# aleximmer/Laplace

Hardware: AMD Instinct MI355X
Metric: KFAC-GGN fit samples/sec, ResNet-18 (higher is better)
Workload: dtype f32 (fp16x2-split products, fp32 accumulate); 1 GPU; c4: ResNet-18 (CIFAR stem, BN frozen) full-network KFAC exact GGN fit, per-GPU minibatch 128, synthetic N(0,1) 3x32x32, 10 classes, N=50000; per_gpu_batch=128, parallelism=dp1, minibatches_in_flight=2

## Files before the change

### include/laplace_hip.h

```cpp
#ifndef LAPLACE_HIP_H
#define LAPLACE_HIP_H

#include <stddef.h>
#include <stdint.h>

#ifdef __cplusplus
extern "C" {
#endif

#define LK_OK 0
#define LK_EINVAL (-1)
#define LK_EWORKSPACE (-2)
#define LK_ELAUNCH (-3)
#define LK_ENOTCONV (-4)

#define LK_GRAM_UPPER_ONLY 1u
#define LK_GRAM_SLABS_PERSIST 2u

int lk_version(void);
const char* lk_last_error(void);

size_t lk_loss_workspace_bytes(int64_t B);
int lk_softmax_hess_sqrt_f32(const float* f, const int64_t* y, int64_t B, int64_t C, float* S,
                             float* loss_accum, float* ws, void* stream);

#define LK_SOFTMAX_CHOL_MAX_C 2000
int lk_softmax_hess_chol_f32(const float* f, const int64_t* y, int64_t B, int64_t C, float* S,
                             float* loss_accum, float* ws, void* stream);

int lk_sq_err_sum_f32(const float* f, const float* y, int64_t numel, float scale, float* loss_accum,
                      float* ws, void* stream);

size_t lk_gram_workspace_bytes(int64_t n, int64_t K);
size_t lk_gram_nt_workspace_bytes(int64_t nb_total, int64_t n, int64_t L);
#define LK_GRAM_TN 0
#define LK_GRAM_NT 1
#define LK_GRAM_CONV 2
#define LK_GRAM_XCORR_FULL 3
#define LK_GRAM_XCORR_STRIPS 4
int lk_gram_launch_variant(int entry, int64_t n, int64_t K, int64_t L, int vec4_ok, unsigned flags, int* out);
int lk_gram_slabs_reduce_f32(float* slabs, size_t slabs_bytes, int64_t n, int64_t L_nt, float alpha, float* C,
                             unsigned flags, void* stream);
int lk_gram_tn_f32(const float* X, int64_t K, int64_t n, int64_t ldx, float alpha, float* C,
                   unsigned flags, void* ws, size_t ws_bytes, void* stream);
int lk_gram_nt_f32(const float* X, int64_t nb, int64_t n, int64_t L, float alpha, float* C,
                   unsigned flags, void* ws, size_t ws_bytes, void* stream);
int lk_gram_nt_seg_f32(const float* const* segs, int64_t nseg, int64_t nb, int64_t n, int64_t L, float alpha,
                       float* C, unsigned flags, void* ws, size_t ws_bytes, void* stream);
int lk_gram_conv_nhwc_f32(const float* x, int64_t B, int64_t H, int64_t W, int64_t Cin, int kh, int kw,
                          int sh, int sw, int ph, int pw, int dh, int dw, float alpha, float* C,
                          unsigned flags, void* ws, size_t ws_bytes, void* stream);

int lk_conv3x3_pixgram_assemble_f32(const float* Cp, int64_t H, int64_t W, int64_t Cin, float alpha, float* A,
                                    void* stream);

int lk_conv3x3_pixpair_plan(int64_t H, int64_t W, int64_t Cin, int64_t* tile, int64_t* n_tiles, int64_t* n_blocks);
int lk_conv3x3_pixpair_tables(int64_t H, int64_t W, int64_t Cin, int32_t* tiles, int32_t* slots);
int lk_conv3x3_pixpair_accumulate_f32(const float* x, int64_t B, int64_t H, int64_t W, int64_t Cin, float alpha,
                                      float* blocks, const int32_t* tiles_dev, int64_t n_tiles, void* stream);
int lk_conv3x3_pixpair_assemble_f32(const float* blocks, const int32_t* slots_dev, int64_t H, int64_t W, int64_t Cin,
                                    float alpha, float* A, void* stream);
int lk_conv3x3_pixpair_assemble2_f32(const float* blocks, const float* blocks2, const int32_t* slots_dev, int64_t H, int64_t W,
                                     int64_t Cin, float alpha, float* A, int upper_only, void* stream);
int lk_conv3x3_pixpair_accumulate_f16x2(const void* x_h, const void* x_l, const int* sexp, int64_t B, int64_t H, int64_t W,
                                        int64_t Cin, float alpha, float* blocks, const int32_t* tiles_dev, int64_t n_tiles,
                                        const void* zero16, void* stream);
int lk_conv3x3_pixpair_accumulate13_f16x2(const void* x_h, const void* x_l, const int* sexp, int64_t B, int64_t H, int64_t W,
                                          int64_t Cin, float alpha, float* blocks, const int32_t* slots_dev, const void* zero16,
                                          void* stream);

size_t lk_conv3x3_shiftcorr_workspace_bytes(int64_t B, int64_t H, int64_t W, int64_t Cin);
int lk_conv3x3_shiftcorr_f32(const float* x, int64_t B, int64_t H, int64_t W, int64_t Cin, float alpha, float* C,
                             void* ws, size_t ws_bytes, void* stream);

int lk_nchw_to_nhwc_f32(const float* src, int64_t B, int64_t C, int64_t HW, float* dst, void* stream);

int lk_symmetrize_f32(float* C, int64_t n, void* stream);

int lk_permute_sym_f32(const float* src, int64_t Cin, int64_t KK, float* dst, int accumulate, void* stream);

int lk_finalize_factors_f32(int64_t count, const float* const* src, float* const* dst, const float* const* scale,
                            const int64_t* n, const int64_t* cin, const int64_t* kk, void* stream);

int lk_absmax_f32(const float* x, int64_t n, const float* cscale, int64_t inner, int64_t C, unsigned* out, void* stream);
int lk_split_f16x2(const float* x, int64_t n, const float* amax, float bound_mul, void* planes_h, void* planes_l,
                   int* sexp, void* stream);
int lk_split_images_f16x2(const float* x, int64_t N, int64_t per, void* planes_h, void* planes_l, int* sexp, unsigned* amax,
                          void* stream);

int lk_im2col_split_f16x2(const float* x, int64_t B, int64_t H, int64_t W, int64_t C, int64_t KH, int64_t KW, int64_t stride,
                          int64_t pad, int64_t Ho, int64_t Wo, int64_t Kp, const float* amax, void* planes_h, void* planes_l,
                          int* sexp, void* stream);
int lk_conv_prep_weights_f16x2(const float* W, int64_t Co, int64_t Ci, int64_t taps, int transpose, const float* cscale,
                               unsigned* amax_ws, void* planes, int* sexp, void* stream);
int lk_conv_nhwc_f16x2(const void* in_h, const void* in_l, const int* in_sexp, int64_t in_nsexp, int64_t N, int64_t Hi,
                       int64_t Wi, int64_t Ci, const void* w_h, const void* w_l, const int* w_sexp, int64_t Co, int64_t Hc,
                       int64_t Wc, int64_t in_mul, int64_t Ho, int64_t Wo, int64_t out_step, int64_t oh0, int64_t ow0,
                       int64_t T, const int* taps, const void* zero16, float* out, int accumulate, unsigned* amax_out,
                       int config, void* stream);

int lk_conv_nhwc_f16x2_planes(const void* in_h, const void* in_l, const int* in_sexp, int64_t in_nsexp, const void* in_amax,
                              int64_t N, int64_t Hi, int64_t Wi, int64_t Ci, const void* w_h, const void* w_l,
                              const int* w_sexp, const float* w_l1, int64_t Co, int64_t Ho, int64_t Wo, int64_t in_mul, int64_t T,
                              const int* taps, const void* zero16, void* out_h, void* out_l, int* out_sexp, int config,
                              void* stream);

int lk_conv_bn_act_nhwc_f16x2(const void* in_h, const void* in_l, const int* in_sexp, int64_t in_nsexp, const void* in_amax,
                              int64_t in_namax, int64_t N, int64_t Hi, int64_t Wi, int64_t Ci, const void* w_h, const void* w_l,
                              const int* w_sexp, const float* w_l1, int64_t Co, int64_t Ho, int64_t Wo, int64_t in_mul,
                              int64_t T, const int* taps, const void* zero16, const float* scale, const float* shift,
                              const void* scale_amax, const void* shift_amax, const float* addend, const float* addend_bound,
                              int64_t addend_nbound, int act, float* y, void* mask, void* y_h, void* y_l, int* y_sexp,
                              float* y_bound, void* y_amax, int config, void* stream);

int lk_conv_nhwc_f16x2_vjp(const void* in_h, const void* in_l, const int* in_sexp, const void* in_amax, int64_t N, int64_t Hi,
                           int64_t Wi, int64_t Ci, const void* w_h, const void* w_l, const int* w_sexp, const float* w_l1,
                           int64_t Co, int64_t Ho, int64_t Wo, int64_t T, const int* taps, const void* zero16,
                           const void* add_h, const void* add_l, const int* add_sexp, const void* mask, int mask_is_float,
                           const void* mult_amax, int64_t mask_rows, const float* scale, const void* scale_amax, void* out_h,
                           void* out_l, int* out_sexp, void* out_amax, int config, void* stream);
int lk_conv_winp_eligible(int64_t N, int64_t Hi, int64_t Wi, int64_t Ci, int64_t Co, int64_t T, int mask_is_float);
int lk_conv_nhwc_f16x2_vjp_wc(const void* in_h, const void* in_l, const int* in_sexp, const void* in_amax, int64_t N, int64_t Hi,
                              int64_t Wi, int64_t Ci, const void* w_h, const void* w_l, const int* w_sexp, const float* w_l1,
                              const void* wc_h, const void* wc_l, int64_t Co, int64_t Ho, int64_t Wo, int64_t T, const int* taps,
                              const void* zero16, const void* add_h, const void* add_l, const int* add_sexp, const void* mask,
                              int mask_is_float, const void* mult_amax, int64_t mask_rows, const float* scale,
                              const void* scale_amax, void* out_h, void* out_l, int* out_sexp, void* out_amax, int config,
                              void* stream);

int lk_conv_nhwc_f16x2_vjp_strided(const void* in_h, const void* in_l, const int* in_sexp, const void* in_amax, const void* w_h,
                                   const void* w_l, const int* w_sexp, const float* w_l1, const void* in2_h, const void* in2_l,
                                   const int* in2_sexp, const void* in2_amax, const void* w2_h, const void* w2_l,
                                   const int* w2_sexp, const float* w2_l1, int64_t N, int64_t Hi, int64_t Wi, int64_t Ci,
                                   int64_t Co, int64_t Ho, int64_t Wo, int64_t os, int64_t T, const int* taps,
                                   const void* zero16, const void* add_h, const void* add_l, const int* add_sexp,
                                   const void* mask, int mask_is_float, const void* mult_amax, int64_t mask_rows,
                                   const float* scale, const void* scale_amax, void* out_h, void* out_l, int* out_sexp,
                                   void* out_amax, int config, void* stream);


int lk_vjp_nhwc_split_f16x2(const float* g, const unsigned* g_amax, const void* g2_h, const void* g2_l, const int* g2_sexp,
                            const void* m, int m_is_float, const unsigned* m_amax, const float* scale,
                            const unsigned* scale_amax, int64_t C, int64_t S, int64_t per, void* out_h, void* out_l,
                            int* out_sexp, void* stream);
int lk_bn_act_fwd_nhwc_f16x2(const float* x, const unsigned* x_amax, int64_t x_namax, const float* x_mul, const float* x_add,
                             const float* scale, const float* shift, const unsigned* scale_amax, const unsigned* shift_amax,
                             const float* addend, const float* addend_bound, int64_t addend_nbound, int act, int64_t C,
                             int64_t N, int64_t per, float* y, void* mask, void* y_h, void* y_l, int* y_sexp, float* y_bound,
                             unsigned* y_amax, void* stream);
int lk_copy_absmax_f32(const float* x, float* y, int64_t n, unsigned* amax, void* stream);

int lk_pack_upper_f32(const float* A, int64_t n, float* packed, void* stream);
int lk_unpack_upper_f32(const float* packed, int64_t n, float* A, void* stream);

int lk_gemm_f32(const float* A, const float* B, const float* E, float* C, int64_t batch, int64_t M, int64_t N, int64_t K,
                int64_t lda, int64_t ldb, int64_t ldc, int64_t lde, int64_t stride_a, int64_t stride_b, int64_t stride_c,
                int trans_a, int trans_b, float alpha, int accumulate, void* stream);
int lk_kron_pow_f32(const float* l1, int64_t n1, const float* l2, int64_t n2, const float* delta, float exponent,
                    int damping, float* lam, void* stream);
int lk_unsplit_transpose_f32(const void* x_h, const void* x_l, const int* sexp, int64_t S, int64_t B, int64_t L, int64_t C,
                             float* out, void* stream);
size_t lk_gram_tn_f16x2_workspace_bytes(int64_t R, int64_t C);
int lk_gram_tn_f16x2(const void* x_h, const void* x_l, const int* sexp, int64_t R, int64_t C, float alpha, float* G,
                     const void* zero16, void* ws, size_t ws_bytes, void* stream);

int lk_diag_ggn_linear_f32(const float* a, const float* g, int64_t B, int64_t Cc, int64_t Di, int64_t Do,
                           float alpha, float* h_w, float* h_b, void* stream);

int lk_jac_linear_f32(const float* a, const float* g, int64_t B, int64_t Cc, int64_t Di, int64_t Do,
                      float* Js, int64_t P, int64_t col0, int64_t bcol0, void* stream);
int lk_jac_conv_f32(const float* x_nchw, const float* g, int64_t B, int64_t Cc, int64_t Cin, int64_t H, int64_t W,
                    int64_t Do, int kh, int kw, int sh, int sw, int ph, int pw, int dh, int dw,
                    float* Js, int64_t P, int64_t col0, int64_t bcol0, void* stream);

int lk_jac_norm_affine_f32(const float* g, const float* xhat, int64_t S, int64_t B, int64_t L, int64_t Ch, int layout,
                           float* Js, int64_t P, int64_t wcol0, int64_t bcol0, void* stream);

int lk_jac_norm_affine_nhwc_f16x2(const void* g_h, const void* g_l, const int* sexp, const float* x, const float* mu,
                                  const float* rstd, int64_t S, int64_t B, int64_t L, int64_t Ch, float* Js, int64_t P,
                                  int64_t wcol0, int64_t bcol0, void* stream);
int lk_normtap_variant(int64_t S, int64_t B, int64_t L, int64_t Ch, int affine, int aligned);

#define LK_NORMVJP_ROW 0
#define LK_NORMVJP_TILE 1
int lk_norm_fwd_f32(const float* x, const float* w, const float* b, int64_t B, int64_t L, int64_t Ch, int64_t G, int layout,
                    float eps, float* y, float* xhat, float* rstd, void* stream);
int lk_norm_vjp_f32(const float* g, const float* xhat, const float* rstd, const float* w, int64_t S, int64_t B, int64_t L,
                    int64_t Ch, int64_t G, int layout, float* dx, unsigned* amax, void* stream);
int lk_norm_sweep_variant(int64_t S, int64_t B, int64_t L, int64_t Ch, int64_t G, int layout, int aligned);

int lk_rmsnorm_fwd_f32(const float* x, const float* w, int64_t rows, int64_t D, float eps, float* y, float* rstd,
                       void* stream);
int lk_rmsnorm_vjp_f32(const float* g, const float* x, const float* rstd, const float* w, int64_t S, int64_t rows, int64_t D,
                       float* dx, unsigned* amax, void* stream);
int lk_rmsnorm_variant(int64_t S, int64_t rows, int64_t D, int aligned);

#define LK_ATTN_RESIDENT_MAX_T 256
int lk_attn_fwd_f32(const float* q, const float* k, const float* v, int64_t B, int64_t H, int64_t T, int64_t D, int layout,
                    float scale, int causal, float* o, float* lse, void* stream);
size_t lk_attn_vjp_workspace_bytes(int64_t S, int64_t B, int64_t H, int64_t T, int64_t D);
int lk_attn_vjp_f32(const float* go, const float* q, const float* k, const float* v, const float* o, const float* lse, int64_t S,
                    int64_t B, int64_t H, int64_t T, int64_t D, int layout, float scale, int causal, float* dq, float* dk,
                    float* dv, void* ws, size_t ws_bytes, void* stream);
int lk_attn_variant(int64_t S, int64_t B, int64_t H, int64_t T, int64_t D, int layout, int causal);

#define LK_POOL_MAX 0
#define LK_POOL_AVG 1
int lk_pool_fwd_nhwc_f32(int kind, const float* x, int64_t B, int64_t H, int64_t W, int64_t C, int kh, int kw, int sh, int sw,
                         int ph, int pw, int count_include_pad, int divisor_override, float* y, uint8_t* arg, void* stream);
int lk_pool_vjp_nhwc_f32(int kind, const float* g, const uint8_t* arg, int64_t S, int64_t B, int64_t H, int64_t W, int64_t C,
                         int kh, int kw, int sh, int sw, int ph, int pw, int count_include_pad, int divisor_override, float* dx,
                         unsigned* amax, void* stream);
int lk_pool_variant(int kind, int64_t S, int64_t B, int64_t H, int64_t W, int64_t C, int kh, int kw, int sh, int sw, int ph,
                    int pw, int aligned);

int lk_dwconv_fwd_nhwc_f32(const float* x, const float* w_tap, const float* bias, int64_t B, int64_t H, int64_t W, int64_t C,
                           int kh, int kw, int sh, int sw, int ph, int pw, float* y, void* stream);
int lk_dwconv_bwd_nhwc_f16x2(const void* g_h, const void* g_l, const int* sexp, const float* w_tap, int64_t S, int64_t B,
                             int64_t H, int64_t W, int64_t C, int kh, int kw, int sh, int sw, int ph, int pw, float* dx,
                             unsigned* amax, void* stream);
int lk_dwconv_variant(int64_t S, int64_t B, int64_t H, int64_t W, int64_t C, int kh, int kw, int sh, int sw, int ph, int pw,
                      int aligned);
// ... 155 lines not shown
```

### laplace_amd/_lib.py

```python
from __future__ import annotations

import ctypes
import os
from typing import Optional

import torch

_HERE = os.path.dirname(os.path.abspath(__file__))
LIB_PATH = os.environ.get("LK_LIB") or os.path.join(_HERE, "csrc", "liblaplace_hip.so")

LK_GRAM_UPPER_ONLY = 1
LK_GRAM_SLABS_PERSIST = 2

_c_f32p = ctypes.c_void_p
_i64 = ctypes.c_int64
_int = ctypes.c_int
_f32 = ctypes.c_float
_sz = ctypes.c_size_t
_vp = ctypes.c_void_p
_u32 = ctypes.c_uint

SIGNATURES = {
    "lk_version": (_int, []),
    "lk_last_error": (ctypes.c_char_p, []),
    "lk_im2col_split_f16x2": (_int, [_vp, _i64, _i64, _i64, _i64, _i64, _i64, _i64, _i64, _i64, _i64, _i64, _vp, _vp, _vp, _vp, _vp]),
    "lk_comm_unique_id": (_int, [_vp]),
    "lk_comm_init_rank": (_int, [ctypes.POINTER(ctypes.c_void_p), _int, _vp, _int]),
    "lk_comm_destroy": (_int, [_vp]),
    "lk_allreduce_sum_f32": (_int, [_vp, _vp, _i64, _vp]),
    "lk_loss_workspace_bytes": (_sz, [_i64]),
    "lk_softmax_hess_sqrt_f32": (_int, [_vp, _vp, _i64, _i64, _vp, _vp, _vp, _vp]),
    "lk_softmax_hess_chol_f32": (_int, [_vp, _vp, _i64, _i64, _vp, _vp, _vp, _vp]),
    "lk_sq_err_sum_f32": (_int, [_vp, _vp, _i64, _f32, _vp, _vp, _vp]),
    "lk_gram_workspace_bytes": (_sz, [_i64, _i64]),
    "lk_gram_nt_workspace_bytes": (_sz, [_i64, _i64, _i64]),
    "lk_gram_launch_variant": (_int, [_int, _i64, _i64, _i64, _int, _u32, _vp]),
    "lk_gram_slabs_reduce_f32": (_int, [_vp, _sz, _i64, _i64, _f32, _vp, _u32, _vp]),
    "lk_gram_tn_f32": (_int, [_vp, _i64, _i64, _i64, _f32, _vp, _u32, _vp, _sz, _vp]),
    "lk_gram_nt_f32": (_int, [_vp, _i64, _i64, _i64, _f32, _vp, _u32, _vp, _sz, _vp]),
    "lk_gram_nt_seg_f32": (_int, [_vp, _i64, _i64, _i64, _i64, _f32, _vp, _u32, _vp, _sz, _vp]),
    "lk_gram_conv_nhwc_f32": (
        _int,
        [_vp, _i64, _i64, _i64, _i64, _int, _int, _int, _int, _int, _int, _int, _int, _f32, _vp, _u32, _vp, _sz, _vp],
    ),
    "lk_conv3x3_shiftcorr_workspace_bytes": (_sz, [_i64, _i64, _i64, _i64]),
    "lk_conv3x3_shiftcorr_f32": (_int, [_vp, _i64, _i64, _i64, _i64, _f32, _vp, _vp, _sz, _vp]),
    "lk_conv3x3_pixgram_assemble_f32": (_int, [_vp, _i64, _i64, _i64, _f32, _vp, _vp]),
    "lk_conv3x3_pixpair_plan": (_int, [_i64, _i64, _i64, _vp, _vp, _vp]),
    "lk_conv3x3_pixpair_tables": (_int, [_i64, _i64, _i64, _vp, _vp]),
    "lk_conv3x3_pixpair_accumulate_f32": (_int, [_vp, _i64, _i64, _i64, _i64, _f32, _vp, _vp, _i64, _vp]),
    "lk_conv3x3_pixpair_accumulate_f16x2": (_int, [_vp, _vp, _vp, _i64, _i64, _i64, _i64, _f32, _vp, _vp, _i64, _vp, _vp]),
    "lk_conv3x3_pixpair_accumulate13_f16x2": (_int, [_vp, _vp, _vp, _i64, _i64, _i64, _i64, _f32, _vp, _vp, _vp, _vp]),
    "lk_conv3x3_pixpair_assemble_f32": (_int, [_vp, _vp, _i64, _i64, _i64, _f32, _vp, _vp]),
    "lk_conv3x3_pixpair_assemble2_f32": (_int, [_vp, _vp, _vp, _i64, _i64, _i64, _f32, _vp, _int, _vp]),
    "lk_nchw_to_nhwc_f32": (_int, [_vp, _i64, _i64, _i64, _vp, _vp]),
    "lk_absmax_f32": (_int, [_vp, _i64, _vp, _i64, _i64, _vp, _vp]),
    "lk_copy_absmax_f32": (_int, [_vp, _vp, _i64, _vp, _vp]),
    "lk_split_f16x2": (_int, [_vp, _i64, _vp, _f32, _vp, _vp, _vp, _vp]),
    "lk_split_images_f16x2": (_int, [_vp, _i64, _i64, _vp, _vp, _vp, _vp, _vp]),
    "lk_conv_prep_weights_f16x2": (_int, [_vp, _i64, _i64, _i64, _int, _vp, _vp, _vp, _vp, _vp]),
    "lk_conv_nhwc_f16x2": (_int, [_vp, _vp, _vp, _i64, _i64, _i64, _i64, _i64, _vp, _vp, _vp, _i64, _i64, _i64, _i64, _i64, _i64,
                                  _i64, _i64, _i64, _i64, _vp, _vp, _vp, _int, _vp, _int, _vp]),
    "lk_conv_nhwc_f16x2_planes": (_int, [_vp, _vp, _vp, _i64, _vp, _i64, _i64, _i64, _i64, _vp, _vp, _vp, _vp, _i64, _i64, _i64, _i64,
                                         _i64, _vp, _vp, _vp, _vp, _vp, _int, _vp]),
    "lk_conv_bn_act_nhwc_f16x2": (_int, [_vp, _vp, _vp, _i64, _vp, _i64, _i64, _i64, _i64, _i64, _vp, _vp, _vp, _vp, _i64, _i64, _i64,
                                         _i64, _i64, _vp, _vp, _vp, _vp, _vp, _vp, _vp, _vp, _i64, _int, _vp, _vp, _vp, _vp, _vp,
                                         _vp, _vp, _int, _vp]),
    "lk_conv_nhwc_f16x2_vjp": (_int, [_vp, _vp, _vp, _vp, _i64, _i64, _i64, _i64, _vp, _vp, _vp, _vp, _i64, _i64, _i64, _i64,
                                      _vp, _vp, _vp, _vp, _vp, _vp, _int, _vp, _i64, _vp, _vp, _vp, _vp, _vp,
                                      _vp, _int, _vp]),
    "lk_conv_winp_eligible": (_int, [_i64, _i64, _i64, _i64, _i64, _i64, _int]),
    "lk_conv_nhwc_f16x2_vjp_wc": (_int, [_vp, _vp, _vp, _vp, _i64, _i64, _i64, _i64, _vp, _vp, _vp, _vp, _vp, _vp, _i64, _i64, _i64,
                                         _i64, _vp, _vp, _vp, _vp, _vp, _vp, _int, _vp, _i64, _vp, _vp, _vp, _vp, _vp, _vp, _int,
                                         _vp]),
    "lk_conv_nhwc_f16x2_vjp_strided": (_int, [_vp] * 16 + [_i64] * 9 + [_vp, _vp, _vp, _vp, _vp, _vp, _int, _vp, _i64, _vp, _vp, _vp,
                                               _vp, _vp, _vp, _int, _vp]),
    "lk_vjp_nhwc_split_f16x2": (_int, [_vp, _vp, _vp, _vp, _vp, _vp, _int, _vp, _vp, _vp, _i64, _i64, _i64, _vp, _vp, _vp, _vp]),
    "lk_bn_act_fwd_nhwc_f16x2": (_int, [_vp, _vp, _i64, _vp, _vp, _vp, _vp, _vp, _vp, _vp, _vp, _i64, _int, _i64, _i64, _i64, _vp, _vp,
                                        _vp, _vp, _vp, _vp, _vp, _vp]),
    "lk_unsplit_transpose_f32": (_int, [_vp, _vp, _vp, _i64, _i64, _i64, _i64, _vp, _vp]),
    "lk_gram_tn_f16x2_workspace_bytes": (_sz, [_i64, _i64]),
    "lk_gram_tn_f16x2": (_int, [_vp, _vp, _vp, _i64, _i64, _f32, _vp, _vp, _vp, _sz, _vp]),
    "lk_gemm_f32": (_int, [_vp, _vp, _vp, _vp, _i64, _i64, _i64, _i64, _i64, _i64, _i64, _i64, _i64, _i64, _i64, _int, _int, _f32,
                           _int, _vp]),
    "lk_kron_pow_f32": (_int, [_vp, _i64, _vp, _i64, _vp, _f32, _int, _vp, _vp]),
    "lk_pack_upper_f32": (_int, [_vp, _i64, _vp, _vp]),
    "lk_unpack_upper_f32": (_int, [_vp, _i64, _vp, _vp]),
    "lk_symmetrize_f32": (_int, [_vp, _i64, _vp]),
    "lk_permute_sym_f32": (_int, [_vp, _i64, _i64, _vp, _int, _vp]),
    "lk_finalize_factors_f32": (_int, [_i64, _vp, _vp, _vp, _vp, _vp, _vp, _vp]),
    "lk_diag_ggn_linear_f32": (_int, [_vp, _vp, _i64, _i64, _i64, _i64, _f32, _vp, _vp, _vp]),
    "lk_jac_linear_f32": (_int, [_vp, _vp, _i64, _i64, _i64, _i64, _vp, _i64, _i64, _i64, _vp]),
    "lk_jac_conv_f32": (
        _int,
        [_vp, _vp, _i64, _i64, _i64, _i64, _i64, _i64, _int, _int, _int, _int, _int, _int, _int, _int, _vp, _i64, _i64, _i64, _vp],
    ),
    "lk_jac_gconv_f32": (
        _int,
        [_vp, _vp, _i64, _i64, _i64, _i64, _i64, _i64, _i64, _int, _int, _int, _int, _int, _int, _int, _int, _vp, _i64, _i64, _i64,
         _vp],
    ),
    "lk_sq_colsum_f32": (_int, [_vp, _i64, _i64, _i64, _i64, _f32, _vp, _vp]),
    "lk_jac_norm_affine_f32": (_int, [_vp, _vp, _i64, _i64, _i64, _i64, _int, _vp, _i64, _i64, _i64, _vp]),
    "lk_norm_fwd_f32": (_int, [_vp, _vp, _vp, _i64, _i64, _i64, _i64, _int, _f32, _vp, _vp, _vp, _vp]),
    "lk_norm_vjp_f32": (_int, [_vp, _vp, _vp, _vp, _i64, _i64, _i64, _i64, _i64, _int, _vp, _vp, _vp]),
    "lk_norm_sweep_variant": (_int, [_i64, _i64, _i64, _i64, _i64, _int, _int]),
    "lk_rmsnorm_fwd_f32": (_int, [_vp, _vp, _i64, _i64, _f32, _vp, _vp, _vp]),
    "lk_rmsnorm_vjp_f32": (_int, [_vp, _vp, _vp, _vp, _i64, _i64, _i64, _vp, _vp, _vp]),
    "lk_rmsnorm_variant": (_int, [_i64, _i64, _i64, _int]),
    "lk_attn_fwd_f32": (_int, [_vp, _vp, _vp, _i64, _i64, _i64, _i64, _int, _f32, _int, _vp, _vp, _vp]),
    "lk_attn_vjp_workspace_bytes": (_sz, [_i64, _i64, _i64, _i64, _i64]),
    "lk_attn_vjp_f32": (_int, [_vp, _vp, _vp, _vp, _vp, _vp, _i64, _i64, _i64, _i64, _i64, _int, _f32, _int, _vp, _vp, _vp, _vp,
                               _sz, _vp]),
    "lk_attn_variant": (_int, [_i64, _i64, _i64, _i64, _i64, _int, _int]),
    "lk_pool_fwd_nhwc_f32": (_int, [_int, _vp, _i64, _i64, _i64, _i64] + [_int] * 8 + [_vp, _vp, _vp]),
    "lk_pool_vjp_nhwc_f32": (_int, [_int, _vp, _vp, _i64, _i64, _i64, _i64, _i64] + [_int] * 8 + [_vp, _vp, _vp]),
    "lk_pool_variant": (_int, [_int, _i64, _i64, _i64, _i64, _i64] + [_int] * 7),
    "lk_cat_fwd_nhwc_f32": (_int, [_vp, _i64, _i64, _vp, _i64, _i64, _vp]),
    "lk_cat_vjp_nhwc_f32": (_int, [_int, _vp, _vp, _vp, _vp, _i64, _i64, _i64, _i64, _vp, _vp, _vp]),
    "lk_cat_variant": (_int, [_int, _int, _i64, _i64, _i64, _i64, _int]),
    "lk_slice_fwd_f32": (_int, [_vp, _i64, _i64, _i64, _i64, _vp, _vp]),
    "lk_slice_vjp_f32": (_int, [_int, _vp, _vp, _vp, _vp, _vp, _vp, _i64, _i64, _vp, _vp, _vp]),
    "lk_slice_variant": (_int, [_int, _int, _vp, _vp, _i64, _i64, _int]),
    "lk_mul_vjp_f32": (_int, [_vp, _vp, _vp, _i64, _i64, _i64, _int, _vp, _vp, _vp]),
    "lk_mul_variant": (_int, [_i64, _i64, _i64, _int, _int, _int, _int]),
    "lk_gate_reduce_nhwc_f32": (_int, [_vp, _vp, _vp, _vp, _vp, _i64, _i64, _i64, _i64, _vp, _vp]),
    "lk_gate_vjp_nhwc_f32": (_int, [_vp, _vp, _vp, _vp, _vp, _vp, _i64, _i64, _i64, _i64, _vp, _vp, _vp]),
    "lk_gate_variant": (_int, [_int, _i64, _i64, _i64, _i64, _int]),
    "lk_softmax_vjp_f32": (_int, [_vp, _vp, _i64, _i64, _i64, _int, _vp, _vp]),
    "lk_softmax_vjp_variant": (_int, [_i64, _i64, _i64, _int, _int]),
    "lk_matmul_vjp_f32": (_int, [_vp, _vp, _vp, _i64, _i64, _i64, _i64, _i64, _vp, _vp, _vp]),
    "lk_matmul_vjp_variant": (_int, [_i64, _i64, _i64, _i64, _i64, _int, _int]),
    "lk_dwconv_fwd_nhwc_f32": (_int, [_vp, _vp, _vp, _i64, _i64, _i64, _i64] + [_int] * 6 + [_vp, _vp]),
    "lk_dwconv_bwd_nhwc_f16x2": (_int, [_vp, _vp, _vp, _vp, _i64, _i64, _i64, _i64, _i64] + [_int] * 6 + [_vp, _vp, _vp]),
    "lk_dwconv_variant": (_int, [_i64, _i64, _i64, _i64, _i64] + [_int] * 7),
    "lk_jac_norm_affine_nhwc_f16x2": (_int, [_vp] * 6 + [_i64] * 4 + [_vp, _i64, _i64, _i64, _vp]),
    "lk_normtap_variant": (_int, [_i64, _i64, _i64, _i64, _int, _int]),
    "lk_bn_act_fwd_f32": (_int, [_vp, _vp, _vp, _vp, _i64, _i64, _i64, _int, _vp, _vp, _vp]),
    "lk_vjp_scale_mask_f32": (_int, [_vp, _vp, _vp, _int, _vp, _i64, _i64, _i64, _i64, _vp, _vp]),
    "lk_ll_ggn_workspace_bytes": (_sz, [_i64, _i64, _i64]),
    "lk_ll_ggn_full_f32": (_int, [_vp, _vp, _i64, _i64, _i64, _int, _f32, _vp, _vp, _sz, _vp]),
    "lk_syevj_workspace_bytes": (_sz, [_i64]),
    "lk_syevj_f32": (_int, [_vp, _i64, _vp, _vp, _int, _int, _vp, _vp, _sz, _vp]),
    "lk_syevj_batched_f32": (_int, [_i64, _vp, _vp, _vp, _vp, _vp, _vp, _vp, _int, _int, _vp, _i64]),
    "lk_kron_logdet_workspace_bytes": (_sz, [_i64]),
    "lk_kron_logdet_f32": (_int, [_vp, _i64, _vp, _i64, _vp, _int, _vp, _vp, _vp, _vp, _vp, _sz, _vp]),
    "lk_kron_logdet_blocks_workspace_bytes": (_sz, [_i64, _i64]),
    "lk_kron_logdet_blocks_f32": (_int, [_i64, _vp, _vp, _vp, _vp, _vp, _vp, _vp, _vp, _vp, _vp, _sz, _vp]),
    "lk_kron_quadform_linear_f32": (_int, [_vp, _vp, _vp, _vp, _vp, _i64, _i64, _i64, _i64, _vp, _vp, _vp, _vp, _vp]),
    "lk_diag_quadform_linear_f32": (_int, [_vp, _vp, _vp, _vp, _i64, _i64, _i64, _i64, _vp, _vp]),
    "lk_quadform_shared_workspace_bytes": (_sz, [_i64, _i64, _i64, _i64]),
    "lk_kron_quadform_shared_planes_f16x2": (_int, [_vp, _vp, _vp, _vp, _vp, _vp, _i64, _vp, _vp, _vp, _i64, _i64, _i64, _i64, _i64,
                                                    _vp, _vp, _vp, _sz, _vp]),
    "lk_kron_quadform_shared_seedmajor_f32": (_int, [_vp, _vp, _vp, _vp, _vp, _i64, _i64, _i64, _i64, _i64, _vp, _vp, _sz, _vp]),
    "lk_kron_quadform_shared_f32": (_int, [_vp, _vp, _vp, _vp, _vp, _i64, _i64, _i64, _i64, _i64, _vp, _vp, _sz, _vp]),
    "lk_diag_quadform_shared_f32": (_int, [_vp, _vp, _vp, _i64, _i64, _i64, _i64, _i64, _vp, _vp, _sz, _vp]),
    "lk_diag_ggn_shared_workspace_bytes": (_sz, [_i64, _i64, _i64]),
    "lk_diag_ggn_shared_f32": (_int, [_vp, _vp, _i64, _i64, _i64, _i64, _i64, ctypes.c_float, _vp, _vp, _sz, _vp]),
    "lk_diag_quadform_js_f32": (_int, [_vp, _vp, _i64, _i64, _i64, _vp, _vp]),
    "lk_dense_quadform_ll_workspace_bytes": (_sz, [_i64, _i64, _i64]),
    "lk_jac_last_layer_f32": (_int, [_vp, _i64, _i64, _i64, _int, _vp, _vp]),
    "lk_dense_quadform_ll_f32": (_int, [_vp, _vp, _i64, _i64, _i64, _int, _vp, _vp, _sz, _vp]),
    "lk_quadform_linear_grid_f32": (_int, [_vp, _vp, _vp, _vp, _vp, _i64, _int, _i64, _i64, _i64, _i64, _vp, _vp, _vp, _vp]),
    "lk_quadform_shared_grid_workspace_bytes": (_sz, [_i64, _i64, _i64, _i64, _i64]),
    "lk_quadform_shared_grid_f32": (_int, [_vp, _vp, _vp, _vp, _vp, _i64, _int, _i64, _i64, _i64, _i64, _i64, _int, _vp, _vp, _sz,
                                           _vp]),
    "lk_quadform_shared_variant": (_int, [_int, _i64, _i64, _i64, _i64, _i64, _int]),
    "lk_conv_launch_variant": (_int, [_int] + [_i64] * 14 + [ctypes.POINTER(ctypes.c_int), _i64, _int, _int, _int,
                                      ctypes.POINTER(ctypes.c_int)]),
    "lk_conv_strided_launch_variant": (_int, [_i64] * 9 + [ctypes.POINTER(ctypes.c_int), _int, ctypes.POINTER(ctypes.c_int)]),
    "lk_probit_nll_grid_f32": (_int, [_vp, _vp, _vp, _i64, _i64, _i64, _vp, _vp]),
    "lk_spectral_workspace_bytes": (_sz, [_int, _i64, _i64, _i64, _i64]),
    "lk_spectral_quadform_ll_f32": (_int, [_vp, _vp, _vp, _f32, _vp, _i64, _i64, _i64, _int, _vp, _vp, _sz, _vp]),
    "lk_spectral_grid_ll_f32": (_int, [_vp, _vp, _vp, _f32, _vp, _i64, _i64, _i64, _i64, _int, _vp, _vp, _sz, _vp]),
    "lk_spectral_quadform_f32": (_int, [_vp, _vp, _f32, _vp, _i64, _i64, _i64, _vp, _vp, _sz, _vp]),
    "lk_spectral_grid_f32": (_int, [_vp, _vp, _f32, _vp, _i64, _i64, _i64, _i64, _vp, _vp, _sz, _vp]),
    "lk_spectral_variant": (_int, [_int, _i64, _i64, _i64, _i64, _int]),
}


class LaplaceHipError(RuntimeError):
    pass


class SplitTensor:

    __slots__ = ("planes", "sexp", "amax", "chunked")

    def __init__(self, planes: torch.Tensor, sexp: torch.Tensor, amax: torch.Tensor | None = None, chunked: bool = False):
        self.planes, self.sexp, self.amax, self.chunked = planes, sexp, amax, bool(chunked)

    @property
    def shape(self):
        if self.chunked:
            _, N, nch, D, w = self.planes.shape
            return torch.Size((N, D, nch * w))
        return self.planes.shape[1:]

    def chunk_major(self) -> "SplitTensor":
        if self.chunked:
            return self
        _, N, D, L = self.planes.shape
        pl = self.planes.view(2, N, D, L // 16, 16).permute(0, 1, 3, 2, 4).contiguous()
        return SplitTensor(pl, self.sexp, self.amax, chunked=True)

    @property
    def per_image(self) -> bool:
# ... 603 lines not shown
        out = torch.empty(B, S, C, H * W, dtype=torch.float32, device=x.planes.device)
        self._rc(self.lib.lk_unsplit_transpose_f32(_ptr(x.planes[0]), _ptr(x.planes[1]), _ptr(x.sexp), S, B, H * W, C,
                                                   _ptr(out), self._stream(out.device)), "lk_unsplit_transpose_f32")
        return out

    def gram_tn_f16x2(self, x, alpha, out):
        _check(out, "out")
        _one_scale(x, "gram_tn_f16x2")
        C = x.planes.shape[-1]
        R = x.planes[0].numel() // C
        nbytes = int(self.lib.lk_gram_tn_f16x2_workspace_bytes(R, C))
        if nbytes == 0 and R:
            raise LaplaceHipError(f"gram_tn_f16x2: C = {C} not supported (64 or a multiple of 128)")
        ws = self._workspace(nbytes, out.device)
        z = self._zero16(out.device)
        self._rc(self._timed("gram16", float(R) * C * (C + 1), out.device, lambda: self.lib.lk_gram_tn_f16x2(
            _ptr(x.planes[0]), _ptr(x.planes[1]), _ptr(x.sexp), R, C, float(alpha), _ptr(out), _ptr(z), _ptr(ws),
            ws.numel(), self._stream(out.device))), "lk_gram_tn_f16x2")
        return out

    def pack_upper(self, A, packed):
        _check(A, "A"), _check(packed, "packed")
        self._rc(self.lib.lk_pack_upper_f32(_ptr(A), A.shape[0], _ptr(packed), self._stream(A.device)), "lk_pack_upper_f32")

    def unpack_upper(self, packed, A):
        _check(A, "A"), _check(packed, "packed")
        self._rc(self.lib.lk_unpack_upper_f32(_ptr(packed), A.shape[0], _ptr(A), self._stream(A.device)), "lk_unpack_upper_f32")

    def gemm(self, A, B, C, batch, M, N, Kd, lda, ldb, ldc, sa=0, sb=0, sc=0, ta=False, tb=False, E=None, lde=0,
             alpha=1.0, accumulate=False):
        self._rc(self.lib.lk_gemm_f32(_ptr(A), _ptr(B), _ptr(E), _ptr(C), batch, M, N, Kd, lda, ldb, ldc, lde, sa, sb, sc,
                                      1 if ta else 0, 1 if tb else 0, float(alpha), 1 if accumulate else 0,
                                      self._stream(C.device)), "lk_gemm_f32")

    def kron_pow(self, l1, l2, delta, exponent, damping=False):
        _check(l1, "l1")
        n1 = l1.numel()
        n2 = 0 if l2 is None else l2.numel()
        lam = torch.empty((n1, n2) if l2 is not None else (n1,), dtype=torch.float32, device=l1.device)
        d = delta.detach().reshape(-1)[:1].to(torch.float32).contiguous()
        self._rc(self.lib.lk_kron_pow_f32(_ptr(l1), n1, _ptr(l2), n2, _ptr(d), float(exponent), 1 if damping else 0,
                                          _ptr(lam), self._stream(l1.device)), "lk_kron_pow_f32")
        return lam

    def kron_sandwich(self, W, col0, P, R, Q1, Q2, lam, out):
        _check(W, "W"), _check(out, "out"), _check(Q1, "Q1"), _check(lam, "lam")
        Wv, Ov = W.reshape(-1)[col0:], out.reshape(-1)[col0:]
        if Q2 is None:
            p = Q1.shape[0]
            T = torch.empty(R, p, dtype=torch.float32, device=W.device)
            self.gemm(Wv, Q1, T, 1, R, p, p, P, p, p, E=lam, lde=0)
            self.gemm(T, Q1, Ov, 1, R, p, p, p, p, P, tb=True)
            return out
        _check(Q2, "Q2")
        pi, po = Q1.shape[0], Q2.shape[0]
        T = torch.empty(R, pi, po, dtype=torch.float32, device=W.device)
        U = torch.empty(R, pi, po, dtype=torch.float32, device=W.device)
        self.gemm(Wv, Q2, T, R, pi, po, po, po, po, po, sa=P, sc=pi * po)
        self.gemm(Q1, T, U, R, pi, po, pi, pi, po, po, sb=pi * po, sc=pi * po, ta=True, E=lam, lde=po)
        self.gemm(Q1, U, T, R, pi, po, pi, pi, po, po, sb=pi * po, sc=pi * po)
        self.gemm(T, Q2, Ov, R, pi, po, po, po, po, po, sa=pi * po, sc=P, tb=True)
        return out

    def gram_conv(self, x, kernel_size, stride, padding, dilation, alpha, out, upper_only=False, native=False):
        _check(out, "out")
        if not self.is_channels_last(x):
            _check(x, "x")
        B, Cin, H, W = x.shape
        kh, kw = _pair(kernel_size)
        sh, sw = _pair(stride)
        ph, pw = _pair(padding)
        dh, dw = _pair(dilation)
        n = Cin * kh * kw
        assert out.shape == (n, n)
        OH = (H + 2 * ph - dh * (kh - 1) - 1) // sh + 1
        OW = (W + 2 * pw - dw * (kw - 1) - 1) // sw + 1
        xh = self.nchw_to_nhwc(x)
        direct = native or kh * kw == 1
        tgt = out if direct else torch.zeros(n, n, dtype=torch.float32, device=x.device)
        if self.use_shiftcorr and (kh, kw, sh, sw, ph, pw, dh, dw) == (3, 3, 1, 1, 1, 1, 1, 1) and H * W >= 256 and B > 0:
            nb = self.lib.lk_conv3x3_shiftcorr_workspace_bytes(B, H, W, Cin)
            ws = self._workspace(nb, x.device)
            self._rc(
                self._timed("shiftcorr", float(B * H * W) * n * (n + 1), x.device, lambda: self.lib.lk_conv3x3_shiftcorr_f32(
                    _ptr(xh), B, H, W, Cin, float(alpha), _ptr(tgt), _ptr(ws), ws.numel(), self._stream(x.device))),
                "lk_conv3x3_shiftcorr_f32",
            )
            if not direct:
                self._rc(self.lib.lk_permute_sym_f32(_ptr(tgt), Cin, kh * kw, _ptr(out), 1, self._stream(x.device)),
                         "lk_permute_sym_f32")
            return out
        nb = self.lib.lk_gram_workspace_bytes(n, max(B * OH * OW, 1))
        ws = self._workspace(nb, x.device)
        self._rc(
            self._timed("gram_conv", float(B * OH * OW) * n * (n + 1), x.device, lambda: self.lib.lk_gram_conv_nhwc_f32(
                _ptr(xh), B, H, W, Cin, kh, kw, sh, sw, ph, pw, dh, dw, float(alpha), _ptr(tgt),
                LK_GRAM_UPPER_ONLY if upper_only else 0, _ptr(ws), ws.numel(), self._stream(x.device))),
            "lk_gram_conv_nhwc_f32",
        )
        if not direct:
            self._rc(self.lib.lk_permute_sym_f32(_ptr(tgt), Cin, kh * kw, _ptr(out), 1, self._stream(x.device)),
                     "lk_permute_sym_f32")
        return out

    pixgram_max_hw = 16

    def pixgram_accumulate(self, x, alpha, Cp):
        _check(Cp, "Cp")
        B = x.shape[0]
        xh = self.nchw_to_nhwc(x)
        return self.gram_tn(xh.reshape(B, -1), alpha, Cp, upper_only=True)

    def pixgram_assemble(self, Cp, H, W, Cin, alpha, A_native):
        _check(Cp, "Cp"), _check(A_native, "A")
        self.symmetrize(Cp)
        self._rc(self.lib.lk_conv3x3_pixgram_assemble_f32(_ptr(Cp), int(H), int(W), int(Cin), float(alpha), _ptr(A_native),
                                                          self._stream(Cp.device)), "lk_conv3x3_pixgram_assemble_f32")
        return A_native

    def pixpair_plan(self, H, W, Cin, dev):
        key = (int(H), int(W), int(Cin), str(dev))
        cache = self.__dict__.setdefault("_pixpair_cache", {})
        if key not in cache:
            T, nt, nb = ctypes.c_int64(), ctypes.c_int64(), ctypes.c_int64()
            plan = None
            if Cin >= 64 and Cin % 64 == 0 and self.lib.lk_conv3x3_pixpair_plan(
                    int(H), int(W), int(Cin), ctypes.byref(T), ctypes.byref(nt), ctypes.byref(nb)) == 0:
                tiles = torch.empty(nt.value, 3, dtype=torch.int32)
                slots = torch.empty(int(H) * int(W), 13, dtype=torch.int32)
                self._rc(self.lib.lk_conv3x3_pixpair_tables(int(H), int(W), int(Cin), ctypes.c_void_p(tiles.data_ptr()),
                                                            ctypes.c_void_p(slots.data_ptr())), "lk_conv3x3_pixpair_tables")
                plan = (nb.value, tiles.to(dev), slots.to(dev))
            cache[key] = plan
        return cache[key]

    def pixpair_accumulate(self, x, alpha, blocks, plan):
        return self.pixpair_accumulate_nhwc(self.nchw_to_nhwc(x), alpha, blocks, plan)

    def pixpair_accumulate_nhwc(self, xh, alpha, blocks, plan):
        _check(xh, "xh"), _check(blocks, "blocks")
        B, H, W, Cin = xh.shape
        nb, tiles, _ = plan
        assert blocks.numel() == nb * Cin * Cin
        x = xh
        self._rc(self._timed("pixpair", 8.0 * blocks.numel() + 4.0 * x.numel(), x.device,
                             lambda: self.lib.lk_conv3x3_pixpair_accumulate_f32(
                                 _ptr(xh), B, H, W, Cin, float(alpha), _ptr(blocks), ctypes.c_void_p(tiles.data_ptr()),
                                 tiles.shape[0], self._stream(x.device))), "lk_conv3x3_pixpair_accumulate_f32")
        return blocks

    use_pixpair16 = True
    use_pixpair13 = True

    def pixpair_accumulate_split(self, xs, alpha, blocks, plan):
        _check(blocks, "blocks")
        _one_scale(xs, "pixpair_accumulate_split")
        B, H, W, Cin = xs.shape
        nb, tiles, slots = plan
        assert blocks.numel() == nb * Cin * Cin
        dev = blocks.device
        z = self._zero16(dev)
        if Cin == 64 and self.use_pixpair13:
            self._rc(self._timed("pixpair16", 8.0 * blocks.numel() + 4.0 * xs.planes[0].numel(), dev,
                                 lambda: self.lib.lk_conv3x3_pixpair_accumulate13_f16x2(
                                     _ptr(xs.planes[0]), _ptr(xs.planes[1]), _ptr(xs.sexp), B, H, W, Cin, float(alpha), _ptr(blocks),
                                     ctypes.c_void_p(slots.data_ptr()), _ptr(z), self._stream(dev))),
                     "lk_conv3x3_pixpair_accumulate13_f16x2")
            return blocks
        self._rc(self._timed("pixpair16", 8.0 * blocks.numel() + 4.0 * xs.planes[0].numel(), dev,
                             lambda: self.lib.lk_conv3x3_pixpair_accumulate_f16x2(
                                 _ptr(xs.planes[0]), _ptr(xs.planes[1]), _ptr(xs.sexp), B, H, W, Cin, float(alpha), _ptr(blocks),
                                 ctypes.c_void_p(tiles.data_ptr()), tiles.shape[0], _ptr(z), self._stream(dev))),
                 "lk_conv3x3_pixpair_accumulate_f16x2")
        return blocks

    def pixpair_assemble(self, blocks, plan, H, W, Cin, alpha, A_native, blocks2=None, upper_only=False):
        _check(blocks, "blocks"), _check(A_native, "A")
        if blocks2 is not None:
            _check(blocks2, "blocks2")
            assert blocks2.numel() == blocks.numel()
        self._rc(self.lib.lk_conv3x3_pixpair_assemble2_f32(_ptr(blocks), _ptr(blocks2), ctypes.c_void_p(plan[2].data_ptr()),
                                                           int(H), int(W), int(Cin), float(alpha), _ptr(A_native),
                                                           1 if upper_only else 0, self._stream(blocks.device)),
                 "lk_conv3x3_pixpair_assemble2_f32")
        return A_native

    def permute_native_to_unfold(self, src, Cin, KK, dst, accumulate=False):
        _check(src, "src"), _check(dst, "dst")
        self._rc(self.lib.lk_permute_sym_f32(_ptr(src), Cin, KK, _ptr(dst), 1 if accumulate else 0, self._stream(src.device)),
                 "lk_permute_sym_f32")
        return dst

    def finalize_factors(self, items):
        items = [it for it in items if it[0].numel()]
        if not items:
            return
        n = len(items)
        dev = items[0][0].device
        src = (ctypes.c_void_p * n)()
        dst = (ctypes.c_void_p * n)()
        scl = (ctypes.c_void_p * n)()
        ns = (ctypes.c_int64 * n)()
        cins = (ctypes.c_int64 * n)()
        kks = (ctypes.c_int64 * n)()
        for i, (s_, d_, sc_, cin, kk) in enumerate(items):
            _check(s_, "src")
            assert s_.dim() == 2 and s_.shape[0] == s_.shape[1] and s_.device == dev
            src[i] = s_.data_ptr()
            if d_ is not None:
                _check(d_, "dst")
                assert d_.shape == s_.shape
                dst[i] = d_.data_ptr()
            if sc_ is not None:
                _check(sc_, "scale")
                assert sc_.numel() == s_.shape[0]
                scl[i] = sc_.data_ptr()
            ns[i], cins[i], kks[i] = s_.shape[0], int(cin), int(kk)
        self._rc(self.lib.lk_finalize_factors_f32(n, src, dst, scl, ns, cins, kks, self._stream(dev)), "lk_finalize_factors_f32")

    def symmetrize(self, C):
        _check(C, "C")
        self._rc(self.lib.lk_symmetrize_f32(_ptr(C), C.shape[0], self._stream(C.device)), "lk_symmetrize_f32")
        return C

    def diag_ggn_linear(self, a, g, alpha, h_w, h_b=None):
        _check(a, "a"), _check(g, "g"), _check(h_w, "h_w")
        Cc, B, Do = g.shape
        Di = a.shape[1]
        assert a.shape[0] == B and h_w.numel() == Do * Di
        if h_b is not None:
            _check(h_b, "h_b")
        self._rc(
            self.lib.lk_diag_ggn_linear_f32(_ptr(a), _ptr(g), B, Cc, Di, Do, float(alpha), _ptr(h_w), _ptr(h_b),
                                            self._stream(a.device)),
            "lk_diag_ggn_linear_f32",
        )

    def jac_linear(self, a, g, Js, col0, bcol0=-1):
        _check(a, "a"), _check(g, "g"), _check(Js, "Js")
        Cc, B, Do = g.shape
        Di = a.shape[1]
        P = Js.shape[-1]
        self._rc(
            self.lib.lk_jac_linear_f32(_ptr(a), _ptr(g), B, Cc, Di, Do, _ptr(Js), P, int(col0), int(bcol0),
                                       self._stream(a.device)),
            "lk_jac_linear_f32",
        )

    def jac_conv(self, x, g, kernel_size, stride, padding, dilation, Js, col0, bcol0=-1):
        _check(x, "x"), _check(g, "g"), _check(Js, "Js")
        B, Cin, H, W = x.shape
        Cc, _, Do = g.shape[:3]
        kh, kw = _pair(kernel_size)
        sh, sw = _pair(stride)
        ph, pw = _pair(padding)
        dh, dw = _pair(dilation)
        P = Js.shape[-1]
        self._rc(
            self.lib.lk_jac_conv_f32(_ptr(x), _ptr(g), B, Cc, Cin, H, W, Do, kh, kw, sh, sw, ph, pw, dh, dw, _ptr(Js), P,
                                     int(col0), int(bcol0), self._stream(x.device)),
            "lk_jac_conv_f32",
        )

    def jac_gconv(self, x, g, kernel_size, stride, padding, dilation, groups, Js, col0, bcol0=-1):
        _check(x, "x"), _check(g, "g"), _check(Js, "Js")
        B, Cin, H, W = x.shape
        Cc, _, Do = g.shape[:3]
        if g.shape[1] != B or Js.shape[:2] != (B, Cc):
            raise LaplaceHipError("jac_gconv: x [B, Cin, H, W], g [S, B, Do, ...] and Js [B, S, P] do not match")
        kh, kw = _pair(kernel_size)
        sh, sw = _pair(stride)
        ph, pw = _pair(padding)
        dh, dw = _pair(dilation)
        self._rc(
            self.lib.lk_jac_gconv_f32(_ptr(x), _ptr(g), B, Cc, Cin, H, W, Do, int(groups), kh, kw, sh, sw, ph, pw, dh, dw,
                                      _ptr(Js), Js.shape[-1], int(col0), int(bcol0), self._stream(x.device)),
            "lk_jac_gconv_f32",
        )

    def jac_norm_affine(self, g, xhat, Ch, layout, Js, wcol0, bcol0=-1):
        _check(g, "g"), _check(xhat, "xhat"), _check(Js, "Js")
        S, B = g.shape[:2]
        if xhat.numel() * S != g.numel() or xhat.shape[0] != B or Js.shape[:2] != (B, S):
            raise LaplaceHipError("jac_norm_affine: g [S, B, ...], xhat [B, ...] and Js [B, S, P] do not match")
        L = xhat.numel() // max(B * int(Ch), 1)
        if B * L * int(Ch) != xhat.numel():
            raise LaplaceHipError("jac_norm_affine: xhat is not [B, Ch, L] / [B, L, Ch]")
        self._rc(
            self.lib.lk_jac_norm_affine_f32(_ptr(g), _ptr(xhat), S, B, L, int(Ch), int(layout), _ptr(Js), Js.shape[-1],
                                            int(wcol0), int(bcol0), self._stream(g.device)),
            "lk_jac_norm_affine_f32",
        )

    def jac_norm_affine_nhwc(self, g: "SplitTensor", x, mu, rstd, S, Js, wcol0, bcol0=-1):
        _one_scale(g, "jac_norm_affine_nhwc")
        if g.chunked:
            raise LaplaceHipError("jac_norm_affine_nhwc: a chunk-major split tensor is an operand of the weight-sharing "
                                  "predictive; this kernel reads position-major planes [S*B, .., Ch]")
        _check(g.planes, "g.planes", torch.float16), _check(g.sexp, "g.sexp", torch.int32), _check(x, "x"), _check(Js, "Js")
        S = int(S)
        if x.dim() < 2 or g.planes.dim() != x.dim() + 1 or S < 1 or g.planes.shape[1] != S * x.shape[0] \
                or tuple(g.planes.shape[2:]) != tuple(x.shape[1:]) or Js.dim() != 3 or tuple(Js.shape[:2]) != (x.shape[0], S):
            raise LaplaceHipError("jac_norm_affine_nhwc: g [S*B, .., Ch], x [B, .., Ch] and Js [B, S, P] do not match")
        B, Ch = x.shape[0], x.shape[-1]
        if (mu is None) != (rstd is None):
            raise LaplaceHipError("jac_norm_affine_nhwc: mu and rstd are given together or not at all")
        for name, t in (("mu", mu), ("rstd", rstd)):
            if t is not None and tuple(_check(t, name).shape) != (Ch,):
                raise LaplaceHipError(f"jac_norm_affine_nhwc: {name} must be [Ch]")
        L = x.numel() // max(B * Ch, 1)
        self._rc(
            self.lib.lk_jac_norm_affine_nhwc_f16x2(_ptr(g.planes[0]), _ptr(g.planes[1]), _ptr(g.sexp), _ptr(x), _ptr(mu), _ptr(rstd),
                                                   S, B, max(L, 1), Ch, _ptr(Js), Js.shape[-1], int(wcol0), int(bcol0),
                                                   self._stream(x.device)),
            "lk_jac_norm_affine_nhwc_f16x2",
        )

    def normtap_variant(self, S, B, L, Ch, affine=True, aligned=True):
        r = int(self.lib.lk_normtap_variant(int(S), int(B), int(L), int(Ch), int(bool(affine)), int(bool(aligned))))
        if r < 0:
            return None
        return {"vec": (1, 4, 8)[r & 3], "seed_split": bool(r & 4), "affine": bool(r & 8), "seeds_per_pass": (r >> 4) & 0xF,
                "lane_rows": 1 << ((r >> 8) & 0xF), "seeds_per_slice": (r >> 12) & 0xFF, "channel_tiles": r >> 20}

    @staticmethod
    def _norm_geometry(x, B, G, layout, what):
        if x.dim() < 2 or x.shape[0] != B:
            raise LaplaceHipError(f"{what}: expected [B, Ch, ...] / [B, ..., Ch]")
        Ch = int(x.shape[1] if layout == 0 else x.shape[-1])
        L = x.numel() // max(B * Ch, 1) if x.numel() else 1
        if G < 1 or Ch % G or layout not in (0, 1):
            raise LaplaceHipError(f"{what}: G must divide the {Ch} channels; layout is 0 or 1")
        return max(L, 1), Ch

    def norm_forward(self, x, w, b, G, layout, eps):
        _check(x, "x")
        B = x.shape[0]
        L, Ch = self._norm_geometry(x, B, int(G), int(layout), "norm_forward")
        for t, name in ((w, "w"), (b, "b")):
            if t is not None:
                _check(t, name)
                if t.numel() != Ch:
                    raise LaplaceHipError(f"norm_forward: {name} must have {Ch} elements")
        y, xhat = torch.empty_like(x), torch.empty_like(x)
        rstd = torch.empty(B, int(G), dtype=torch.float32, device=x.device)
        self._rc(self.lib.lk_norm_fwd_f32(_ptr(x), _ptr(w), _ptr(b), B, L, Ch, int(G), int(layout), float(eps), _ptr(y),
                                          _ptr(xhat), _ptr(rstd), self._stream(x.device)), "lk_norm_fwd_f32")
        return y, xhat, rstd

    def norm_vjp(self, g, xhat, rstd, w, S, G, layout, amax=None):
        _check(g, "g"), _check(xhat, "xhat"), _check(rstd, "rstd")
        B = xhat.shape[0]
        L, Ch = self._norm_geometry(xhat, B, int(G), int(layout), "norm_vjp")
        if g.numel() != int(S) * xhat.numel() or rstd.numel() != B * int(G):
            raise LaplaceHipError("norm_vjp: g [S*B, ...], xhat [B, ...] and rstd [B, G] do not match")
        if w is not None:
            _check(w, "w")
            if w.numel() != Ch:
                raise LaplaceHipError(f"norm_vjp: w must have {Ch} elements")
        if amax is not None and (amax.numel() != 1 or amax.element_size() != 4):
            raise LaplaceHipError("norm_vjp: amax is one 32-bit device word")
        dx = torch.empty_like(g)
        self._rc(self.lib.lk_norm_vjp_f32(_ptr(g), _ptr(xhat), _ptr(rstd), _ptr(w), int(S), B, L, Ch, int(G), int(layout),
                                          _ptr(dx), _ptr(amax), self._stream(g.device)), "lk_norm_vjp_f32")
        return dx

    NORMVJP_ROW, NORMVJP_TILE = 0, 1

    def norm_sweep_variant(self, S, B, L, Ch, G, layout, aligned=True):
        r = int(self.lib.lk_norm_sweep_variant(int(S), int(B), int(L), int(Ch), int(G), int(layout), int(bool(aligned))))
        if r < 0:
# ... 894 lines not shown
```

### laplace_amd/backend.py

```python
from __future__ import annotations

import collections
import math
import threading
import os
from collections.abc import MutableMapping

import torch
import torch.nn.functional as F
from torch import nn

from laplace_amd._lib import SplitTensor, get_kernels, is_channels_last, keep_layout
from laplace_amd.capture import NormTapReused, Tape, norm_servable
from laplace_amd.sweep import SeedBatchedSweep, SweepUnsupported
from laplace_amd.sweep_nhwc import NhwcNormGrad, SplitSweep
from laplace_amd.kron import HipKron
from laplace_amd.refapi import EFInterface, GGNInterface


_OWN_ROTATION = True


def shared_operands(tap, g, B, C, Q1=None, Q2=None, bounds=None, planes: bool = True):
    m = tap.module
# ... 565 lines not shown
            K.jac_norm_affine(g.g.reshape(g.g.shape[0] // B, *g.xhat.shape), g.xhat, self._norm_channels(tap.module), 1, Js,
                              wcol0, bcol0)
        else:
            xhat, Ch, layout = self._norm_xhat(tap)
            K.jac_norm_affine(g.contiguous(), xhat, Ch, layout, Js, wcol0, bcol0)

    def _norm_block(self, tap, g):
        Ch = self._norm_channels(tap.module)
        if isinstance(g, (SplitTensor, NhwcNormGrad)):
            B = tap.a.shape[0]
            S, dev = (g.shape[0] if isinstance(g, SplitTensor) else g.g.shape[0]) // B, tap.a.device
        else:
            S, B, dev = g.shape[0], g.shape[1], g.device
        n_w, n_b = (Ch if tap.w_off >= 0 else 0), (Ch if tap.b_off >= 0 else 0)
        Jl = torch.zeros(B, S, n_w + n_b, dtype=torch.float32, device=dev)
        self._norm_columns(tap, g, Jl, 0 if n_w else -1, n_w if n_b else -1)
        return Jl, n_w, n_b

    def _kron_impl(self, x, y, N, seeds_fn, hess_scale_fn, kfac_approx):
        if kfac_approx not in ("expand", "reduce"):
            raise ValueError(f"kfac_approx must be 'expand' or 'reduce', got {kfac_approx!r}")
        acc = KronAccumulator(self, N, kfac_approx, overlap=True)
        acc.defer_pix = bool(self.lazy_kron and self.lazy_pixpair and acc.use_pixgram and kfac_approx == "expand")
        if not acc.defer_pix:
            acc.use_pixgram = False
        acc._persist_slabs = False
        acc.lanes = 1
        acc.coalesce = False
        try:
            acc.add_batch(x, y)
        except NotImplementedError as e:
            if "KFAC supports" in str(e):
                raise NotImplementedError(
                    "KFAC supports nn.Linear / nn.Conv2d parameters only (as the reference, docs/index.md:364-366); "
                    "freeze the others (requires_grad=False)") from e
            raise
        if self.lazy_kron:
            return acc.loss[0].clone(), HipKron(None, pending=acc)
        return acc.finalize()

    lazy_kron = True
    lazy_pixpair = True

    def _diag_impl(self, x, y, seeds_fn, alpha):
        K = get_kernels()
        f, tape, grad_fn = self._forward(x, norm=True)
        if self._unserved(tape):
            tape.release()
            return None
        loss = torch.zeros(1, dtype=torch.float32, device=f.device)
        seeds, _ = seeds_fn(f, y, loss)
        grads = grad_fn(seeds)
        h = torch.zeros(tape.n_params, dtype=torch.float32, device=f.device)
        B, S = f.shape[0], seeds.shape[0]
        for tap, g in zip(self._served_taps(tape), grads):
            if tap.kind == "norm":
                Jl, n_w, n_b = self._norm_block(tap, g)
                if n_w:
                    K.sq_colsum(Jl, 0, n_w, alpha, h[tap.w_off:tap.w_off + n_w])
                if n_b:
                    K.sq_colsum(Jl, n_w, n_b, alpha, h[tap.b_off:tap.b_off + n_b])
                continue
            if tap.kind == "gconv":
                for _, Jl, n_w, n_b in self._gconv_blocks(tap, g):
                    K.sq_colsum(Jl, 0, n_w, alpha, h[tap.w_off:tap.w_off + n_w])
                    if n_b:
                        K.sq_colsum(Jl, n_w, n_b, alpha, h[tap.b_off:tap.b_off + n_b])
                continue
            a = tap.a.to(torch.float32)
            m = tap.module
            if tap.kind == "linear" and a.ndim == 2:
                n_w = m.out_features * m.in_features
                K.diag_ggn_linear(a.contiguous(), g.contiguous(), alpha, h[tap.w_off:tap.w_off + n_w],
                                  h[tap.b_off:tap.b_off + m.out_features] if tap.has_bias else None)
            else:
                width = m.weight.numel()
                n_out = m.weight.shape[0]
                if n_out >= 32 and width // n_out >= 64:
                    smax = K.quadform_shared_max_outputs
                    u, v, gsum = shared_operands(tap, g, B, S)
                    for s0 in range(0, S, smax):
                        us = u if S <= smax else u[:, s0:s0 + smax].contiguous()
                        K.diag_ggn_shared(us, v, alpha, h[tap.w_off:tap.w_off + width])
                    if tap.has_bias:
                        h[tap.b_off:tap.b_off + n_out] += alpha * (gsum * gsum).sum((0, 1))
                else:
                    Jl = torch.zeros(B, S, width + (n_out if tap.has_bias else 0), dtype=torch.float32, device=f.device)
                    a4, g5, ks, st, pd, dl = self._conv_view(tap, a, g)
                    K.jac_conv(a4, g5, ks, st, pd, dl, Jl, 0, width if tap.has_bias else -1)
                    K.sq_colsum(Jl, 0, width, alpha, h[tap.w_off:tap.w_off + width])
                    if tap.has_bias:
                        K.sq_colsum(Jl, width, n_out, alpha, h[tap.b_off:tap.b_off + n_out])
        tape.release()
        if self.subnetwork_indices is not None:
            h = h[self.subnetwork_indices]
        return loss[0], h

    def _full_from_rows(self, Z, alpha):
        K = get_kernels()
        Z2 = Z.reshape(-1, Z.shape[-1])
        if self.subnetwork_indices is not None:
            Z2 = Z2[:, self.subnetwork_indices]
        Z2 = Z2.contiguous()
        H = torch.zeros(Z2.shape[1], Z2.shape[1], dtype=torch.float32, device=Z.device)
        return K.gram_tn(Z2, alpha, H)


class CurvatureExchange(list):

    owner = None


_PROCESS_STREAMS: dict = {}
_PROCESS_STREAMS_LOCK = threading.Lock()


def _process_streams(key, make):
    with _PROCESS_STREAMS_LOCK:
        return _process_streams_locked(key, make)


def _process_streams_locked(key, make):
    hit = _PROCESS_STREAMS.get(key)
    if hit is None:
        hit = _PROCESS_STREAMS[key] = make()
    return hit


class KronAccumulator:

    use_pixgram = True
    _defer_bn = True
    _persist_slabs = True
    pix_group = 8
    lag_join = True

    def __init__(self, backend, N: int, kfac_approx: str = "expand", overlap: bool = True):
        twin, dt = backend._twin() if hasattr(backend, "_twin") else (None, torch.float32)
        self._caller, self._out_dtype = (backend, dt) if twin is not None else (None, torch.float32)
        if twin is not None:
            backend = twin
        self.backend, self.N, self.kfac_approx = backend, N, kfac_approx
        self.overlap = overlap
        self._side = None
        self._side_done = None
        self._side_older = []
        self.lag_depth = 1
        self.factors = None
        self.loss = None
        self._taps_meta = None
        self.defer_pix = False
        self._pix_inputs = {}
        self._pix_early = set()
        self.coalesce = bool(type(self).default_coalesce)
        self._stash, self._stash_n = [], 0
        self._dispatched = 0
        self._act_numel = 0
        self.lanes = max(1, int(type(self).default_lanes))
        self._lane_accs, self._lane_next, self._lane_id, self._lane_stream = None, 0, 0, None
        self._lane_sig = None
        self._ahead = collections.deque()
        self._a_done = None
        self._lanes_anywhere = False

    def _alloc(self, tape, dev):
        self.factors, self._taps_meta = [], []
        shapes = []
        for tap in tape.taps:
            m = tap.module
            if tap.kind == "linear":
                do, di = m.out_features, m.in_features
                native = None
            else:
                do, di = m.out_channels, m.in_channels * m.kernel_size[0] * m.kernel_size[1]
                native = (m.in_channels, m.kernel_size[0] * m.kernel_size[1])
            shapes.append((do, di, native is not None and native[1] > 1))
            self._taps_meta.append((tap.has_bias, native))
        pad = lambda n: (n + 63) // 64 * 64
        kept = sum(pad(do * do) + (0 if nat else pad(di * di)) for do, di, nat in shapes) + 64
        natv = sum(pad(di * di) for do, di, nat in shapes if nat)
        flat_k = torch.zeros(kept, dtype=torch.float32, device=dev)
        flat_n = torch.zeros(natv, dtype=torch.float32, device=dev) if natv else None
        ok, on = 0, 0
        for do, di, nat in shapes:
            G = flat_k[ok:ok + do * do].view(do, do)
            ok += pad(do * do)
            if nat:
                A = flat_n[on:on + di * di].view(di, di)
                on += pad(di * di)
            else:
                A = flat_k[ok:ok + di * di].view(di, di)
                ok += pad(di * di)
            self.factors.append([G, A])
        self.loss = flat_k[ok:ok + 1]
        self._pix = {}
        self._pix_pending = {}
        self._gscale = {}
        self._gslabs = {}
        self._tap_index = {tap.name: i for i, tap in enumerate(tape.taps)}

    def ensure_allocated(self, device):
        self._fold_lanes()
        if self.factors is None:
            self._alloc(self.backend._tape(), device)

    def _pix_geometry(self, tap):
        m = tap.module
        if tap.kind != "conv2d" or self.kfac_approx != "expand" or not self.use_pixgram:
            return None
        if (tuple(m.kernel_size), tuple(m.stride), tuple(m.padding), tuple(m.dilation)) != ((3, 3), (1, 1), (1, 1), (1, 1)):
            return None
        K = get_kernels()
        H, W = (int(v) for v in tap.a.shape[-2:])
        Cin = int(m.in_channels)
        if H * W > K.pixgram_max_hw or Cin % 64 == 0:
            plan = K.pixpair_plan(H, W, Cin, tap.a.device)
            if plan is not None and plan[0] * Cin * Cin * 4 <= (1 << 30):
                return ("pair", H, W, Cin, plan)
        if H * W <= K.pixgram_max_hw and H * W * Cin <= 16384:
            return ("dense", H, W, Cin)
        return None

    def _accumulate_A(self, idx, tap, F, rt):
        K = get_kernels()
        if self.defer_pix:
            geo = self._pix_geometry(tap)
            if geo is not None and geo[0] == "pair" and tap.a.dtype == torch.float32:
                t = K.nchw_to_nhwc(keep_layout(tap.a))
                self._pix_inputs.setdefault(idx, []).append((geo, rt / (self.N * geo[1] * geo[2]), t, tap.module))
                return
            self.backend._factor_A(tap, self.N, rt, self.kfac_approx, F[1], fused=True)
            return
        acc = self._pix.get(idx)
        if acc is None:
            self.backend._factor_A(tap, self.N, rt, self.kfac_approx, F[1], fused=True)
            return
        geo, buf = acc
        alpha = rt / (self.N * geo[1] * geo[2])
        a = keep_layout(tap.a.to(torch.float32))
        if geo[0] != "pair":
            K.pixgram_accumulate(a, alpha, buf)
        elif self.pix_group <= 1:
            K.pixpair_accumulate(a, alpha, buf, geo[4])
        else:
            self._push_pix_input(idx, geo, alpha, a, nhwc=False)

    direct_stack = True

    def _pix_sink(self, name, shape, device):
        idx = self._tap_index.get(name)
        pend = self._pix_pending.get(idx) if idx is not None else None
        if pend is None or pend["n"] >= self.pix_group:
            return None
        B = pend["B"]
        stack = pend["stack"]
        if tuple(shape) != (B,) + tuple(stack.shape[1:]) or stack.device != device:
            return None
        cur = torch.cuda.current_stream(device)
        free = pend.pop("free", None)
        if free is not None:
            cur.wait_event(free)
        stack.record_stream(cur)
        return stack[pend["n"] * B:(pend["n"] + 1) * B]

    def _push_pix_input(self, idx, geo, alpha, a, nhwc: bool):
        K = get_kernels()
        B = a.shape[0]
        pend = self._pix_pending.get(idx)
        if pend is not None and (pend["B"] != B or pend["alpha"] != alpha):
            self._drain_pixpair(idx)
            pend = None
        if pend is None:
            stack = torch.empty(self.pix_group * B, geo[1], geo[2], geo[3], dtype=torch.float32, device=a.device)
            planes = (torch.empty((2,) + tuple(stack.shape), dtype=torch.float16, device=a.device)
                      if getattr(K, "use_pixpair16", False) and stack.numel() % 8 == 0 else None)
            word = torch.zeros(1, dtype=torch.float32, device=a.device) if planes is not None and getattr(K, "use_copy_absmax", False) else None
            pend = self._pix_pending[idx] = {"B": B, "alpha": alpha, "stack": stack, "n": 0, "planes": planes, "amax": word}
        slot = pend["stack"][pend["n"] * B:(pend["n"] + 1) * B]
        src = a if nhwc else (a.permute(0, 2, 3, 1) if K.is_channels_last(a) else None)
        if src is not None and src.data_ptr() == slot.data_ptr() and tuple(src.shape) == tuple(slot.shape) and src.is_contiguous():
            pend["amax"] = None
        elif (pend["amax"] is not None and src is not None and src.is_contiguous() and src.dtype == torch.float32
                and src.numel() % 4 == 0 and src.data_ptr() % 16 == 0 and slot.data_ptr() % 16 == 0):
            K.copy_absmax(src, slot, pend["amax"])
        else:
            pend["amax"] = None
            if nhwc:
                slot.copy_(a)
            else:
                K.nchw_to_nhwc(a, out=slot)
        pend["n"] += 1
        if pend["n"] == self.pix_group:
            self._drain_pixpair(idx, keep=True)

    def _adopt_pix_inputs(self, other):
        todo = []
        for idx, items in other._pix_inputs.items():
            if idx not in self._pix:
                mine = self._pix_inputs.setdefault(idx, [])
                mine.extend(items)
                if len(mine) < max(self.pix_group, 2):
                    continue
                geo = mine[0][0]
                self._pix[idx] = (geo, torch.zeros(geo[4][0] * geo[3] * geo[3], dtype=torch.float32, device=mine[0][2].device))
                items = self._pix_inputs.pop(idx)
            todo.append((idx, items))
        return todo

    def _push_adopted(self, todo):
        for idx, items in todo:
            for geo, alpha, t, _ in items:
                self._push_pix_input(idx, geo, alpha, t, nhwc=True)

    def _resolve_pix_inputs(self):
        if not self._pix_inputs:
            return
        K = get_kernels()
        self._join_side()
        for idx, items in self._pix_inputs.items():
            for _, alpha, t, m in items:
                K.gram_conv(t.permute(0, 3, 1, 2), m.kernel_size, m.stride, m.padding, m.dilation, alpha, self.factors[idx][1],
                            upper_only=True, native=True)
        self._pix_inputs = {}

    def _drain_pixpair(self, idx, keep=False):
        pend = self._pix_pending.get(idx)
        if pend is None:
            return
        if pend["n"]:
            geo, buf = self._pix[idx]
            xh = pend["stack"][:pend["n"] * pend["B"]]
            cur = torch.cuda.current_stream(xh.device) if xh.is_cuda else None
            K = get_kernels()
            if getattr(K, "use_pixpair16", False) and xh.numel() % 8 == 0:
                ws = pend.get("planes")
                xs = K.split_f16x2(xh, amax=pend.get("amax"), out=None if ws is None else ws[:, :xh.shape[0]])
                if cur is not None and keep:
                    pend["free"] = torch.cuda.Event()
                    pend["free"].record(cur)
                K.pixpair_accumulate_split(xs, pend["alpha"], buf, geo[4])
            else:
                K.pixpair_accumulate_nhwc(xh, pend["alpha"], buf, geo[4])
                if cur is not None and keep:
                    pend["free"] = torch.cuda.Event()
                    pend["free"].record(cur)
            if cur is not None:
                pend["stack"].record_stream(cur)
                if pend.get("planes") is not None:
                    pend["planes"].record_stream(cur)
                if pend.get("amax") is not None:
                    pend["amax"].record_stream(cur)
        if keep:
            pend["n"] = 0
            if pend.get("planes") is not None and getattr(get_kernels(), "use_copy_absmax", False):
                pend["amax"] = torch.zeros(1, dtype=torch.float32, device=pend["stack"].device)
        else:
            del self._pix_pending[idx]

    def _ensure_pixgrams(self, tape):
        todo = []
        for idx, tap in enumerate(tape.taps):
            if idx in self._pix:
                old = self._pix[idx][0]
                if (old[1], old[2]) == tuple(int(v) for v in tap.a.shape[-2:]):
                    continue
                self._flush_pixgrams(only=idx)
                self._pix_early.add(idx)
            geo = self._pix_geometry(tap)
            if geo is None:
                continue
            if geo[0] == "pair":
                todo.append((idx, geo, (geo[4][0] * geo[3] * geo[3],), tap.a.device))
            else:
                npix = geo[1] * geo[2] * geo[3]
                todo.append((idx, geo, (npix, npix), tap.a.device))
        if not todo:
            return
        pad = lambda n: (n + 63) // 64 * 64
        numel = [math.prod(shape) for _, _, shape, _ in todo]
        flat = torch.zeros(sum(pad(n) for n in numel), dtype=torch.float32, device=todo[0][3])
        off = 0
        for (idx, geo, shape, _), n in zip(todo, numel):
            self._pix[idx] = (geo, flat[off:off + n].view(shape))
            off += pad(n)

    flush_streams = 3
    lane_priority = -1

    def _flush_pixgrams(self, only=None):
        K = get_kernels()
        self._join_side()
        todo = [only] if only is not None else sorted(self._pix, key=lambda i: -self._pix[i][1].numel())

        def one(idx):
            self._drain_pixpair(idx)
            geo, buf = self._pix.pop(idx)
            if geo[0] == "pair":
                K.pixpair_assemble(buf, geo[4], geo[1], geo[2], geo[3], 1.0, self.factors[idx][1], upper_only=True)
            else:
                K.pixgram_assemble(buf, geo[1], geo[2], geo[3], 1.0, self.factors[idx][1])
            return buf

        dev = self.loss.device if self.loss is not None else None
        if len(todo) < 3 or self.flush_streams < 2 or dev is None or dev.type != "cuda" or not self.overlap:
            for idx in todo:
                one(idx)
            return
        streams = _process_streams(("flush", dev, self.flush_streams), lambda: [torch.cuda.Stream(dev) for _ in range(self.flush_streams)])
        cur = torch.cuda.current_stream(dev)
        for st in streams:
            st.wait_stream(cur)
        for j, idx in enumerate(todo):
            st = streams[j % len(streams)]
            with torch.cuda.stream(st):
                buf = one(idx)
            buf.record_stream(st)
            self.factors[idx][1].record_stream(st)
        for st in streams:
            cur.wait_stream(st)

    def _lane_add_batch(self, x, y):
        dev = x.device
        on_device = x.is_cuda
        cur = torch.cuda.current_stream(dev) if on_device else None
        if self._lane_accs is None:
            streams = [None] * self.lanes
            if on_device:
                prio = int(self.lane_priority)
                streams = _process_streams(("lanes", dev, self.lanes, prio),
                                           lambda: [torch.cuda.Stream(dev, priority=prio) for _ in range(self.lanes)])
            self._lane_accs = []
            for k in range(self.lanes):
                sub = KronAccumulator(self.backend, self.N, self.kfac_approx, self.overlap)
                sub.lanes, sub._lane_id, sub._lane_stream = 1, k, streams[k]
                sub.coalesce = False
                sub.use_pixgram, sub.pix_group, sub.lag_join = self.use_pixgram, self.pix_group, self.lag_join
                sub.lag_depth, sub.direct_stack = self.lag_depth, self.direct_stack
                sub._defer_bn, sub._persist_slabs = self._defer_bn, self._persist_slabs
                self._lane_accs.append(sub)
        k = self._lane_next
        self._lane_next = (k + 1) % self.lanes
        sub = self._lane_accs[k]
        if not on_device:
            sub.add_batch(x, y)
            return
        st = sub._lane_stream
        x = x.clone()
        y = y.clone() if torch.is_tensor(y) and y.is_cuda else y
        st.wait_stream(cur)
        if sub.factors is None and k > 0 and self.backend.__dict__.get("_lanes_warm") != self._shared_signature(x):
            first = self._lane_accs[0]
            st.wait_stream(first._lane_stream)
            if first._side is not None:
                st.wait_stream(first._side)
        if self._lane_sig is None:
            self._lane_sig = self._shared_signature(x)
        with torch.cuda.stream(st):
            sub.add_batch(x, y)
        for t in (x, y):
            if torch.is_tensor(t) and t.is_cuda:
                t.record_stream(st)
        self._act_numel = max(self._act_numel, sub._act_numel)
        sub.max_ahead = self.max_ahead
        sub._throttle(st)

    def _shared_signature(self, x):
        m = self.backend.model
        ts = list(m.parameters()) + list(m.buffers())
        return (tuple((t.data_ptr(), t._version) for t in ts), tuple(x.shape[1:]), x.dtype, x.device)

    early_flush = True
    drain_before_fold = True

    def _fold_lanes(self):
        self._flush_stash()
        subs, self._lane_accs = self._lane_accs, None
        if not subs:
            return
        if self._lane_sig is not None and any(sub.factors is not None for sub in subs):
            self.backend.__dict__["_lanes_warm"] = self._lane_sig
        K = get_kernels()
        on_device = subs[0]._lane_stream is not None
        dev = subs[0]._lane_stream.device if on_device else None
        cur = torch.cuda.current_stream(dev) if on_device else None
        live = [sub for sub in subs if sub.factors is not None]
        if on_device and self.drain_before_fold:
            for sub in subs:
                sub._lane_stream.synchronize()
                if sub._side is not None:
                    sub._side.synchronize()
        early = (on_device and self.overlap and self.early_flush and bool(live) and all(sub._a_done is not None for sub in live)
                 and any(sub._pix for sub in live))
        fstreams = None
        if early:
            nfs = max(self.flush_streams, 1)
            fstreams = _process_streams(("flush", dev, nfs), lambda: [torch.cuda.Stream(dev) for _ in range(nfs)])
            for st in fstreams:
                st.wait_stream(cur)
                for sub in live:
                    st.wait_event(sub._a_done)
        else:
            for sub in subs:
                if on_device:
                    cur.wait_stream(sub._lane_stream)
            for sub in live:
                sub._join_side()
        merged = set()
        if live:
            base = live[0]

            def one(idx, st):
                geo, buf = base._pix[idx]
                others = []
                for sub in live[1:]:
                    o = sub._pix.get(idx)
                    if o is None or o[0][:4] != geo[:4] or (geo[0] == "pair" and o[0][4] is not geo[4]):
                        continue
                    pend = sub._pix_pending.pop(idx, None)
                    if pend is not None and pend["n"]:
                        bp = base._pix_pending.get(idx)
                        B = pend["B"]
                        if (bp is not None and bp["B"] == B and bp["alpha"] == pend["alpha"]
                                and bp["n"] + pend["n"] <= bp["stack"].shape[0] // B):
                            bp["stack"][bp["n"] * B:(bp["n"] + pend["n"]) * B].copy_(pend["stack"][:pend["n"] * B])
                            bp["n"] += pend["n"]
                            if bp.get("amax") is not None:
                                if pend.get("amax") is not None:
                                    torch.maximum(bp["amax"], pend["amax"], out=bp["amax"])
                                else:
                                    bp["amax"] = None
                            if st is not None:
                                pend["stack"].record_stream(st)
                        else:
                            sub._pix_pending[idx] = pend
                            sub._drain_pixpair(idx)
                    others.append(o[1])
                    del sub._pix[idx]
                if not others:
                    return False
                base._drain_pixpair(idx)
                del base._pix[idx]
                A = base.factors[idx][1]
                for o in others[1:]:
                    buf.add_(o)
                if geo[0] == "pair":
                    K.pixpair_assemble(buf, geo[4], geo[1], geo[2], geo[3], 1.0, A, blocks2=others[0], upper_only=True)
                else:
                    buf.add_(others[0])
                    K.pixgram_assemble(buf, geo[1], geo[2], geo[3], 1.0, A)
                if st is not None:
                    for t in [buf, A] + others:
                        t.record_stream(st)
                return True

            todo = sorted(base._pix, key=lambda i: -base._pix[i][1].numel())
            for j, idx in enumerate(todo):
                if fstreams is not None:
                    st = fstreams[j % len(fstreams)]
                    with torch.cuda.stream(st):
                        if one(idx, st):
                            merged.add(idx)
                elif one(idx, None):
                    merged.add(idx)
        if early:
            for sub in subs:
                cur.wait_stream(sub._lane_stream)
            for sub in live:
                sub._join_side()
            for st in fstreams:
                cur.wait_stream(st)
        first = True
        for sub in subs:
            if sub.factors is None:
                continue
            sub._flush_pixgrams()
            sub._flush_g_slabs()
            if self.factors is None:
                self.factors, self.loss, self._taps_meta = sub.factors, sub.loss, sub._taps_meta
                self._pix, self._pix_pending, self._gslabs = {}, {}, {}
                self._gscale, self._tap_index = dict(sub._gscale), dict(sub._tap_index)
            else:
                if set(self._gscale) != set(sub._gscale):
                    raise RuntimeError("the lanes of a fit disagree about the deferred BatchNorm scales")
                skip = (merged - sub._pix_early) if not first else set()
                mine = [t for i, F in enumerate(self.factors) for j, t in enumerate(F) if not (j == 1 and i in skip)] + [self.loss]
                theirs = [t for i, F in enumerate(sub.factors) for j, t in enumerate(F) if not (j == 1 and i in skip)] + [sub.loss]
                torch._foreach_add_(mine, theirs)
            first = False
            if on_device:
                for t in sub._raw_tensors():
                    t.record_stream(cur)

    default_coalesce = True
    default_lanes = 2
    coalesce_act_floats = 1 << 28
    coalesce_max_batches = 32

    def coalesce_target(self, x) -> int:
        b = self.backend
        if (not self.coalesce or not torch.is_tensor(x) or not x.is_floating_point() or x.dim() < 2
                or getattr(b, "stochastic", False) or b.last_layer or not self._dispatched):
            return 0
        n_params = sum(p.numel() for p in b.params)
        act = max(int(self._act_numel), x[0].numel(), 1)
        target = min(8192, (1 << 27) // max(n_params, 1), (1 << 24) // max(x[0].numel(), 1),
                     int(self.coalesce_act_floats) // act, int(self.coalesce_max_batches) * x.shape[0])
        return target if target >= 2 * x.shape[0] else 0

    def _flush_stash(self):
        if not self._stash:
            return
        stash, self._stash, self._stash_n = self._stash, [], 0
        if len(stash) == 1:
            self._dispatch(*stash[0])
        else:
            self._dispatch(torch.cat([x for x, _ in stash]), torch.cat([y for _, y in stash]))

    def add_batch(self, x, y):
        if self._caller is not None:
            twin, _ = self._caller._twin()
            x, y = twin._to32(x), twin._to32(y)
        target = self.coalesce_target(x) if torch.is_tensor(x) and torch.is_tensor(y) and y.shape[:1] == x.shape[:1] else 0
        if target:
            if self._stash and (self._stash[0][0].shape[1:] != x.shape[1:] or self._stash[0][0].dtype != x.dtype
                                or self._stash[0][1].shape[1:] != y.shape[1:] or self._stash[0][1].dtype != y.dtype
                                or self._stash[0][0].device != x.device or self._stash_n + x.shape[0] > target):
                self._flush_stash()
            self._stash.append((x.clone(), y.clone()))
            self._stash_n += x.shape[0]
            if self._stash_n >= target:
                self._flush_stash()
            return
        self._flush_stash()
        self._dispatch(x, y)

    max_ahead = 2

    def _throttle(self, stream):
        if not self.max_ahead or stream is None:
            return
        ev = torch.cuda.Event()
        ev.record(stream)
        self._ahead.append(ev)
        if len(self._ahead) > self.max_ahead:
            self._ahead.popleft().synchronize()

    def _dispatch(self, x, y):
        b = self.backend
        self._dispatched += 1
        if self.lanes > 1 and self.overlap and not self.defer_pix and torch.is_tensor(x) and (x.is_cuda or self._lanes_anywhere):
            return self._lane_add_batch(x, y)
        self._add_batch(x, y)
        if torch.is_tensor(x) and x.is_cuda and self._lane_stream is None:
            self._throttle(torch.cuda.current_stream(x.device))

    def _add_batch(self, x, y):
        b = self.backend
        b._tape().refuse_kfac()
        b._act_sink = self._pix_sink if (self.direct_stack and self.overlap and not self.defer_pix and getattr(self, "_pix_pending", None)
                                         and torch.is_tensor(x) and x.is_cuda) else None
        try:
            f, tape, grad_fn = b._forward(x)
        finally:
            b._act_sink = None
        if tape.uncovered:
            raise NotImplementedError("KFAC supports nn.Linear / nn.Conv2d parameters only")
        if self.factors is None:
            self._alloc(tape, f.device)
        if not self._act_numel:
            nb = max(int(f.shape[0]), 1)
            acts = [int(t.a.numel()) // nb for t in tape.taps if torch.is_tensor(getattr(t, "a", None))]
            self._act_numel = max(acts + [1]) * max(int(f.shape[-1]) - 1, 1)
        rt = math.sqrt(float(b.factor))
        if not self.defer_pix:
            self._ensure_pixgrams(tape)
        side = None
        if self.overlap and f.is_cuda:
            if self._side is None:
                self._side = _process_streams(("side", f.device, self._lane_id), lambda: torch.cuda.Stream(f.device))
            side = self._side
            main = torch.cuda.current_stream(f.device)
            side.wait_stream(main)
            with torch.cuda.stream(side):
                for i, (tap, F) in enumerate(zip(tape.taps, self.factors)):
                    self._accumulate_A(i, tap, F, rt)
            self._a_done = torch.cuda.Event()
            self._a_done.record(side)
        else:
            for i, (tap, F) in enumerate(zip(tape.taps, self.factors)):
                self._accumulate_A(i, tap, F, rt)
        seeds, hs = b._kron_seeds(f, y, self.loss)
        defer = getattr(grad_fn, "streams_taps", False) and self._defer_bn
        if getattr(grad_fn, "streams_taps", False):
            by_name = {tap.name: (tap, F) for tap, F in zip(tape.taps, self.factors)}

            def on_tap(name, g):
                tap, F = by_name[name]
                persist = None if isinstance(g, SplitTensor) else self._g_slabs(tap, g, rt * hs)
                if side is None:
                    b._factor_G(tap, g, rt * hs, self.kfac_approx, F[0], fused=True, persist=persist)
                    return
                ev = torch.cuda.Event()
                ev.record(main)
                side.wait_event(ev)
                with torch.cuda.stream(side):
                    b._factor_G(tap, g, rt * hs, self.kfac_approx, F[0], fused=True, persist=persist)
                (g.planes if isinstance(g, SplitTensor) else g).record_stream(side)
                if isinstance(g, SplitTensor) and torch.is_tensor(g.sexp):
                    g.sexp.record_stream(side)

            grad_fn(seeds, stack=False, on_tap=on_tap, defer_bn_scale=defer)
        else:
            grads = grad_fn(seeds, stack=False)
            for tap, g, F in zip(tape.taps, grads, self.factors):
                b._factor_G(tap, g, rt * hs, self.kfac_approx, F[0], fused=True)
        if defer:
            self._note_grad_scales(tape, grad_fn.grad_scale())
        if side is not None:
            if self.lag_join:
                for tap in tape.taps:
                    if torch.is_tensor(tap.a) and tap.a.is_cuda:
                        tap.a.record_stream(side)
                if self._side_done is not None:
                    self._side_older.append(self._side_done)
                while len(self._side_older) >= self.lag_depth and self._side_older:
                    main.wait_event(self._side_older.pop(0))
                self._side_done = torch.cuda.Event()
                self._side_done.record(side)
            else:
                main.wait_stream(side)
        tape.release()

    def _g_slabs(self, tap, g, alpha):
        if not self._persist_slabs or tap.kind != "conv2d" or self.kfac_approx != "expand" or g.dim() != 5:
            return None
        K = get_kernels()
        S, B, Do = g.shape[0], g.shape[1], g.shape[2]
        L = g.shape[3] * g.shape[4]
        need = K.gram_nt_slab_bytes(S * B, Do, L)
        idx = self._tap_index[tap.name]
        cur = self._gslabs.get(idx)
        if cur is not None and (cur[0].numel() < need or cur[2] != L or cur[3] != alpha):
            self._flush_g_slabs(only=idx)
            cur = None
        if cur is None:
            cur = (torch.zeros(need, dtype=torch.uint8, device=g.device), Do, L, alpha)
            self._gslabs[idx] = cur
        return cur[0]

    def _raw_tensors(self):
        return [t for F in self.factors for t in F] + [self.loss]

    def _raw_compatible(self, other) -> bool:
        return (self.factors is not None and other.factors is not None and not other._pix
                and not other._pix_pending and not self._gslabs and not other._gslabs
                and (not (self._pix or self._pix_pending) or all(g[0] == "pair" for g, _ in self._pix.values()))
                and self.N == other.N and self.kfac_approx == other.kfac_approx and self.backend is other.backend
                and self._taps_meta == other._taps_meta and len(self.factors) == len(other.factors)
                and all(a.shape == b.shape for a, b in zip(self._raw_tensors(), other._raw_tensors()))
                and set(self._gscale) == set(other._gscale)
                and all(self._gscale[k] is other._gscale[k] or torch.equal(self._gscale[k], other._gscale[k])
                        for k in self._gscale))

    def clone(self) -> "KronAccumulator":
        self._fold_lanes()
        self._join_side()
        new = KronAccumulator(self.backend, self.N, self.kfac_approx, self.overlap)
        new._caller, new._out_dtype, new.coalesce = self._caller, self._out_dtype, self.coalesce
        new.use_pixgram, new._persist_slabs = self.use_pixgram, self._persist_slabs
        new.defer_pix, new.pix_group = self.defer_pix, self.pix_group
        new._pix_inputs = {k: list(v) for k, v in self._pix_inputs.items()}
        if self.factors is not None:
            if self._gslabs or any(g[0] != "pair" for g, _ in self._pix.values()):
                raise RuntimeError("clone() of an accumulator with dense pixel-pair / slab state is not supported")
            for idx in list(self._pix_pending):
                self._drain_pixpair(idx)
            new.factors = [[t.clone() for t in F] for F in self.factors]
            new.loss = self.loss.clone()
            new._taps_meta = list(self._taps_meta)
            new._gscale = dict(self._gscale)
            new._tap_index = dict(self._tap_index)
            new._pix = {idx: (geo, buf.clone()) for idx, (geo, buf) in self._pix.items()}
            new._pix_pending, new._gslabs = {}, {}
            new._side = self._side
        return new

    def merge_(self, other: "KronAccumulator") -> bool:
        self._fold_lanes()
        other._fold_lanes()
        if not self._raw_compatible(other):
            return False
        skip = set(other._pix_inputs)
        mine = [t for i, F in enumerate(self.factors) for j, t in enumerate(F) if not (j == 1 and i in skip)] + [self.loss]
        theirs = [t for i, F in enumerate(other.factors) for j, t in enumerate(F) if not (j == 1 and i in skip)] + [other.loss]
        side = self._side or other._side
        if side is None or not self.lag_join or not self.loss.is_cuda:
            self._join_side()
            other._join_side()
            torch._foreach_add_(mine, theirs)
            self._push_adopted(self._adopt_pix_inputs(other))
        else:
            self._side = side
            main = torch.cuda.current_stream(self.loss.device)
            if self._side_done is not None:
                main.wait_event(self._side_done)
            todo = self._adopt_pix_inputs(other)
            side.wait_stream(main)
            with torch.cuda.stream(side):
                torch._foreach_add_(mine, theirs)
                self._push_adopted(todo)
            for t in theirs:
                t.record_stream(side)
            for items in other._pix_inputs.values():
                for _, _, t, _ in items:
                    t.record_stream(side)
            self._side_done = torch.cuda.Event()
            self._side_done.record(side)
        return True

    def _join_side(self):
        if self._side is not None:
            torch.cuda.current_stream(self._side.device).wait_stream(self._side)
            self._side_done = None
            self._side_older = []

    def _flush_g_slabs(self, only=None):
        K = get_kernels()
        if self._gslabs:
            self._join_side()
        for idx in ([only] if only is not None else list(self._gslabs)):
            buf, n, L, alpha = self._gslabs.pop(idx)
            K.gram_slabs_reduce(buf, n, L, alpha, self.factors[idx][0], upper_only=True)

    def _note_grad_scales(self, tape, scales):
        for idx, tap in enumerate(tape.taps):
            s_new = scales.get(tap.name)
            s_old = self._gscale.get(idx)
            if s_old is None:
                if s_new is not None:
                    self._gscale[idx] = s_new
            elif s_new is None or (s_new is not s_old and not torch.equal(s_new, s_old)):
                raise RuntimeError(f"{tap.name}: the BatchNorm scale changed during the fit (model not in eval mode?)")

    def _apply_grad_scales(self):
        self._join_side()
        for idx, s_ in self._gscale.items():
            G = self.factors[idx][0]
            G.mul_(s_.reshape(-1, 1) * s_.reshape(1, -1))
        self._gscale = {}

    def tensors(self) -> list[torch.Tensor]:
        self._fold_lanes()
        self._resolve_pix_inputs()
        self._flush_pixgrams()
        self._flush_g_slabs()
        self._apply_grad_scales()
        out = CurvatureExchange([t for F in self.factors for t in F] + [self.loss])
        out.owner = self
        return out

    def finalize(self):
        K = get_kernels()
        rt = math.sqrt(float(self.backend.factor))
        self._fold_lanes()
        self._resolve_pix_inputs()
        self._flush_pixgrams()
        self._flush_g_slabs()
        self._join_side()
        items, done = [], []
        for idx, ((G, A), (has_bias, native)) in enumerate(zip(self.factors, self._taps_meta)):
            s_ = self._gscale.get(idx)
            if s_ is not None:
                s_ = s_.detach().to(torch.float32).reshape(-1).contiguous()
            items.append((G, None, s_, 0, 1))
            if native is not None and native[1] > 1:
                A_out = torch.empty_like(A)
                items.append((A, A_out, None, native[0], native[1]))
                A = A_out
            else:
                items.append((A, None, None, 0, 1))
            done.append((G, A, has_bias))
        K.finalize_factors(items)
        self._gscale = {}
        kfacs = []
        for G, A, has_bias in done:
            if G.numel() == 1 and A.numel() == 1 and not has_bias:
                kfacs.append([G * A])
            else:
                kfacs.append([G, A])
            if has_bias:
                kfacs.append([G * rt])
        self.factors = None
        if self._out_dtype != torch.float32:
            return _HipCurvatureMixin._cast((self.loss[0], HipKron(kfacs)), self._out_dtype)
        return self.loss[0], HipKron(kfacs)


class HipGGN(_HipCurvatureMixin, GGNInterface):

    def __init__(self, model, likelihood, last_layer=False, subnetwork_indices=None,
                 dict_key_x="input_ids", dict_key_y="labels", stochastic=False, num_samples=1):
        if stochastic and int(num_samples) < 1:
            raise ValueError("num_samples must be >= 1")
        super().__init__(model, likelihood, last_layer, subnetwork_indices, dict_key_x, dict_key_y,
                         stochastic=stochastic, num_samples=num_samples)
        self.generator = None

    _kron_seeds = _HipCurvatureMixin._ggn_seeds

    def kron_accumulator(self, N: int, **kwargs) -> KronAccumulator:
        acc = KronAccumulator(self, N, kwargs.get("kfac_approx", "expand"), kwargs.get("overlap", True))
        if kwargs.get("coalesce") is not None:
            acc.coalesce = bool(kwargs["coalesce"])
        return acc

    def kron(self, x, y, N, **kwargs):
        twin, dt = self._twin()
        if twin is not None:
            return self._cast(twin.kron(self._to32(x), self._to32(y), N, **kwargs), dt)
        kfac_approx = kwargs.get("kfac_approx", "expand")
        return self._kron_impl(x, y, N, self._ggn_seeds, None, kfac_approx)

    def diag(self, x, y, **kwargs):
        twin, dt = self._twin()
        if twin is not None:
            return self._cast(twin.diag(self._to32(x), self._to32(y), **kwargs), dt)
        out = self._diag_impl(x, y, self._ggn_seeds, 1.0)
        if out is None:
            return super().diag(x, y, **kwargs)
        return out

    def full(self, x, y, **kwargs):
        twin, dt = self._twin()
        if twin is not None:
            return self._cast(twin.full(self._to32(x), self._to32(y), **kwargs), dt)
        K = get_kernels()
        if self.last_layer and self.subnetwork_indices is None and not self.stochastic:
            f, tape, _ = self._forward(x)
            phi = tape.taps[0].a.to(torch.float32).contiguous()
            B, C = f.shape
            has_bias = tape.taps[0].has_bias
            loss = torch.zeros(1, dtype=torch.float32, device=f.device)
            if self.likelihood == "regression":
                K.sq_err_sum(f, y.reshape(B, C).to(torch.float32).contiguous(), self.factor, loss)
                probs = None
            else:
                K.softmax_hess_sqrt(f, y.reshape(B).to(torch.int64).contiguous(), loss)
                probs = torch.softmax(f, dim=-1).contiguous()
            P = tape.n_params
            H = torch.zeros(P, P, dtype=torch.float32, device=f.device)
            K.ll_ggn_full(phi, probs, has_bias, 1.0, H)
            tape.release()
            return loss[0], H
        if not self._supported():
            return super().full(x, y, **kwargs)
        loss = None

        def seeds_fn(f):
            nonlocal loss
            loss = torch.zeros(1, dtype=torch.float32, device=f.device)
            return self._ggn_seeds(f, y, loss)[0]

        try:
            Z, _ = self._rows(x, seeds_fn)
        except Unserved:
            return super().full(x, y, **kwargs)
        return loss[0], self._full_from_rows(Z, 1.0)

    def last_layer_jacobians(self, x, enable_backprop: bool = False):
        twin, dt = self._twin()
        if twin is not None and not enable_backprop:
            return self._cast(twin.last_layer_jacobians(self._to32(x), False), dt)
        if enable_backprop or not self._supported() or not self.last_layer:
            return super().last_layer_jacobians(x, enable_backprop)
        try:
            f, tape, _ = self._forward(x)
        except NotImplementedError:
            return super().last_layer_jacobians(x, enable_backprop)
        tap = tape.taps[0]
        phi = tap.a.reshape(tap.a.shape[0], -1).contiguous()
        tap.a = None
        C = f.shape[1]
        Js = get_kernels().jac_last_layer(phi, C, tap.module.bias is not None)
        return Js, f

    def jacobians(self, x, enable_backprop: bool = False):
        twin, dt = self._twin()
        if twin is not None and not enable_backprop:
            return self._cast(twin.jacobians(self._to32(x), False), dt)
        if enable_backprop or self.last_layer or not self._supported():
            return super().jacobians(x, enable_backprop)

        def seeds_fn(f):
            B, C = f.shape
            eye = torch.eye(C, dtype=f.dtype, device=f.device)
            return eye[:, None, :].expand(C, B, C).contiguous()

        try:
            Js, f = self._rows(x, seeds_fn)
        except Unserved:
            return super().jacobians(x, enable_backprop)
        if self.subnetwork_indices is not None:
            Js = Js[:, :, self.subnetwork_indices]
        return Js, f


class HipEF(_HipCurvatureMixin, EFInterface):

    def _ef_seeds(self, f, y, loss):
        return self._ef_seed(f, y, loss), 1.0

    _kron_seeds = _ef_seeds

    def kron_accumulator(self, N: int, **kwargs) -> KronAccumulator:
        acc = KronAccumulator(self, N, kwargs.get("kfac_approx", "expand"))
        if kwargs.get("coalesce") is not None:
            acc.coalesce = bool(kwargs["coalesce"])
        return acc

    def kron(self, x, y, N, **kwargs):
        twin, dt = self._twin()
        if twin is not None:
            return self._cast(twin.kron(self._to32(x), self._to32(y), N, **kwargs), dt)
        return self._kron_impl(x, y, N, self._ef_seeds, None, kwargs.get("kfac_approx", "expand"))

    def diag(self, x, y, **kwargs):
        twin, dt = self._twin()
        if twin is not None:
            return self._cast(twin.diag(self._to32(x), self._to32(y), **kwargs), dt)
        out = self._diag_impl(x, y, self._ef_seeds, float(self.factor))
        if out is None:
            return super().diag(x, y, **kwargs)
        return out

# ... 41 lines not shown
```

### laplace_amd/csrc/lk_gram.hip

```cpp
#include <cstdlib>

#include "lk_common.h"
#include "lk_split16.h"

namespace lk {

enum { MODE_TN = 0, MODE_NT = 1, MODE_CONV = 2, MODE_XCORR = 3, MODE_TNP = 4, MODE_NTB = 5 };
__host__ __device__ constexpr bool is_nt(int mode) { return mode == MODE_NT || mode == MODE_NTB; }
#ifdef LK_GRAM_TRACE
__device__ long long g_gram_trace[5];
#endif
constexpr int MAX_SEG = 16;

struct GramGeom {
  const float* x;
  int64_t K;
  int n;
  int64_t ldx;
  const int* tiles;
  int ldc;
  int slab_accumulate;
  int L, Lp;
  int seg_nb;
  int nseg;
// ... 891 lines not shown
#pragma unroll
    for (int a = 0; a < 3; ++a)
#pragma unroll
      for (int b = 0; b < 3; ++b) {
        const int dy = a - 1, dx = b - 1;
        if (!(dy >= dy_lo && dy <= dy_hi && dx >= dx_lo && dx <= dx_hi)) continue;
        const int d = a * 3 + b, e = (dy + Dy + 1) * 3 + (dx + Dx + 1);
        const float4 t = acc[a][b];
        const float v4[4] = {alpha * t.x, alpha * t.y, alpha * t.z, alpha * t.w};
        float4* dst = reinterpret_cast<float4*>(A + (int64_t)(d * Cin + ci) * n + e * Cin + cj);
        float4 o = *dst;
        o.x += v4[0], o.y += v4[1], o.z += v4[2], o.w += v4[3];
        *dst = o;
        if (MIRROR && h != 0) {
#pragma unroll
          for (int j = 0; j < 4; ++j) A[(int64_t)(e * Cin + cj + j) * n + d * Cin + ci] += v4[j];
        }
      }
  }
}

struct ShiftCorrPlan {
  size_t off_Rf, off_strips, off_pix, off_ws, ws_each, total;
};
static ShiftCorrPlan shiftcorr_plan(int64_t B, int64_t H, int64_t W, int64_t Cin) {
  ShiftCorrPlan p;
  size_t off = 0;
  p.off_Rf = off; off += align_up((size_t)Cin * 13 * Cin * 4, 256);
  p.off_strips = off;
  p.off_pix = off + (size_t)4 * Cin * 25 * Cin * 4;
  off += align_up((size_t)8 * Cin * 25 * Cin * 4, 256);
  size_t w = make_plan_rect(Cin, 13 * Cin, B * H * W).ws_bytes;
  const int64_t strip_len = H > W ? H : W;
  size_t w2 = make_plan_rect(Cin, 25 * Cin, B * strip_len).ws_bytes * 8;
  p.ws_each = w > w2 ? w : w2;
  p.off_ws = off; off += align_up(p.ws_each, 256);
  p.total = off;
  return p;
}

__global__ __launch_bounds__(256) void nchw_to_nhwc_kernel(const float* __restrict__ src, int C, int HW,
                                                           float* __restrict__ dst) {
  __shared__ float tile[64][65];
  const int b = blockIdx.z;
  const int c0 = blockIdx.y * 64, p0 = blockIdx.x * 64;
  const int tx = threadIdx.x & 63, ty = threadIdx.x >> 6;
  const float* s = src + (int64_t)b * C * HW;
  float* d = dst + (int64_t)b * C * HW;
  for (int i = ty; i < 64; i += 4) {
    const int c = c0 + i, p = p0 + tx;
    tile[i][tx] = (c < C && p < HW) ? s[(int64_t)c * HW + p] : 0.f;
  }
  __syncthreads();
  for (int i = ty; i < 64; i += 4) {
    const int p = p0 + i, c = c0 + tx;
    if (c < C && p < HW) d[(int64_t)p * C + c] = tile[tx][i];
  }
}

__global__ __launch_bounds__(256) void symmetrize_kernel(float* __restrict__ Cm, int n) {
  __shared__ float tile[64][65];
  const int bi = blockIdx.y, bj = blockIdx.x;
  if (bi > bj) return;
  const int tx = threadIdx.x & 63, ty = threadIdx.x >> 6;
  for (int i = ty; i < 64; i += 4) {
    const int r = bi * 64 + i, c = bj * 64 + tx;
    tile[i][tx] = (r < n && c < n) ? Cm[(int64_t)r * n + c] : 0.f;
  }
  __syncthreads();
  for (int i = ty; i < 64; i += 4) {
    const int r = bj * 64 + i, c = bi * 64 + tx;
    if (r < n && c < n && r > c) Cm[(int64_t)r * n + c] = tile[tx][i];
  }
}

__global__ __launch_bounds__(256) void permute_sym_kernel(const float* __restrict__ src, int Cin, int KK,
                                                          float* __restrict__ dst, int accumulate) {
  const int n = Cin * KK;
  const int64_t total = (int64_t)n * n;
  for (int64_t idx = (int64_t)blockIdx.x * 256 + threadIdx.x; idx < total; idx += (int64_t)gridDim.x * 256) {
    const int r = (int)(idx / n), c = (int)(idx - (int64_t)r * n);
    const int ci = r / KK, d = r - ci * KK;
    const int cj = c / KK, e = c - cj * KK;
    const float v = src[(int64_t)(d * Cin + ci) * n + (e * Cin + cj)];
    dst[idx] = accumulate ? dst[idx] + v : v;
  }
}

struct FinDesc {
  const float* src;
  float* dst;
  const float* scale;
  int n, cin, kk, blk0;
};
constexpr int FIN_MAX = 48;
struct FinBatch {
  int count, nblk;
  FinDesc d[FIN_MAX];
};
constexpr int FIN_PERM_ELEMS = 4096;

__global__ __launch_bounds__(256) void finalize_factors_kernel(const FinBatch fb) {
  __shared__ float tile[64][65];
  int k = 0;
  for (int i = 1; i < fb.count; ++i)
    if ((int)blockIdx.x >= fb.d[i].blk0) k = i;
  const FinDesc& D = fb.d[k];
  const int local = (int)blockIdx.x - D.blk0;
  const int n = D.n;
  if (D.kk <= 1) {
    int bj = (int)((sqrtf(8.f * (float)local + 1.f) - 1.f) * 0.5f);
    while ((bj + 1) * (bj + 2) / 2 <= local) ++bj;
    while (bj * (bj + 1) / 2 > local) --bj;
    const int bi = local - bj * (bj + 1) / 2;
    float* Cm = D.dst ? D.dst : const_cast<float*>(D.src);
    const int tx = threadIdx.x & 63, ty = threadIdx.x >> 6;
    for (int i = ty; i < 64; i += 4) {
      const int r = bi * 64 + i, c = bj * 64 + tx;
      float v = (r < n && c < n) ? D.src[(int64_t)r * n + c] : 0.f;
      if (D.scale && r < n && c < n) v *= D.scale[r] * D.scale[c];
      tile[i][tx] = v;
    }
    __syncthreads();
    if (D.scale || D.dst) {
      for (int i = ty; i < 64; i += 4) {
        const int r = bi * 64 + i, c = bj * 64 + tx;
        if (r < n && c < n && r <= c) Cm[(int64_t)r * n + c] = tile[i][tx];
      }
    }
    for (int i = ty; i < 64; i += 4) {
      const int r = bj * 64 + i, c = bi * 64 + tx;
      if (r < n && c < n && r > c) Cm[(int64_t)r * n + c] = tile[tx][i];
    }
    return;
  }
  const int Cin = D.cin, KK = D.kk;
  const int64_t total = (int64_t)n * n;
  const int64_t e0 = (int64_t)local * FIN_PERM_ELEMS;
  for (int j = threadIdx.x; j < FIN_PERM_ELEMS; j += 256) {
    const int64_t idx = e0 + j;
    if (idx >= total) break;
    const int r = (int)(idx / n), c = (int)(idx - (int64_t)r * n);
    const int ci = r / KK, d = r - ci * KK;
    const int cj = c / KK, e = c - cj * KK;
    int rs = d * Cin + ci, cs = e * Cin + cj;
    if (rs > cs) {
      const int t = rs;
      rs = cs, cs = t;
    }
    D.dst[idx] = D.src[(int64_t)rs * n + cs];
  }
}

}

using namespace lk;

#ifdef LK_GRAM_TRACE
extern "C" int lk_gram_trace_read(long long* out) {
  return hipMemcpyFromSymbol(out, HIP_SYMBOL(g_gram_trace), 5 * sizeof(long long)) == hipSuccess ? 0 : -1;
}
#endif

extern "C" size_t lk_gram_workspace_bytes(int64_t n, int64_t K) {
  if (n <= 0) return 0;
  return make_plan(n, K < 1 ? 1 : K).ws_bytes;
}

extern "C" size_t lk_gram_nt_workspace_bytes(int64_t nb_total, int64_t n, int64_t L) {
  if (n <= 0 || L <= 0) return 0;
  const int BK = nt_chunk_rows(n, L);
  const int64_t Lp = (L + BK - 1) / BK * BK;
  return make_plan(n, nb_total < 1 ? Lp : nb_total * Lp, L).ws_bytes;
}

extern "C" int lk_gram_launch_variant(int entry, int64_t n, int64_t K, int64_t L, int vec4_ok, unsigned flags, int* out) {
  if (!out || entry < LK_GRAM_TN || entry > LK_GRAM_XCORR_STRIPS) return -1;
  if (n < 1 || K < 0 || n >= (1 << 30)) return -1;
  GramPlan p;
  int mode;
  bool vec4;
  unsigned fl = flags;
  if (entry == LK_GRAM_TN) {
    p = make_plan(n, K);
    mode = MODE_TN;
    vec4 = vec4_rule(n, vec4_ok != 0);
  } else if (entry == LK_GRAM_NT) {
    if (L < 1 || L >= (1 << 30)) return -1;
    const int BK = nt_chunk_rows(n, L);
    const int64_t Lp = (L + BK - 1) / BK * BK;
    p = make_plan(n, K * Lp, L);
    vec4 = vec4_rule(L, vec4_ok != 0);
    mode = nt_mode_rule(vec4, BK);
  } else if (entry == LK_GRAM_CONV) {
    if (K >= (1ll << 31) - 64) return -1;
    p = make_plan(n, K);
    mode = MODE_CONV;
    vec4 = vec4_ok != 0;
  } else {
    if (K < 1 || K >= (1ll << 31) - 64 || 25 * n >= (1 << 24)) return -1;
    p = make_plan_rect(n, (entry == LK_GRAM_XCORR_FULL ? 13 : 25) * n, K);
    mode = MODE_XCORR;
    vec4 = vec4_rule(n, vec4_ok != 0);
    fl = 0;
  }
  const bool persist = (fl & LK_GRAM_SLABS_PERSIST) != 0;
  const bool direct = direct_rule(p, fl);
  out[0] = mode, out[1] = vec4 ? 4 : 1, out[2] = p.cfg, out[3] = p.T, out[4] = p.BK, out[5] = p.npairs;
  out[6] = p.nchunks, out[7] = p.nsplit, out[8] = p.chunks_per_split;
  out[9] = persist ? 2 : (direct ? 1 : 0);
  out[10] = (!direct && two_level_rule(p.nslabs)) ? 1 : 0;
  out[11] = p.rpw;
  return 0;
}

extern "C" int lk_gram_slabs_reduce_f32(float* slabs, size_t slabs_bytes, int64_t n, int64_t L_nt, float alpha, float* C,
                                        unsigned flags, void* stream) {
  LK_REQUIRE(slabs && C && n > 0 && n < (1 << 30), "lk_gram_slabs_reduce_f32: bad arguments");
  const GramPlan p = make_plan(n, 1, L_nt);
  const size_t slab_bytes = (size_t)p.npairs * p.T * p.T * sizeof(float);
  const int nslabs = (int)(slabs_bytes / slab_bytes);
  LK_REQUIRE(nslabs >= 1, "lk_gram_slabs_reduce_f32: buffer smaller than one slab");
  return reduce_slabs(p, slabs, nslabs, alpha, C, (int)n, flags, (hipStream_t)stream);
}

extern "C" int lk_gram_tn_f32(const float* X, int64_t K, int64_t n, int64_t ldx, float alpha, float* C,
                              unsigned flags, void* ws, size_t ws_bytes, void* stream) {
  LK_REQUIRE(X && C && K >= 0 && n >= 0 && ldx >= n, "lk_gram_tn_f32: bad arguments");
  LK_REQUIRE(n < (1 << 30), "lk_gram_tn_f32: n too large");
  GramGeom g{};
  g.x = X; g.K = K; g.n = (int)n; g.ldx = ldx;
  const bool vec4 = vec4_rule(n, ldx % 4 == 0 && aligned16(X));
  return launch_gram<MODE_TN>(g, vec4, alpha, C, flags, ws, ws_bytes, (hipStream_t)stream);
}

extern "C" int lk_gram_nt_seg_f32(const float* const* segs, int64_t nseg, int64_t nb, int64_t n, int64_t L,
                                  float alpha, float* C, unsigned flags, void* ws, size_t ws_bytes, void* stream) {
  LK_REQUIRE(segs && C && nseg >= 1 && nseg <= MAX_SEG && nb >= 0 && n >= 0 && L >= 1,
             "lk_gram_nt_seg_f32: bad arguments (at most 16 segments)");
  LK_REQUIRE(n < (1 << 30) && L < (1 << 30), "lk_gram_nt_seg_f32: dims too large");
  const int BK = nt_chunk_rows(n, L);
  GramGeom g{};
  g.n = (int)n; g.L = (int)L;
  g.Lp = (int)((L + BK - 1) / BK * BK);
  g.seg_nb = (int)(nb > 0 ? nb : 1);
  g.nseg = (int)nseg;
  g.K = nseg * nb * g.Lp;
  bool all_aligned = true;
  for (int i = 0; i < nseg; ++i) {
    LK_REQUIRE(segs[i] != nullptr, "lk_gram_nt_seg_f32: null segment");
    g.seg[i] = segs[i];
    all_aligned = all_aligned && aligned16(segs[i]);
  }
  const bool vec4 = vec4_rule(L, all_aligned);
  g.x = segs[0];
  if (nt_mode_rule(vec4, BK) == MODE_NTB) return launch_gram<MODE_NTB>(g, vec4, alpha, C, flags, ws, ws_bytes, (hipStream_t)stream);
  return launch_gram<MODE_NT>(g, vec4, alpha, C, flags, ws, ws_bytes, (hipStream_t)stream);
}

extern "C" int lk_gram_nt_f32(const float* X, int64_t nb, int64_t n, int64_t L, float alpha, float* C,
                              unsigned flags, void* ws, size_t ws_bytes, void* stream) {
  LK_REQUIRE(X != nullptr, "lk_gram_nt_f32: bad arguments");
  const float* segs[1] = {X};
  return lk_gram_nt_seg_f32(segs, 1, nb, n, L, alpha, C, flags, ws, ws_bytes, stream);
}

extern "C" int lk_gram_conv_nhwc_f32(const float* x, int64_t B, int64_t H, int64_t W, int64_t Cin, int kh, int kw,
                                     int sh, int sw, int ph, int pw, int dh, int dw, float alpha, float* C,
                                     unsigned flags, void* ws, size_t ws_bytes, void* stream) {
  LK_REQUIRE(x && C && B >= 0 && H > 0 && W > 0 && Cin > 0 && kh > 0 && kw > 0 && sh > 0 && sw > 0 && dh > 0 && dw > 0,
             "lk_gram_conv_nhwc_f32: bad arguments");
  const int64_t OH = (H + 2 * ph - dh * (kh - 1) - 1) / sh + 1;
  const int64_t OW = (W + 2 * pw - dw * (kw - 1) - 1) / sw + 1;
  LK_REQUIRE(OH > 0 && OW > 0, "lk_gram_conv_nhwc_f32: empty output");
  GramGeom g{};
  g.x = x; g.n = (int)(Cin * kh * kw); g.K = B * OH * OW;
  g.H = (int)H; g.W = (int)W; g.Cin = (int)Cin; g.OH = (int)OH; g.OW = (int)OW; g.kw = kw;
  g.sh = sh; g.sw = sw; g.ph = ph; g.pw = pw; g.dh = dh; g.dw = dw;
  LK_REQUIRE(g.K < (1ll << 31) - 64, "lk_gram_conv_nhwc_f32: B*OH*OW must be < 2^31");
  g.div_ohw = make_fastdiv((int)(OH * OW));
  g.div_ow = make_fastdiv((int)OW);
  const bool vec4 = vec4_rule(Cin, aligned16(x));
  return launch_gram<MODE_CONV>(g, vec4, alpha, C, flags, ws, ws_bytes, (hipStream_t)stream);
}

extern "C" int lk_nchw_to_nhwc_f32(const float* src, int64_t B, int64_t C, int64_t HW, float* dst, void* stream) {
  LK_REQUIRE(src && dst && B >= 0 && C > 0 && HW > 0, "lk_nchw_to_nhwc_f32: bad arguments");
  if (B == 0) return LK_OK;
  LK_REQUIRE(B < 65536, "lk_nchw_to_nhwc_f32: batch too large for grid.z");
  LK_REQUIRE(C <= 65535 * 64 && HW < (1ll << 31) - 64, "lk_nchw_to_nhwc_f32: C too large for grid.y (C <= %d) or HW >= 2^31 - 64", 65535 * 64);
  dim3 grid((unsigned)((HW + 63) / 64), (unsigned)((C + 63) / 64), (unsigned)B);
  hipLaunchKernelGGL(nchw_to_nhwc_kernel, grid, dim3(256), 0, (hipStream_t)stream, src, (int)C, (int)HW, dst);
  return check_launch("nchw_to_nhwc_kernel");
}

extern "C" int lk_symmetrize_f32(float* C, int64_t n, void* stream) {
  LK_REQUIRE(C && n >= 0, "lk_symmetrize_f32: bad arguments");
  LK_REQUIRE(n <= 65535 * 64, "lk_symmetrize_f32: n too large for grid.y (n <= %d)", 65535 * 64);
  if (n == 0) return LK_OK;
  const unsigned nb = (unsigned)((n + 63) / 64);
  hipLaunchKernelGGL(symmetrize_kernel, dim3(nb, nb), dim3(256), 0, (hipStream_t)stream, C, (int)n);
  return check_launch("symmetrize_kernel");
}

extern "C" int lk_permute_sym_f32(const float* src, int64_t Cin, int64_t KK, float* dst, int accumulate,
                                  void* stream) {
  LK_REQUIRE(src && dst && Cin > 0 && KK > 0 && src != dst, "lk_permute_sym_f32: bad arguments");
  LK_REQUIRE(Cin < (1ll << 24) && KK < (1ll << 24) && Cin * KK < (1ll << 24), "lk_permute_sym_f32: Cin * KK must be < 2^24");
  const int64_t n = Cin * KK;
  const int64_t total = n * n;
  int64_t blocks = (total + 255) / 256;
  if (blocks > 8192) blocks = 8192;
  hipLaunchKernelGGL(permute_sym_kernel, dim3((unsigned)blocks), dim3(256), 0, (hipStream_t)stream, src, (int)Cin,
                     (int)KK, dst, accumulate);
  return check_launch("permute_sym_kernel");
}

extern "C" int lk_finalize_factors_f32(int64_t count, const float* const* src, float* const* dst, const float* const* scale,
                                       const int64_t* n, const int64_t* cin, const int64_t* kk, void* stream) {
  LK_REQUIRE(count >= 0 && (count == 0 || (src && dst && scale && n && cin && kk)), "lk_finalize_factors_f32: bad arguments");
  int64_t i = 0;
  while (i < count) {
    FinBatch fb;
    fb.count = 0, fb.nblk = 0;
    for (; i < count && fb.count < FIN_MAX; ++i) {
      LK_REQUIRE(src[i] && n[i] >= 0 && n[i] < (1ll << 24), "lk_finalize_factors_f32: bad factor");
      if (n[i] == 0) continue;
      FinDesc& D = fb.d[fb.count];
      D.src = src[i], D.dst = dst[i], D.scale = scale[i];
      D.n = (int)n[i], D.cin = (int)cin[i], D.kk = (int)kk[i], D.blk0 = fb.nblk;
      int64_t blocks;
      if (kk[i] > 1) {
        LK_REQUIRE(dst[i] && dst[i] != src[i] && cin[i] * kk[i] == n[i] && !scale[i],
                   "lk_finalize_factors_f32: a permuted factor needs dst != src, n = cin * kk and no scale");
        blocks = (n[i] * n[i] + FIN_PERM_ELEMS - 1) / FIN_PERM_ELEMS;
      } else {
        const int64_t nb = (n[i] + 63) / 64;
        blocks = nb * (nb + 1) / 2;
      }
      if ((int64_t)fb.nblk + blocks >= (1ll << 30)) break;
      fb.nblk += (int)blocks;
      ++fb.count;
    }
    if (fb.count == 0) continue;
    hipLaunchKernelGGL(finalize_factors_kernel, dim3((unsigned)fb.nblk), dim3(256), 0, (hipStream_t)stream, fb);
    if (int rc = check_launch("finalize_factors_kernel")) return rc;
  }
  return LK_OK;
}

extern "C" int lk_conv3x3_pixpair_plan(int64_t H, int64_t W, int64_t Cin, int64_t* tile, int64_t* n_tiles,
                                       int64_t* n_blocks) {
  LK_REQUIRE(H >= 1 && W >= 1 && Cin >= 64 && Cin % 64 == 0 && tile && n_tiles && n_blocks,
             "lk_conv3x3_pixpair_plan: needs Cin % 64 == 0");
  LK_REQUIRE(H < (1ll << 31) && W < (1ll << 31) && Cin < (1ll << 31) && H * W < (1ll << 31) && H * W * Cin < (1ll << 31),
             "lk_conv3x3_pixpair_plan: problem too large");
  int64_t nb = 0;
  for (int64_t y = 0; y < H; ++y)
    for (int64_t x = 0; x < W; ++x)
      for (int h = 0; h < 13; ++h) {
        const int64_t y2 = y + kHalfDy[h], x2 = x + kHalfDx[h];
        nb += (y2 >= 0 && y2 < H && x2 >= 0 && x2 < W);
      }
  const int64_t T = Cin % 128 == 0 ? 128 : 64, tpp = Cin / T;
  LK_REQUIRE(nb * Cin * Cin < (1ll << 31) && H * W * Cin < (1ll << 31), "lk_conv3x3_pixpair_plan: problem too large");
  *tile = T;
  *n_blocks = nb;
  *n_tiles = nb * tpp * tpp;
  return LK_OK;
}

extern "C" int lk_conv3x3_pixpair_tables(int64_t H, int64_t W, int64_t Cin, int32_t* tiles, int32_t* slots) {
  int64_t T, nt, nb;
  if (int rc = lk_conv3x3_pixpair_plan(H, W, Cin, &T, &nt, &nb)) return rc;
  LK_REQUIRE(tiles && slots, "lk_conv3x3_pixpair_tables: null table");
  const int64_t tpp = Cin / T;
  int64_t slot = 0, k = 0;
  for (int64_t y = 0; y < H; ++y)
    for (int64_t x = 0; x < W; ++x)
      for (int h = 0; h < 13; ++h) {
        const int64_t q = y * W + x, y2 = y + kHalfDy[h], x2 = x + kHalfDx[h];
        if (!(y2 >= 0 && y2 < H && x2 >= 0 && x2 < W)) {
          slots[q * 13 + h] = -1;
          continue;
        }
        const int64_t q2 = y2 * W + x2;
        slots[q * 13 + h] = (int32_t)slot;
        for (int64_t ta = 0; ta < tpp; ++ta)
          for (int64_t tb = 0; tb < tpp; ++tb) {
            tiles[3 * k] = (int32_t)(q * Cin + ta * T);
            tiles[3 * k + 1] = (int32_t)(q2 * Cin + tb * T);
            tiles[3 * k + 2] = (int32_t)(slot * Cin * Cin + ta * T * Cin + tb * T);
            ++k;
          }
        ++slot;
      }
  return LK_OK;
}

extern "C" int lk_conv3x3_pixpair_accumulate_f32(const float* x, int64_t B, int64_t H, int64_t W, int64_t Cin, float alpha,
                                                 float* blocks, const int32_t* tiles_dev, int64_t n_tiles, void* stream) {
  LK_REQUIRE(x && blocks && tiles_dev && B >= 0 && n_tiles >= 0, "lk_conv3x3_pixpair_accumulate_f32: bad arguments");
  int64_t T, nt, nb;
  if (int rc = lk_conv3x3_pixpair_plan(H, W, Cin, &T, &nt, &nb)) return rc;
  LK_REQUIRE(nt == n_tiles, "lk_conv3x3_pixpair_accumulate_f32: table does not match the geometry");
  LK_REQUIRE(aligned16(x) && n_tiles < (1ll << 31), "lk_conv3x3_pixpair_accumulate_f32: unaligned input / too many tiles");
  if (B == 0 || n_tiles == 0) return LK_OK;
  GramGeom g{};
  g.x = x; g.K = B; g.n = (int)(H * W * Cin); g.ldx = H * W * Cin;
  g.tiles = tiles_dev; g.ldc = (int)Cin;
  const int cfg = T == 64 ? CFG_SMALL16 : CFG_BIG;
  const int nchunks = (int)((B + cfg_bk(cfg) - 1) / cfg_bk(cfg));
  const size_t lds = cfg_lds_bytes(cfg, true);
  dim3 grid((unsigned)n_tiles, 1), block(256);
  hipStream_t st = (hipStream_t)stream;
  if (cfg == CFG_SMALL16) {
    hipLaunchKernelGGL((gram_kernel<MODE_TNP, 4, CFG_SMALL16>), grid, block, lds, st, g, (float*)nullptr, 1, (int)n_tiles,
                       nchunks, nchunks, blocks, alpha);
  } else {
    if (!allow_big_lds((const void*)gram_kernel<MODE_TNP, 4, CFG_BIG>, lds)) return LK_ELAUNCH;
    hipLaunchKernelGGL((gram_kernel<MODE_TNP, 4, CFG_BIG>), grid, block, lds, st, g, (float*)nullptr, 1, (int)n_tiles, nchunks,
                       nchunks, blocks, alpha);
  }
  return check_launch("gram_kernel<TNP>");
}

extern "C" int lk_conv3x3_pixpair_assemble2_f32(const float* blocks, const float* blocks2, const int32_t* slots_dev, int64_t H,
                                                int64_t W, int64_t Cin, float alpha, float* A, int upper_only, void* stream) {
  LK_REQUIRE(blocks && slots_dev && A && H >= 1 && W >= 1 && Cin >= 1 && 9 * Cin < (1ll << 24) && H * W < (1ll << 24),
             "lk_conv3x3_pixpair_assemble_f32: bad arguments");
  LK_REQUIRE(Cin % 4 == 0 && ((reinterpret_cast<uintptr_t>(blocks) | reinterpret_cast<uintptr_t>(blocks2) | reinterpret_cast<uintptr_t>(A)) & 15) == 0,
             "lk_conv3x3_pixpair_assemble_f32: Cin % 4 == 0 and 16-byte aligned buffers");
  const int64_t total4 = 13 * Cin * Cin / 4;
  int64_t nblk = (total4 + 63) / 64;
  if (nblk > 65536) nblk = 65536;
  int P = 1;
  while (P < 4 && nblk * 64 * P < (1 << 18) && H * W >= 64 * P) P *= 2;
  if (upper_only)
    hipLaunchKernelGGL(pixpair_assemble_kernel<false>, dim3((unsigned)nblk), dim3(64 * P), 0, (hipStream_t)stream, blocks, blocks2,
                       slots_dev, (int)H, (int)W, (int)Cin, alpha, A);
  else
    hipLaunchKernelGGL(pixpair_assemble_kernel<true>, dim3((unsigned)nblk), dim3(64 * P), 0, (hipStream_t)stream, blocks, blocks2,
                       slots_dev, (int)H, (int)W, (int)Cin, alpha, A);
  return check_launch("pixpair_assemble_kernel");
}

extern "C" int lk_conv3x3_pixpair_assemble_f32(const float* blocks, const int32_t* slots_dev, int64_t H, int64_t W,
                                               int64_t Cin, float alpha, float* A, void* stream) {
  return lk_conv3x3_pixpair_assemble2_f32(blocks, nullptr, slots_dev, H, W, Cin, alpha, A, 0, stream);
}

extern "C" int lk_conv3x3_pixgram_assemble_f32(const float* Cp, int64_t H, int64_t W, int64_t Cin, float alpha, float* A,
                                               void* stream) {
  LK_REQUIRE(Cp && A && H >= 1 && W >= 1 && Cin >= 1 && H * W * Cin < (1ll << 31) && 9 * Cin < (1ll << 24),
             "lk_conv3x3_pixgram_assemble_f32: bad arguments");
  const int64_t total = 81 * Cin * Cin;
  int64_t blocks = (total + 255) / 256;
  if (blocks > 16384) blocks = 16384;
  hipLaunchKernelGGL(pixgram_assemble_kernel, dim3((unsigned)blocks), dim3(256), 0, (hipStream_t)stream, Cp, (int)H, (int)W,
                     (int)Cin, alpha, A);
  return check_launch("pixgram_assemble_kernel");
}

extern "C" size_t lk_conv3x3_shiftcorr_workspace_bytes(int64_t B, int64_t H, int64_t W, int64_t Cin) {
  if (B < 0 || H < 1 || W < 1 || Cin < 1) return 0;
  return shiftcorr_plan(B < 1 ? 1 : B, H, W, Cin).total;
}

extern "C" int lk_conv3x3_shiftcorr_f32(const float* x, int64_t B, int64_t H, int64_t W, int64_t Cin, float alpha,
                                        float* C, void* ws, size_t ws_bytes, void* stream_) {
  LK_REQUIRE(x && C && B >= 0 && H >= 2 && W >= 2 && Cin >= 1, "lk_conv3x3_shiftcorr_f32: bad arguments");
  LK_REQUIRE(B * H * W < (1ll << 31) - 64 && 25 * Cin < (1 << 24), "lk_conv3x3_shiftcorr_f32: problem too large");
  if (B == 0) return LK_OK;
  hipStream_t stream = (hipStream_t)stream_;
  const ShiftCorrPlan p = shiftcorr_plan(B, H, W, Cin);
  if (ws == nullptr || ws_bytes < p.total) {
    set_error("lk_conv3x3_shiftcorr_f32: workspace too small (%zu < %zu bytes)", ws_bytes, p.total);
    return LK_EWORKSPACE;
  }
  char* base = static_cast<char*>(ws);
  float* Rf = reinterpret_cast<float*>(base + p.off_Rf);
  float* strips = reinterpret_cast<float*>(base + p.off_strips);
  float* pix = reinterpret_cast<float*>(base + p.off_pix);
  void* gws = base + p.off_ws;
  if (hipMemsetAsync(base, 0, p.off_ws, stream) != hipSuccess) {
    set_error("lk_conv3x3_shiftcorr_f32: hipMemsetAsync failed");
    return LK_ELAUNCH;
  }
  signed char hy[13], hx[13], ay[25], ax[25];
  int k = 0;
  for (int dx = 0; dx <= 2; ++dx) { hy[k] = 0; hx[k] = (signed char)dx; ++k; }
  for (int dy = 1; dy <= 2; ++dy)
    for (int dx = -2; dx <= 2; ++dx) { hy[k] = (signed char)dy; hx[k] = (signed char)dx; ++k; }
  for (int t = 0; t < 25; ++t) { ay[t] = (signed char)(t / 5 - 2); ax[t] = (signed char)(t % 5 - 2); }
  const int h = (int)H, w = (int)W, c = (int)Cin;
  const int64_t blk = Cin * 25 * Cin;
  const Region full = {0, 0, h, w};
  int rc = launch_xcorr(x, B, h, w, c, &full, 1, hy, hx, 13, Rf, gws, p.ws_each, stream);
  if (rc) return rc;
  const Region regs[8] = {{0, 0, 1, w},     {h - 1, 0, 1, w},     {0, 0, h, 1},     {0, w - 1, h, 1},
                          {0, 0, 1, 1},     {0, w - 1, 1, 1},     {h - 1, 0, 1, 1}, {h - 1, w - 1, 1, 1}};
  if (pix != strips + 4 * blk) {
    set_error("lk_conv3x3_shiftcorr_f32: internal layout error");
    return LK_EINVAL;
  }
  rc = launch_xcorr(x, B, h, w, c, regs, 8, ay, ax, 25, strips, gws, p.ws_each, stream);
  if (rc) return rc;
  const int64_t total = 81 * Cin * Cin;
  int64_t blocks = (total + 255) / 256;
  if (blocks > 8192) blocks = 8192;
  hipLaunchKernelGGL(shiftcorr_assemble_kernel, dim3((unsigned)blocks), dim3(256), 0, stream, Rf, strips, pix, c, alpha,
                     C);
  return check_launch("shiftcorr_assemble_kernel");
}
```

### laplace_amd/csrc/lk_sweep16.hip

```cpp
#include "lk_common.h"
#include "lk_split16.h"

namespace lk {

typedef short s16x4 __attribute__((ext_vector_type(4)));

template <bool MFLOAT>
__global__ __launch_bounds__(256) void vjp_nhwc_split_kernel(
    const float* __restrict__ g, const unsigned* __restrict__ g_amax, const _Float16* __restrict__ g2h,
    const _Float16* __restrict__ g2l, const int* __restrict__ g2_sexp, const void* __restrict__ m,
    const unsigned* __restrict__ m_amax, const float* __restrict__ scale, const unsigned* __restrict__ scale_amax, int C,
    int S, int64_t per8, _Float16* __restrict__ oh, _Float16* __restrict__ ol, int* __restrict__ out_sexp) {
  float bound = 0.f;
  if (g) bound += __uint_as_float(g_amax[0]);
  const VjpScale vs = vjp_bound_scale<true>(bound, g2h != nullptr, g2_sexp, m != nullptr, MFLOAT, m_amax, scale != nullptr, scale_amax);
  const float sc_out = exp2i_sat(vs.so);
  if (blockIdx.x == 0 && threadIdx.x == 0) out_sexp[0] = vs.so;
  const int64_t e8 = (int64_t)blockIdx.x * 256 + threadIdx.x;
  if (e8 >= per8) return;
  float mult[8];
#pragma unroll
  for (int j = 0; j < 8; ++j) mult[j] = sc_out;
  if (m) {
    if (MFLOAT) vjp_mult8_times(mult, reinterpret_cast<const float*>(m) + 8 * e8);
    else vjp_mult8_mask(mult, reinterpret_cast<const uint2*>(m)[e8]);
  }
  if (scale) vjp_mult8_times(mult, scale + (int)((e8 * 8) % C));
#pragma unroll 2
  for (int s = 0; s < S; ++s) {
    const int64_t i8 = (int64_t)s * per8 + e8;
    float v[8];
    if (g) {
      const float4 a = reinterpret_cast<const float4*>(g)[2 * i8], b = reinterpret_cast<const float4*>(g)[2 * i8 + 1];
      v[0] = a.x, v[1] = a.y, v[2] = a.z, v[3] = a.w, v[4] = b.x, v[5] = b.y, v[6] = b.z, v[7] = b.w;
    } else {
#pragma unroll
      for (int j = 0; j < 8; ++j) v[j] = 0.f;
    }
    if (g2h) vjp_add8(v, reinterpret_cast<const f16x8*>(g2h)[i8], reinterpret_cast<const f16x8*>(g2l)[i8], vs.inv2);
    f16x8 h, l;
    unsigned vmax = 0;
    vjp_chunk8(v, mult, vmax, h, l);
    reinterpret_cast<f16x8*>(oh)[i8] = h;
    reinterpret_cast<f16x8*>(ol)[i8] = l;
  }
}

constexpr int BN_ACT_IT = 4;
__global__ __launch_bounds__(256) void bn_act_fwd_nhwc_kernel(
    const float* __restrict__ x, const unsigned* __restrict__ x_amax, int x_namax, const float* __restrict__ x_mul,
    const float* __restrict__ x_add, const float* __restrict__ scale, const float* __restrict__ shift,
    const unsigned* __restrict__ scale_amax, const unsigned* __restrict__ shift_amax, const float* __restrict__ addend,
    const float* __restrict__ addend_bound, int addend_nbound, int act, int C, int64_t per8, float* __restrict__ y,
    unsigned char* __restrict__ mask, _Float16* __restrict__ yh, _Float16* __restrict__ yl, int* __restrict__ y_sexp,
    float* __restrict__ y_bound, unsigned* __restrict__ y_amax) {
  const int n = blockIdx.y;
  float bx = __uint_as_float(x_amax[n < x_namax ? n : x_namax - 1]);
  if (x_mul) bx *= x_mul[0];
  if (x_add) bx += x_add[0];
  float bound = bx * __uint_as_float(scale_amax[0]) + __uint_as_float(shift_amax[0]);
  if (addend) bound += addend_bound[n < addend_nbound ? n : addend_nbound - 1];
  if (act == 2) bound = 1.f;
  const int so = scale_exp_for(bound);
  if (blockIdx.x == 0 && threadIdx.x == 0) {
    y_sexp[n] = so;
    y_bound[n] = bound;
  }
  const float sc_out = exp2i_sat(so);
  unsigned vmax = 0;
  for (int64_t i8 = (int64_t)blockIdx.x * (256 * BN_ACT_IT) + threadIdx.x, it = 0; it < BN_ACT_IT && i8 < per8; ++it, i8 += 256) {
    const int64_t e8 = (int64_t)n * per8 + i8;
    const int c0 = (int)((i8 * 8) % C);
    const float4 s0 = *reinterpret_cast<const float4*>(scale + c0), s1 = *reinterpret_cast<const float4*>(scale + c0 + 4);
    const float4 t0 = *reinterpret_cast<const float4*>(shift + c0), t1 = *reinterpret_cast<const float4*>(shift + c0 + 4);
    const float4 a = reinterpret_cast<const float4*>(x)[2 * e8], b = reinterpret_cast<const float4*>(x)[2 * e8 + 1];
    float v[8] = {a.x * s0.x + t0.x, a.y * s0.y + t0.y, a.z * s0.z + t0.z, a.w * s0.w + t0.w,
                  b.x * s1.x + t1.x, b.y * s1.y + t1.y, b.z * s1.z + t1.z, b.w * s1.w + t1.w};
    if (addend) {
      const float4 p = reinterpret_cast<const float4*>(addend)[2 * e8], q = reinterpret_cast<const float4*>(addend)[2 * e8 + 1];
      v[0] += p.x, v[1] += p.y, v[2] += p.z, v[3] += p.w, v[4] += q.x, v[5] += q.y, v[6] += q.z, v[7] += q.w;
    }
    if (act == 1) {
      unsigned m0 = 0, m1 = 0;
#pragma unroll
      for (int j = 0; j < 8; ++j) {
        v[j] = fmaxf(v[j], 0.f);
        if (v[j] > 0.f) (j < 4 ? m0 : m1) |= 1u << (8 * (j & 3));
      }
      if (mask) reinterpret_cast<uint2*>(mask)[e8] = make_uint2(m0, m1);
    } else if (act == 2) {
#pragma unroll
      for (int j = 0; j < 8; ++j) v[j] = tanhf(v[j]);
    }
    reinterpret_cast<float4*>(y)[2 * e8] = make_float4(v[0], v[1], v[2], v[3]);
    reinterpret_cast<float4*>(y)[2 * e8 + 1] = make_float4(v[4], v[5], v[6], v[7]);
#pragma unroll
    for (int j = 0; j < 8; ++j) vmax = max(vmax, __float_as_uint(v[j]) & 0x7fffffffu);
    if (yh) {
      f16x8 h, l;
#pragma unroll
      for (int j = 0; j < 8; ++j) split2_at(v[j] * sc_out, h, l, j);
      reinterpret_cast<f16x8*>(yh)[e8] = h;
      reinterpret_cast<f16x8*>(yl)[e8] = l;
    }
  }
  if (y_amax) {
    __shared__ unsigned wave_max[4];
#pragma unroll
    for (int off = 32; off > 0; off >>= 1) vmax = max(vmax, (unsigned)__shfl_xor((int)vmax, off, 64));
    if ((threadIdx.x & 63) == 0) wave_max[threadIdx.x >> 6] = vmax;
    __syncthreads();
    if (threadIdx.x == 0) {
      vmax = max(max(wave_max[0], wave_max[1]), max(wave_max[2], wave_max[3]));
      if (vmax) atomicMax(y_amax + n, vmax);
    }
  }
}

__global__ __launch_bounds__(256) void unsplit_transpose_kernel(const _Float16* __restrict__ xh,
                                                                const _Float16* __restrict__ xl,
                                                                const int* __restrict__ sexp, int S, int B, int L, int C,
                                                                float* __restrict__ out) {
  __shared__ float tile[32][33];
  const int n = blockIdx.z, s = n / B, b = n - s * B;
  const int c0 = blockIdx.x * 32, l0 = blockIdx.y * 32;
  const float inv = exp2i_sat(-sexp[0]);
  const int tx = threadIdx.x & 31, ty = threadIdx.x >> 5;
  for (int i = ty; i < 32; i += 8) {
    const int l = l0 + i, c = c0 + tx;
    float v = 0.f;
    if (l < L && c < C) {
      const int64_t e = ((int64_t)n * L + l) * C + c;
      v = ((float)xh[e] + (float)xl[e]) * inv;
    }
    tile[i][tx] = v;
  }
  __syncthreads();
  for (int i = ty; i < 32; i += 8) {
    const int c = c0 + i, l = l0 + tx;
    if (l < L && c < C) out[(((int64_t)b * S + s) * C + c) * L + l] = tile[tx][i];
  }
}

template <int NB, int BKR, int KW>
struct Gram16Cfg {
  static constexpr int PITCH = NB * 2;
  static constexpr int PLANE = BKR * PITCH;
  static constexpr int PANEL = 2 * PLANE;
  static constexpr int STAGE = 2 * PANEL;
  static constexpr int SLOTS = BKR * NB / 8;
  static constexpr int LD = SLOTS / 256;
  static constexpr int TW = KW == 4 ? NB / 32 : NB / 64;
  static_assert(SLOTS % 256 == 0, "whole instructions");
};

template <int NB>
__device__ __forceinline__ int gram16_swz(int row) {
  return NB == 64 ? ((row >> 1) & 1) : (row & 3);
}

__device__ __forceinline__ float gram16_unscale_add(float old, float v, float alpha, float inv) {
  return __builtin_fmaf(alpha, (v * inv) * inv, old);
}

typedef __attribute__((address_space(3))) void lds_void16;
typedef __attribute__((address_space(1))) const void gbl_void16;

struct Gram16Tnp {
  const int* tiles;
  int ldc;
  const int* sexp;
  float alpha;
  float* blocks;
};

template <int NB, int BKR, int KW, bool TNP>
__global__ __launch_bounds__(256) void gram16_kernel(const _Float16* __restrict__ Xh, const _Float16* __restrict__ Xl,
                                                     int64_t R, int64_t C, int64_t rows_per_split,
                                                     const _Float16* __restrict__ zero16, float* __restrict__ ws,
                                                     int nbc, const Gram16Tnp tp) {
  using G = Gram16Cfg<NB, BKR, KW>;
  constexpr int TW = G::TW;
  extern __shared__ __attribute__((aligned(16))) char smem[];
  const int tid = threadIdx.x, lane = tid & 63, wave = tid >> 6;
  int bi = 0, bj = 0;
  int64_t colA = 0, colB = 0, out_off = 0;
  if constexpr (TNP) {
    const int nblk = gridDim.x;
    int bid = blockIdx.x;
    bid = xcd_tile_order(bid, nblk);
    colA = tp.tiles[3 * bid], colB = tp.tiles[3 * bid + 1], out_off = tp.tiles[3 * bid + 2];
  } else {
    int p = blockIdx.x;
    while (p >= nbc - bi) p -= nbc - bi, ++bi;
    bj = bi + p;
    colA = (int64_t)bi * NB, colB = (int64_t)bj * NB;
  }
  const bool diag = !TNP && bi == bj;
  const int64_t r0 = TNP ? 0 : (int64_t)blockIdx.y * rows_per_split;
  const int64_t r1 = TNP ? R : (r0 + rows_per_split < R ? r0 + rows_per_split : R);
  const int nstage = r1 > r0 ? (int)((r1 - r0 + BKR - 1) / BKR) : 0;

  int st_row[G::LD], st_col[G::LD];
#pragma unroll
  for (int i = 0; i < G::LD; ++i) {
    const int slot = i * 256 + tid;
    const int row = slot / (NB / 8), pq = slot % (NB / 8);
    st_row[i] = row;
    st_col[i] = (pq ^ (gram16_swz<NB>(row) << 2)) * 8;
  }
  auto stage = [&](int s, int buf) {
    char* base = smem + buf * G::STAGE;
    const int64_t rb = r0 + (int64_t)s * BKR;
#pragma unroll
    for (int pnl = 0; pnl < 2; ++pnl) {
      if (pnl == 1 && diag) break;
      const int64_t cb = pnl ? colB : colA;
#pragma unroll
      for (int i = 0; i < G::LD; ++i) {
        const int64_t r = rb + st_row[i];
        const bool ok = r < r1;
        const int64_t e = r * C + cb + st_col[i];
        char* d = base + pnl * G::PANEL + (i * 256 + wave * 64) * 16;
        __builtin_amdgcn_global_load_lds((gbl_void16*)(ok ? Xh + e : zero16), (lds_void16*)d, 16, 0, 0);
        __builtin_amdgcn_global_load_lds((gbl_void16*)(ok ? Xl + e : zero16), (lds_void16*)(d + G::PLANE), 16, 0, 0);
      }
    }
  };

  const int wr = KW == 4 ? 0 : (wave >> 1), wc = KW == 4 ? 0 : (wave & 1);
  const bool wave_active = !(KW == 1 && diag && wr > wc);
  f32x16 acc[TW][TW];
#pragma unroll
  for (int a = 0; a < TW; ++a)
#pragma unroll
    for (int b = 0; b < TW; ++b)
#pragma unroll
      for (int r = 0; r < 16; ++r) acc[a][b][r] = 0.f;

  const int grp = lane >> 4, r16 = lane & 15;
  const int f_row = (grp >> 1) * 8 + (r16 >> 2);
  const int f_col = (grp & 1) * 16 + (r16 & 3) * 4;

  auto load_frag = [&](const char* plane, int k16, int col0) -> f16x8 {
    s16x4 v[2];
#pragma unroll
    for (int j = 0; j < 2; ++j) {
      const int row = k16 * 16 + f_row + j * 4;
      const int col = col0 + f_col;
      const int off = row * G::PITCH + (((col >> 5) ^ gram16_swz<NB>(row)) << 6) + (col & 31) * 2;
      const unsigned addr = (unsigned)(uintptr_t)(__attribute__((address_space(3))) const char*)(plane + off);
      asm volatile("ds_read_b64_tr_b16 %0, %1" : "=v"(v[j]) : "v"(addr));
    }
    const f16x4 f0 = __builtin_bit_cast(f16x4, v[0]), f1 = __builtin_bit_cast(f16x4, v[1]);
    return f16x8{f0[0], f0[1], f0[2], f0[3], f1[0], f1[1], f1[2], f1[3]};
  };

  constexpr int NOLD = TNP ? (KW == 4 ? TW * TW * 4 : TW * TW * 16) : 1;
  float old[NOLD];
  if constexpr (TNP) {
    const int lr_ = lane & 31, lh_ = lane >> 5;
    if (KW == 4) {
#pragma unroll
      for (int i = 0; i < NOLD; ++i) {
        const int e = tid + 256 * i, t = e >> 10, a = t / TW, b = t % TW, row = (e >> 5) & 31, col = e & 31;
        old[i] = tp.blocks[out_off + (int64_t)(a * 32 + row) * tp.ldc + b * 32 + col];
      }
    } else {
#pragma unroll
      for (int a = 0; a < TW; ++a)
#pragma unroll
        for (int b = 0; b < TW; ++b)
#pragma unroll
          for (int r = 0; r < 16; ++r) {
            const int row = wr * 64 + a * 32 + (r & 3) + 8 * (r >> 2) + 4 * lh_;
            const int col = wc * 64 + b * 32 + lr_;
            old[(a * TW + b) * 16 + r] = tp.blocks[out_off + (int64_t)row * tp.ldc + col];
          }
    }
  }
  if (nstage > 0) stage(0, 0);
  for (int s = 0; s < nstage; ++s) {
    const int buf = s & 1;
    __builtin_amdgcn_s_waitcnt(0x0f70);
    __syncthreads();
    if (s + 1 < nstage) stage(s + 1, buf ^ 1);
    if (!wave_active) continue;
    const char* pa = smem + buf * G::STAGE;
    const char* pb = diag ? pa : pa + G::PANEL;
#pragma unroll
    for (int kk = 0; kk < (KW == 4 ? 1 : BKR / 16); ++kk) {
      const int k16 = KW == 4 ? wave : kk;
      f16x8 ah[TW], al[TW], bh[TW], bl[TW];
#pragma unroll
      for (int a = 0; a < TW; ++a) {
        ah[a] = load_frag(pa, k16, wr * 64 + a * 32);
        al[a] = load_frag(pa + G::PLANE, k16, wr * 64 + a * 32);
      }
#pragma unroll
      for (int b = 0; b < TW; ++b) {
        bh[b] = load_frag(pb, k16, wc * 64 + b * 32);
        bl[b] = load_frag(pb + G::PLANE, k16, wc * 64 + b * 32);
      }
      if constexpr (TW == 2)
        asm volatile("s_waitcnt lgkmcnt(0)" : "+v"(ah[0]), "+v"(al[0]), "+v"(bh[0]), "+v"(bl[0]), "+v"(ah[1]), "+v"(al[1]), "+v"(bh[1]), "+v"(bl[1]));
      else
        asm volatile("s_waitcnt lgkmcnt(0)" : "+v"(ah[0]), "+v"(al[0]), "+v"(bh[0]), "+v"(bl[0]));
#pragma unroll
      for (int a = 0; a < TW; ++a)
#pragma unroll
        for (int b = 0; b < TW; ++b) {
          if (diag && wr == wc && a > b) continue;
          f32x16 c = acc[a][b];
          c = __builtin_amdgcn_mfma_f32_32x32x16_f16(al[a], bh[b], c, 0, 0, 0);
          c = __builtin_amdgcn_mfma_f32_32x32x16_f16(ah[a], bl[b], c, 0, 0, 0);
          c = __builtin_amdgcn_mfma_f32_32x32x16_f16(ah[a], bh[b], c, 0, 0, 0);
          acc[a][b] = c;
        }
    }
  }

  const int lr = lane & 31, lh = lane >> 5;
  float* blk = TNP ? nullptr : ws + ((int64_t)blockIdx.y * gridDim.x + blockIdx.x) * (NB * NB);
  if (KW == 4) {
    __syncthreads();
    float* red = reinterpret_cast<float*>(smem);
#pragma unroll
    for (int a = 0; a < TW; ++a)
#pragma unroll
      for (int b = 0; b < TW; ++b) {
        if (!TNP && a > b) continue;
#pragma unroll
        for (int r = 0; r < 16; ++r) {
          const int row = (r & 3) + 8 * (r >> 2) + 4 * lh;
          red[((wave * TW + a) * TW + b) * 1024 + row * 32 + lr] = acc[a][b][r];
        }
      }
    __syncthreads();
    float inv = 0.f;
    if constexpr (TNP) inv = exp2i_sat(-tp.sexp[0]);
#pragma unroll
    for (int i = 0; i < TW * TW * 4; ++i) {
      const int e = tid + 256 * i;
      const int t = e >> 10, a = t / TW, b = t % TW;
      if (!TNP && a > b) continue;
      const float v = ((red[e] + red[TW * TW * 1024 + e]) + red[2 * TW * TW * 1024 + e]) + red[3 * TW * TW * 1024 + e];
      const int row = (e >> 5) & 31, col = e & 31;
      if constexpr (TNP) tp.blocks[out_off + (int64_t)(a * 32 + row) * tp.ldc + b * 32 + col] = gram16_unscale_add(old[i], v, tp.alpha, inv);
      else blk[(a * 32 + row) * NB + b * 32 + col] = v;
    }
    return;
  }
  if (!wave_active) return;
  float inv = 0.f;
  if constexpr (TNP) inv = exp2i_sat(-tp.sexp[0]);
#pragma unroll
  for (int a = 0; a < TW; ++a)
#pragma unroll
    for (int b = 0; b < TW; ++b) {
      if (diag && wr == wc && a > b) continue;
#pragma unroll
      for (int r = 0; r < 16; ++r) {
        const int row = wr * 64 + a * 32 + (r & 3) + 8 * (r >> 2) + 4 * lh;
        const int col = wc * 64 + b * 32 + lr;
        if constexpr (TNP)
          tp.blocks[out_off + (int64_t)row * tp.ldc + col] = gram16_unscale_add(old[(a * TW + b) * 16 + r], acc[a][b][r], tp.alpha, inv);
        else blk[row * NB + col] = acc[a][b][r];
      }
    }
}

template <int NB>
__global__ __launch_bounds__(256) void gram16_reduce4_kernel(const float* __restrict__ ws, int nparts, int npairs, int nbc,
                                                             int C, const int* __restrict__ sexp, float alpha,
                                                             float* __restrict__ Gm) {
  __shared__ float4 red[4][64];
  const int pair = blockIdx.y;
  int bi = 0, bj = 0;
  {
    int p = pair;
    while (p >= nbc - bi) p -= nbc - bi, ++bi;
    bj = bi + p;
  }
  const int q = threadIdx.x & 63, g = threadIdx.x >> 6;
  const int e = blockIdx.x * 256 + 4 * q;
  const int row = e / NB, col = e % NB;
  const bool live = !(bi == bj && (row >> 5) > (col >> 5));
  float4 s = make_float4(0.f, 0.f, 0.f, 0.f);
  const float* src = ws + (int64_t)pair * (NB * NB) + e;
  const int64_t pstride = (int64_t)npairs * (NB * NB);
  int p = g;
  for (; live && p + 28 < nparts; p += 32) {
    float4 v[8];
#pragma unroll
    for (int u = 0; u < 8; ++u) v[u] = *reinterpret_cast<const float4*>(src + (int64_t)(p + 4 * u) * pstride);
#pragma unroll
    for (int u = 0; u < 8; ++u) s.x += v[u].x, s.y += v[u].y, s.z += v[u].z, s.w += v[u].w;
  }
  for (; live && p < nparts; p += 4) {
    const float4 v = *reinterpret_cast<const float4*>(src + (int64_t)p * pstride);
    s.x += v.x, s.y += v.y, s.z += v.z, s.w += v.w;
  }
  red[g][q] = s;
  __syncthreads();
  if (g == 0 && live) {
    float4 t = red[0][q];
#pragma unroll
    for (int k = 1; k < 4; ++k) t.x += red[k][q].x, t.y += red[k][q].y, t.z += red[k][q].z, t.w += red[k][q].w;
    const float inv = exp2i_sat(-sexp[0]);
    float4* dst = reinterpret_cast<float4*>(Gm + (int64_t)(bi * NB + row) * C + bj * NB + col);
    float4 o = *dst;
    o.x = gram16_unscale_add(o.x, t.x, alpha, inv), o.y = gram16_unscale_add(o.y, t.y, alpha, inv);
    o.z = gram16_unscale_add(o.z, t.z, alpha, inv), o.w = gram16_unscale_add(o.w, t.w, alpha, inv);
// ... 4 lines not shown
}

using namespace lk;

extern "C" int lk_vjp_nhwc_split_f16x2(const float* g, const unsigned* g_amax, const void* g2_h, const void* g2_l,
                                       const int* g2_sexp, const void* m, int m_is_float, const unsigned* m_amax,
                                       const float* scale, const unsigned* scale_amax, int64_t C, int64_t S, int64_t per,
                                       void* out_h, void* out_l, int* out_sexp, void* stream) {
  LK_REQUIRE((g || g2_h) && out_h && out_l && out_sexp && S >= 0 && per >= 0, "lk_vjp_nhwc_split_f16x2: bad arguments");
  LK_REQUIRE(!g || g_amax, "lk_vjp_nhwc_split_f16x2: the fp32 addend needs its max|.| word");
  LK_REQUIRE(!g2_h || (g2_l && g2_sexp), "lk_vjp_nhwc_split_f16x2: incomplete split addend");
  LK_REQUIRE(!scale || (scale_amax && C >= 8 && C % 8 == 0 && per % C == 0), "lk_vjp_nhwc_split_f16x2: scale needs C % 8 == 0");
  LK_REQUIRE(per % 8 == 0 && S < (1 << 30), "lk_vjp_nhwc_split_f16x2: per % 8 == 0");
  if (S == 0 || per == 0) return LK_OK;
  const int64_t per8 = per / 8, nb = (per8 + 255) / 256;
  LK_REQUIRE(nb < (1ll << 31), "lk_vjp_nhwc_split_f16x2: grid too large");
  hipStream_t st = (hipStream_t)stream;
  if (m && m_is_float)
    hipLaunchKernelGGL(vjp_nhwc_split_kernel<true>, dim3((unsigned)nb), dim3(256), 0, st, g, g_amax, (const _Float16*)g2_h,
                       (const _Float16*)g2_l, g2_sexp, m, m_amax, scale, scale_amax, (int)(scale ? C : 8), (int)S, per8,
                       (_Float16*)out_h, (_Float16*)out_l, out_sexp);
  else
    hipLaunchKernelGGL(vjp_nhwc_split_kernel<false>, dim3((unsigned)nb), dim3(256), 0, st, g, g_amax, (const _Float16*)g2_h,
                       (const _Float16*)g2_l, g2_sexp, m, m_amax, scale, scale_amax, (int)(scale ? C : 8), (int)S, per8,
                       (_Float16*)out_h, (_Float16*)out_l, out_sexp);
  return check_launch("vjp_nhwc_split_kernel");
}

extern "C" int lk_bn_act_fwd_nhwc_f16x2(const float* x, const unsigned* x_amax, int64_t x_namax, const float* x_mul,
                                       const float* x_add, const float* scale, const float* shift,
                                       const unsigned* scale_amax, const unsigned* shift_amax, const float* addend,
                                       const float* addend_bound, int64_t addend_nbound, int act, int64_t C, int64_t N,
                                       int64_t per, float* y, void* mask, void* y_h, void* y_l, int* y_sexp, float* y_bound,
                                       unsigned* y_amax, void* stream) {
  LK_REQUIRE(x && x_amax && scale && shift && scale_amax && shift_amax && y && y_sexp && y_bound && per >= 0 && N >= 0,
             "lk_bn_act_fwd_nhwc_f16x2: null pointer");
  LK_REQUIRE(C >= 8 && C % 8 == 0 && per % C == 0 && act >= 0 && act <= 2, "lk_bn_act_fwd_nhwc_f16x2: C % 8 == 0, act in 0..2");
  LK_REQUIRE(x_namax == 1 || x_namax == N, "lk_bn_act_fwd_nhwc_f16x2: x_amax has 1 or N words");
  LK_REQUIRE(!addend || (addend_bound && (addend_nbound == 1 || addend_nbound == N)),
             "lk_bn_act_fwd_nhwc_f16x2: the addend needs its bound (1 or N words)");
  LK_REQUIRE((y_h == nullptr) == (y_l == nullptr), "lk_bn_act_fwd_nhwc_f16x2: both planes or none");
  LK_REQUIRE(N <= 65535, "lk_bn_act_fwd_nhwc_f16x2: at most 65535 images");
  if (per == 0 || N == 0) return LK_OK;
  const int64_t per8 = per / 8, nb = (per8 + 256 * BN_ACT_IT - 1) / (256 * BN_ACT_IT);
  LK_REQUIRE(nb < (1ll << 31), "lk_bn_act_fwd_nhwc_f16x2: grid too large");
  hipLaunchKernelGGL(bn_act_fwd_nhwc_kernel, dim3((unsigned)nb, (unsigned)N), dim3(256), 0, (hipStream_t)stream, x, x_amax,
                     (int)x_namax, x_mul, x_add, scale, shift, scale_amax, shift_amax, addend, addend_bound,
                     (int)(addend ? addend_nbound : 1), act, (int)C, per8, y, (unsigned char*)mask, (_Float16*)y_h,
                     (_Float16*)y_l, y_sexp, y_bound, y_amax);
  return check_launch("bn_act_fwd_nhwc_kernel");
}

extern "C" int lk_unsplit_transpose_f32(const void* x_h, const void* x_l, const int* sexp, int64_t S, int64_t B, int64_t L,
                                       int64_t C, float* out, void* stream) {
  LK_REQUIRE(x_h && x_l && sexp && out && S >= 0 && B >= 0 && L >= 0 && C >= 0 && S * B <= 65535,
             "lk_unsplit_transpose_f32: bad arguments (S * B <= 65535)");
  LK_REQUIRE(L <= 65535 * 32ll, "lk_unsplit_transpose_f32: L too large for grid.y (L <= %lld positions)", 65535 * 32ll);
  LK_REQUIRE(C < (1ll << 31) - 32, "lk_unsplit_transpose_f32: C too large (C < 2^31 - 32 channels)");
  if (S * B == 0 || L == 0 || C == 0) return LK_OK;
  hipLaunchKernelGGL(unsplit_transpose_kernel, dim3((unsigned)((C + 31) / 32), (unsigned)((L + 31) / 32), (unsigned)(S * B)),
                     dim3(256), 0, (hipStream_t)stream, (const _Float16*)x_h, (const _Float16*)x_l, sexp, (int)S, (int)B,
                     (int)L, (int)C, out);
  return check_launch("unsplit_transpose_kernel");
}

namespace {
struct Gram16Plan {
  int nb, nbc, npairs, kw, bkr;
  int64_t nsplit, rows_per_split, nparts;
};
Gram16Plan gram16_plan(int64_t R, int64_t C) {
  Gram16Plan p;
  p.nb = C == 64 ? 64 : 128;
  p.kw = C == 64 ? 4 : 1;
  p.bkr = C == 64 ? 64 : 32;
  p.nbc = (int)(C / p.nb);
  p.npairs = p.nbc * (p.nbc + 1) / 2;
  int64_t want = (512 + p.npairs - 1) / p.npairs;
  int64_t stages = (R + p.bkr - 1) / p.bkr;
  int64_t per = (stages + want - 1) / want;
  if (per < 8) per = 8;
  p.rows_per_split = per * p.bkr;
  p.nsplit = (R + p.rows_per_split - 1) / p.rows_per_split;
  if (p.nsplit < 1) p.nsplit = 1;
  p.nparts = p.nsplit;
  return p;
}
}

extern "C" size_t lk_gram_tn_f16x2_workspace_bytes(int64_t R, int64_t C) {
  if (C < 64 || (C != 64 && C % 128)) return 0;
  const Gram16Plan p = gram16_plan(R, C);
  return (size_t)p.nparts * p.npairs * p.nb * p.nb * sizeof(float);
}

extern "C" int lk_gram_tn_f16x2(const void* x_h, const void* x_l, const int* sexp, int64_t R, int64_t C, float alpha,
                                float* Gm, const void* zero16, void* ws, size_t ws_bytes, void* stream) {
  LK_REQUIRE(x_h && x_l && sexp && Gm && zero16 && ws && R >= 0, "lk_gram_tn_f16x2: null pointer");
  LK_REQUIRE(C == 64 || (C >= 128 && C % 128 == 0 && C <= 4096), "lk_gram_tn_f16x2: C must be 64 or a multiple of 128");
  if (R == 0) return LK_OK;
  const Gram16Plan p = gram16_plan(R, C);
  LK_REQUIRE(ws_bytes >= lk_gram_tn_f16x2_workspace_bytes(R, C), "lk_gram_tn_f16x2: workspace too small");
  hipStream_t st = (hipStream_t)stream;
  dim3 grid((unsigned)p.npairs, (unsigned)p.nsplit);
  if (C == 64) {
    using Gc = Gram16Cfg<64, 64, 4>;
    hipLaunchKernelGGL((gram16_kernel<64, 64, 4, false>), grid, dim3(256), 2 * Gc::STAGE, st, (const _Float16*)x_h,
                       (const _Float16*)x_l, R, C, p.rows_per_split, (const _Float16*)zero16, (float*)ws, p.nbc, Gram16Tnp{});
  } else {
    using Gc = Gram16Cfg<128, 32, 1>;
    hipLaunchKernelGGL((gram16_kernel<128, 32, 1, false>), grid, dim3(256), 2 * Gc::STAGE, st, (const _Float16*)x_h,
                       (const _Float16*)x_l, R, C, p.rows_per_split, (const _Float16*)zero16, (float*)ws, p.nbc, Gram16Tnp{});
  }
  int rc = check_launch("gram16_kernel");
  if (rc != LK_OK) return rc;
  dim3 rgrid((unsigned)(p.nb * p.nb / 256), (unsigned)p.npairs);
  if (C == 64)
    hipLaunchKernelGGL(gram16_reduce4_kernel<64>, rgrid, dim3(256), 0, st, (const float*)ws, (int)p.nparts, p.npairs, p.nbc,
                       (int)C, sexp, alpha, Gm);
  else
    hipLaunchKernelGGL(gram16_reduce4_kernel<128>, rgrid, dim3(256), 0, st, (const float*)ws, (int)p.nparts, p.npairs, p.nbc,
                       (int)C, sexp, alpha, Gm);
  return check_launch("gram16_reduce4_kernel");
}

namespace lk {
struct Pix13Args {
  const _Float16 *xh, *xl;
  const _Float16* zero16;
  const int* slots;
  const int* sexp;
  float* blocks;
  float alpha;
  int R, H, W;
};

__device__ __forceinline__ f16x8 pix13_frag(unsigned plane, int lane, int col0) {
  const int grp = lane >> 4, r16 = lane & 15;
  const int f_row = (grp >> 1) * 8 + (r16 >> 2), col = col0 + (grp & 1) * 16 + (r16 & 3) * 4;
  s16x4 v[2];
#pragma unroll
  for (int j = 0; j < 2; ++j) {
    const int row = f_row + j * 4;
    const unsigned off = plane + row * 128 + (((col >> 5) ^ gram16_swz<64>(row)) << 6) + (col & 31) * 2;
    asm volatile("ds_read_b64_tr_b16 %0, %1" : "=v"(v[j]) : "v"(off));
  }
  const f16x4 f0 = __builtin_bit_cast(f16x4, v[0]), f1 = __builtin_bit_cast(f16x4, v[1]);
  return f16x8{f0[0], f0[1], f0[2], f0[3], f1[0], f1[1], f1[2], f1[3]};
}

#ifndef LK_PIX13_ABLATE
#define LK_PIX13_ABLATE 0
#endif
__global__ __launch_bounds__(512) void pixpair13_kernel(const Pix13Args p) {
  constexpr int C = 64, BKR = 16, PLANE = BKR * C * 2, PANEL = 2 * PLANE, STAGE = 13 * PANEL;
  extern __shared__ __attribute__((aligned(16))) char smem[];
  const int tid = threadIdx.x, lane = tid & 63;
  const int wave = __builtin_amdgcn_readfirstlane(tid >> 6);
  int q;
  {
    const int nblk = gridDim.x, bid = blockIdx.x;
    q = xcd_tile_order(bid, nblk);
  }
  auto panel_col = [&](int h) {
    const int dy = h < 3 ? 0 : (h < 8 ? 1 : 2), dx = h < 3 ? h : (h < 8 ? h - 5 : h - 10);
    return (q + dy * p.W + dx) * C;
  };
  unsigned valid = 0;
#pragma unroll
  for (int h = 0; h < 13; ++h)
    if (p.slots[q * 13 + h] >= 0) valid |= 1u << h;
  valid = (unsigned)__builtin_amdgcn_readfirstlane((int)valid);
  const int g = wave >> 2;
  int myslot[7];
#pragma unroll
  for (int i = 0; i < 7; ++i) myslot[i] = g * 7 + i < 13 ? __builtin_amdgcn_readfirstlane(p.slots[q * 13 + (g * 7 + i < 13 ? g * 7 + i : 0)]) : -1;
  const int64_t ld = (int64_t)p.H * p.W * C;
  const int nstage = (p.R + BKR - 1) / BKR;
  const unsigned lds0 = (unsigned)(uintptr_t)(__attribute__((address_space(3))) char*)smem;

  const int s_half = wave & 1, s_pl = wave >> 1;
  const int s_row = s_half * 8 + (lane >> 3);
  const int s_col = ((lane & 7) ^ (gram16_swz<64>(s_row) << 2)) * 8;
  auto stage_one = [&](int s, int buf, int i) {
    const int64_t r = (int64_t)s * BKR + s_row;
    const bool ok = r < p.R;
    const int64_t e0 = r * ld + s_col;
    int pnl = 2 * i + (s_pl >> 1), hl = s_pl & 1;
    if (pnl > 12) pnl = 12;
    const bool live = ok && ((valid >> pnl) & 1u);
    const _Float16* src = live ? (hl ? p.xl : p.xh) + e0 + panel_col(pnl) : p.zero16;
    const unsigned dst = lds0 + buf * STAGE + pnl * PANEL + hl * PLANE + s_half * 1024;
    __builtin_amdgcn_global_load_lds((gbl_void16*)src, (lds_void16*)(uintptr_t)dst, 16, 0, 0);
  };
  auto stage = [&](int s, int buf) {
#pragma unroll
    for (int i = 0; i < 7; ++i) stage_one(s, buf, i);
  };

  const int t_a = (wave >> 1) & 1, t_b = wave & 1;
  f32x16 acc[7];
#pragma unroll
  for (int i = 0; i < 7; ++i)
#pragma unroll
    for (int r = 0; r < 16; ++r) acc[i][r] = 0.f;

  if (nstage > 0) stage(0, 0);
  if (nstage > 1) stage(1, 1);
  int buf = 0;
  for (int s = 0; s < nstage; ++s) {
    if (s + 1 < nstage) asm volatile("s_waitcnt vmcnt(7)\n\ts_barrier" ::: "memory");
    else asm volatile("s_waitcnt vmcnt(0)\n\ts_barrier" ::: "memory");
    const bool more = !(LK_PIX13_ABLATE & 2) && s + 2 < nstage;
    const int nbuf = buf == 0 ? 2 : buf - 1;
    const unsigned base = lds0 + buf * STAGE;
    buf = buf == 2 ? 0 : buf + 1;
    if (LK_PIX13_ABLATE & 4) {
      if (more) stage(s + 2, nbuf);
      continue;
    }
    f16x8 ah = pix13_frag(base, lane, t_a * 32), al = pix13_frag(base + PLANE, lane, t_a * 32);
#pragma unroll
    for (int i = 0; i < 7; ++i) {
      const int h = g * 7 + i;
      if (more) stage_one(s + 2, nbuf, i);
      if (myslot[i] >= 0) {
        f16x8 bh = pix13_frag(base + h * PANEL, lane, t_b * 32), bl = pix13_frag(base + h * PANEL + PLANE, lane, t_b * 32);
        asm volatile("s_waitcnt lgkmcnt(0)" : "+v"(ah), "+v"(al), "+v"(bh), "+v"(bl));
        f32x16 c = acc[i];
        c = __builtin_amdgcn_mfma_f32_32x32x16_f16(al, bh, c, 0, 0, 0);
        c = __builtin_amdgcn_mfma_f32_32x32x16_f16(ah, bl, c, 0, 0, 0);
        c = __builtin_amdgcn_mfma_f32_32x32x16_f16(ah, bh, c, 0, 0, 0);
        acc[i] = c;
      }
      __builtin_amdgcn_sched_barrier(0);
    }
  }

  const float inv = exp2i_sat(-p.sexp[0]);
  const int lr = lane & 31, lh = lane >> 5;
#pragma unroll
  for (int i0 = 0; i0 < 7; i0 += 4) {
    float old[4][16];
#pragma unroll
    for (int i = i0; i < (i0 + 4 < 7 ? i0 + 4 : 7); ++i) {
      if (myslot[i] < 0 || ((LK_PIX13_ABLATE & 1) && p.alpha != 12345.f)) continue;
      const float* blk = p.blocks + (int64_t)myslot[i] * (C * C);
#pragma unroll
      for (int r = 0; r < 16; ++r) old[i - i0][r] = blk[(t_a * 32 + (r & 3) + 8 * (r >> 2) + 4 * lh) * C + t_b * 32 + lr];
    }
#pragma unroll
    for (int i = i0; i < (i0 + 4 < 7 ? i0 + 4 : 7); ++i) {
      if (myslot[i] < 0 || ((LK_PIX13_ABLATE & 1) && p.alpha != 12345.f)) continue;
      float* blk = p.blocks + (int64_t)myslot[i] * (C * C);
#pragma unroll
      for (int r = 0; r < 16; ++r) blk[(t_a * 32 + (r & 3) + 8 * (r >> 2) + 4 * lh) * C + t_b * 32 + lr] =
            gram16_unscale_add(old[i - i0][r], acc[i][r], p.alpha, inv);
    }
  }
}
}

extern "C" int lk_conv3x3_pixpair_accumulate13_f16x2(const void* x_h, const void* x_l, const int* sexp, int64_t B, int64_t H,
                                                     int64_t W, int64_t Cin, float alpha, float* blocks,
                                                     const int32_t* slots_dev, const void* zero16, void* stream) {
  LK_REQUIRE(x_h && x_l && sexp && blocks && slots_dev && zero16 && B >= 0 && H >= 1 && W >= 1,
             "lk_conv3x3_pixpair_accumulate13_f16x2: bad arguments");
  LK_REQUIRE(Cin == 64 && H * W * Cin < (1ll << 31) && B < (1ll << 31) && H * W * 13 * Cin * Cin < (1ll << 31),
             "lk_conv3x3_pixpair_accumulate13_f16x2: needs Cin == 64 (and a map within 2^31 elements)");
  if (B == 0) return LK_OK;
  Pix13Args a;
  a.xh = (const _Float16*)x_h, a.xl = (const _Float16*)x_l, a.zero16 = (const _Float16*)zero16, a.slots = slots_dev, a.sexp = sexp;
  a.blocks = blocks, a.alpha = alpha, a.R = (int)B, a.H = (int)H, a.W = (int)W;
  constexpr int LDS = 3 * 13 * 4096;
  static bool attr_set = false;
  if (!attr_set) {
    (void)hipFuncSetAttribute((const void*)pixpair13_kernel, hipFuncAttributeMaxDynamicSharedMemorySize, LDS);
    attr_set = true;
  }
  hipLaunchKernelGGL(pixpair13_kernel, dim3((unsigned)(H * W)), dim3(512), LDS, (hipStream_t)stream, a);
  return check_launch("pixpair13_kernel");
}

extern "C" int lk_conv3x3_pixpair_accumulate_f16x2(const void* x_h, const void* x_l, const int* sexp, int64_t B, int64_t H,
                                                   int64_t W, int64_t Cin, float alpha, float* blocks,
                                                   const int32_t* tiles_dev, int64_t n_tiles, const void* zero16,
                                                   void* stream) {
  LK_REQUIRE(x_h && x_l && sexp && blocks && tiles_dev && zero16 && B >= 0 && n_tiles >= 0,
             "lk_conv3x3_pixpair_accumulate_f16x2: bad arguments");
  LK_REQUIRE(Cin >= 64 && Cin % 64 == 0 && n_tiles < (1ll << 31) && H * W * Cin < (1ll << 31),
             "lk_conv3x3_pixpair_accumulate_f16x2: needs Cin % 64 == 0");
  if (B == 0 || n_tiles == 0) return LK_OK;
  Gram16Tnp tp;
  tp.tiles = tiles_dev, tp.ldc = (int)Cin, tp.sexp = sexp, tp.alpha = alpha, tp.blocks = blocks;
  hipStream_t st = (hipStream_t)stream;
  const int64_t ld = H * W * Cin;
  if (Cin % 128) {
    using Gc = Gram16Cfg<64, 64, 4>;
    hipLaunchKernelGGL((gram16_kernel<64, 64, 4, true>), dim3((unsigned)n_tiles), dim3(256), 2 * Gc::STAGE, st,
                       (const _Float16*)x_h, (const _Float16*)x_l, B, ld, B, (const _Float16*)zero16, (float*)nullptr, 0, tp);
  } else {
    using Gc = Gram16Cfg<128, 32, 1>;
    hipLaunchKernelGGL((gram16_kernel<128, 32, 1, true>), dim3((unsigned)n_tiles), dim3(256), 2 * Gc::STAGE, st,
                       (const _Float16*)x_h, (const _Float16*)x_l, B, ld, B, (const _Float16*)zero16, (float*)nullptr, 0, tp);
  }
  return check_launch("gram16_kernel<pixel pairs>");
}
```

Baseline: 20990 samples/s.

## Overwrite fresh pixel-pair blocks and batch the finalize assembly into one kernel

Pixel-pair block buffers are now allocated uninitialised. The first accumulate into each buffer uses new overwrite kernel variants that skip reading the old values, which removes both the zero-fill and one read of the buffer. At finalize time, the lane-fold assembly and the factor finalize for conv3x3 pair layers are deferred and run as one batched finish kernel, which also adds a dirty addend where needed. Every path that reads the buffer first has to go through a settle step, otherwise it would see uninitialised memory, so the bookkeeping gets more complex.

```diff
diff --git a/include/laplace_hip.h b/include/laplace_hip.h
--- a/include/laplace_hip.h
+++ b/include/laplace_hip.h
@@ -62,12 +62,21 @@
                                     float alpha, float* A, void* stream);
 int lk_conv3x3_pixpair_assemble2_f32(const float* blocks, const float* blocks2, const int32_t* slots_dev, int64_t H, int64_t W,
                                      int64_t Cin, float alpha, float* A, int upper_only, void* stream);
+int lk_conv3x3_pixpair_finish_f32(int64_t count, const float* const* blocks, const float* const* blocks2,
+                                  const int32_t* const* slots_dev, const int64_t* H, const int64_t* W, const int64_t* Cin,
+                                  const float* alpha, const float* const* addend, float* const* dst, void* stream);
 int lk_conv3x3_pixpair_accumulate_f16x2(const void* x_h, const void* x_l, const int* sexp, int64_t B, int64_t H, int64_t W,
                                         int64_t Cin, float alpha, float* blocks, const int32_t* tiles_dev, int64_t n_tiles,
                                         const void* zero16, void* stream);
 int lk_conv3x3_pixpair_accumulate13_f16x2(const void* x_h, const void* x_l, const int* sexp, int64_t B, int64_t H, int64_t W,
                                           int64_t Cin, float alpha, float* blocks, const int32_t* slots_dev, const void* zero16,
                                           void* stream);
+int lk_conv3x3_pixpair_accumulate_ow_f16x2(const void* x_h, const void* x_l, const int* sexp, int64_t B, int64_t H, int64_t W,
+                                           int64_t Cin, float alpha, float* blocks, const int32_t* tiles_dev, int64_t n_tiles,
+                                           const void* zero16, void* stream);
+int lk_conv3x3_pixpair_accumulate13_ow_f16x2(const void* x_h, const void* x_l, const int* sexp, int64_t B, int64_t H, int64_t W,
+                                             int64_t Cin, float alpha, float* blocks, const int32_t* slots_dev, const void* zero16,
+                                             void* stream);
 
 size_t lk_conv3x3_shiftcorr_workspace_bytes(int64_t B, int64_t H, int64_t W, int64_t Cin);
 int lk_conv3x3_shiftcorr_f32(const float* x, int64_t B, int64_t H, int64_t W, int64_t Cin, float alpha, float* C,
diff --git a/laplace_amd/_lib.py b/laplace_amd/_lib.py
--- a/laplace_amd/_lib.py
+++ b/laplace_amd/_lib.py
@@ -51,8 +51,11 @@
     "lk_conv3x3_pixpair_accumulate_f32": (_int, [_vp, _i64, _i64, _i64, _i64, _f32, _vp, _vp, _i64, _vp]),
     "lk_conv3x3_pixpair_accumulate_f16x2": (_int, [_vp, _vp, _vp, _i64, _i64, _i64, _i64, _f32, _vp, _vp, _i64, _vp, _vp]),
     "lk_conv3x3_pixpair_accumulate13_f16x2": (_int, [_vp, _vp, _vp, _i64, _i64, _i64, _i64, _f32, _vp, _vp, _vp, _vp]),
+    "lk_conv3x3_pixpair_accumulate_ow_f16x2": (_int, [_vp, _vp, _vp, _i64, _i64, _i64, _i64, _f32, _vp, _vp, _i64, _vp, _vp]),
+    "lk_conv3x3_pixpair_accumulate13_ow_f16x2": (_int, [_vp, _vp, _vp, _i64, _i64, _i64, _i64, _f32, _vp, _vp, _vp, _vp]),
     "lk_conv3x3_pixpair_assemble_f32": (_int, [_vp, _vp, _i64, _i64, _i64, _f32, _vp, _vp]),
     "lk_conv3x3_pixpair_assemble2_f32": (_int, [_vp, _vp, _vp, _i64, _i64, _i64, _f32, _vp, _int, _vp]),
+    "lk_conv3x3_pixpair_finish_f32": (_int, [_i64, _vp, _vp, _vp, _vp, _vp, _vp, _vp, _vp, _vp, _vp]),
     "lk_nchw_to_nhwc_f32": (_int, [_vp, _i64, _i64, _i64, _vp, _vp]),
     "lk_absmax_f32": (_int, [_vp, _i64, _vp, _i64, _i64, _vp, _vp]),
     "lk_copy_absmax_f32": (_int, [_vp, _vp, _i64, _vp, _vp]),
@@ -962,7 +965,9 @@
     use_pixpair16 = True
     use_pixpair13 = True
 
-    def pixpair_accumulate_split(self, xs, alpha, blocks, plan):
+    pixpair_overwrite = True
+
+    def pixpair_accumulate_split(self, xs, alpha, blocks, plan, overwrite=False):
         _check(blocks, "blocks")
         _one_scale(xs, "pixpair_accumulate_split")
         B, H, W, Cin = xs.shape
@@ -970,18 +975,19 @@
         assert blocks.numel() == nb * Cin * Cin
         dev = blocks.device
         z = self._zero16(dev)
+        work = (4.0 if overwrite else 8.0) * blocks.numel() + 4.0 * xs.planes[0].numel()
         if Cin == 64 and self.use_pixpair13:
-            self._rc(self._timed("pixpair16", 8.0 * blocks.numel() + 4.0 * xs.planes[0].numel(), dev,
-                                 lambda: self.lib.lk_conv3x3_pixpair_accumulate13_f16x2(
-                                     _ptr(xs.planes[0]), _ptr(xs.planes[1]), _ptr(xs.sexp), B, H, W, Cin, float(alpha), _ptr(blocks),
-                                     ctypes.c_void_p(slots.data_ptr()), _ptr(z), self._stream(dev))),
-                     "lk_conv3x3_pixpair_accumulate13_f16x2")
+            name = "lk_conv3x3_pixpair_accumulate13_ow_f16x2" if overwrite else "lk_conv3x3_pixpair_accumulate13_f16x2"
+            fn = getattr(self.lib, name)
+            self._rc(self._timed("pixpair16", work, dev,
+                                 lambda: fn(_ptr(xs.planes[0]), _ptr(xs.planes[1]), _ptr(xs.sexp), B, H, W, Cin, float(alpha), _ptr(blocks),
+                                            ctypes.c_void_p(slots.data_ptr()), _ptr(z), self._stream(dev))), name)
             return blocks
-        self._rc(self._timed("pixpair16", 8.0 * blocks.numel() + 4.0 * xs.planes[0].numel(), dev,
-                             lambda: self.lib.lk_conv3x3_pixpair_accumulate_f16x2(
-                                 _ptr(xs.planes[0]), _ptr(xs.planes[1]), _ptr(xs.sexp), B, H, W, Cin, float(alpha), _ptr(blocks),
-                                 ctypes.c_void_p(tiles.data_ptr()), tiles.shape[0], _ptr(z), self._stream(dev))),
-                 "lk_conv3x3_pixpair_accumulate_f16x2")
+        name = "lk_conv3x3_pixpair_accumulate_ow_f16x2" if overwrite else "lk_conv3x3_pixpair_accumulate_f16x2"
+        fn = getattr(self.lib, name)
+        self._rc(self._timed("pixpair16", work, dev,
+                             lambda: fn(_ptr(xs.planes[0]), _ptr(xs.planes[1]), _ptr(xs.sexp), B, H, W, Cin, float(alpha), _ptr(blocks),
+                                        ctypes.c_void_p(tiles.data_ptr()), tiles.shape[0], _ptr(z), self._stream(dev))), name)
         return blocks
 
     def pixpair_assemble(self, blocks, plan, H, W, Cin, alpha, A_native, blocks2=None, upper_only=False):
@@ -1027,6 +1033,33 @@
                 scl[i] = sc_.data_ptr()
             ns[i], cins[i], kks[i] = s_.shape[0], int(cin), int(kk)
         self._rc(self.lib.lk_finalize_factors_f32(n, src, dst, scl, ns, cins, kks, self._stream(dev)), "lk_finalize_factors_f32")
+
+    pixpair_finish_max = 48
+
+    def pixpair_finish(self, items):
+        if not items:
+            return
+        n = len(items)
+        assert n <= self.pixpair_finish_max
+        dev = items[0][0].device
+        b1, b2, sl, ad, ds = ((ctypes.c_void_p * n)() for _ in range(5))
+        Hs, Ws, Cs = ((ctypes.c_int64 * n)() for _ in range(3))
+        al = (ctypes.c_float * n)()
+        for i, (blocks, blocks2, plan, H, W, Cin, alpha, addend, dst) in enumerate(items):
+            _check(blocks, "blocks"), _check(dst, "dst")
+            assert blocks.numel() == plan[0] * Cin * Cin and tuple(dst.shape) == (9 * Cin, 9 * Cin) and blocks.device == dev
+            b1[i], sl[i], ds[i] = blocks.data_ptr(), plan[2].data_ptr(), dst.data_ptr()
+            if blocks2 is not None:
+                _check(blocks2, "blocks2")
+                assert blocks2.numel() == blocks.numel()
+                b2[i] = blocks2.data_ptr()
+            if addend is not None:
+                _check(addend, "addend")
+                assert addend.shape == dst.shape
+                ad[i] = addend.data_ptr()
+            Hs[i], Ws[i], Cs[i], al[i] = int(H), int(W), int(Cin), float(alpha)
+        self._rc(self.lib.lk_conv3x3_pixpair_finish_f32(n, b1, b2, sl, Hs, Ws, Cs, al, ad, ds, self._stream(dev)),
+                 "lk_conv3x3_pixpair_finish_f32")
 
     def symmetrize(self, C):
         _check(C, "C")
diff --git a/laplace_amd/backend.py b/laplace_amd/backend.py
--- a/laplace_amd/backend.py
+++ b/laplace_amd/backend.py
@@ -741,6 +741,7 @@
         self.defer_pix = False
         self._pix_inputs = {}
         self._pix_early = set()
+        self._pix_fresh = set()
         self.coalesce = bool(type(self).default_coalesce)
         self._stash, self._stash_n = [], 0
         self._dispatched = 0
@@ -783,6 +784,7 @@
             self.factors.append([G, A])
         self.loss = flat_k[ok:ok + 1]
         self._pix = {}
+        self._pix_fresh = set()
         self._pix_pending = {}
         self._gscale = {}
         self._gslabs = {}
@@ -830,6 +832,7 @@
         if geo[0] != "pair":
             K.pixgram_accumulate(a, alpha, buf)
         elif self.pix_group <= 1:
+            self._pix_settle(idx)
             K.pixpair_accumulate(a, alpha, buf, geo[4])
         else:
             self._push_pix_input(idx, geo, alpha, a, nhwc=False)
@@ -927,8 +930,13 @@
                 if cur is not None and keep:
                     pend["free"] = torch.cuda.Event()
                     pend["free"].record(cur)
-                K.pixpair_accumulate_split(xs, pend["alpha"], buf, geo[4])
+                if idx in self._pix_fresh:
+                    K.pixpair_accumulate_split(xs, pend["alpha"], buf, geo[4], overwrite=True)
+                    self._pix_fresh.discard(idx)
+                else:
+                    K.pixpair_accumulate_split(xs, pend["alpha"], buf, geo[4])
             else:
+                self._pix_settle(idx)
                 K.pixpair_accumulate_nhwc(xh, pend["alpha"], buf, geo[4])
                 if cur is not None and keep:
                     pend["free"] = torch.cuda.Event()
@@ -967,11 +975,27 @@
             return
         pad = lambda n: (n + 63) // 64 * 64
         numel = [math.prod(shape) for _, _, shape, _ in todo]
-        flat = torch.zeros(sum(pad(n) for n in numel), dtype=torch.float32, device=todo[0][3])
+        K = get_kernels()
+        lazy = (bool(getattr(K, "pixpair_overwrite", False)) and bool(getattr(K, "use_pixpair16", False)) and self.pix_group > 1
+                and todo[0][3].type == "cuda")
+        if lazy and any(geo[0] == "pair" for _, geo, _, _ in todo):
+            flat = torch.empty(sum(pad(n) for n in numel), dtype=torch.float32, device=todo[0][3])
+        else:
+            lazy = False
+            flat = torch.zeros(sum(pad(n) for n in numel), dtype=torch.float32, device=todo[0][3])
         off = 0
         for (idx, geo, shape, _), n in zip(todo, numel):
             self._pix[idx] = (geo, flat[off:off + n].view(shape))
+            if lazy and geo[0] == "pair":
+                self._pix_fresh.add(idx)
+            elif lazy:
+                self._pix[idx][1].zero_()
             off += pad(n)
+
+    def _pix_settle(self, idx):
+        if idx in self._pix_fresh:
+            self._pix_fresh.discard(idx)
+            self._pix[idx][1].zero_()
 
     flush_streams = 3
     lane_priority = -1
@@ -983,6 +1007,7 @@
 
         def one(idx):
             self._drain_pixpair(idx)
+            self._pix_settle(idx)
             geo, buf = self._pix.pop(idx)
             if geo[0] == "pair":
                 K.pixpair_assemble(buf, geo[4], geo[1], geo[2], geo[3], 1.0, self.factors[idx][1], upper_only=True)
@@ -1061,7 +1086,7 @@
     early_flush = True
     drain_before_fold = True
 
-    def _fold_lanes(self):
+    def _fold_lanes(self, defer_finish=False):
         self._flush_stash()
         subs, self._lane_accs = self._lane_accs, None
         if not subs:
@@ -1095,6 +1120,8 @@
             for sub in live:
                 sub._join_side()
         merged = set()
+        finish = {} if (defer_finish and on_device and getattr(K, "pixpair_finish", None) is not None) else None
+        self._pix_finish = finish
         if live:
             base = live[0]
 
@@ -1123,16 +1150,20 @@
                         else:
                             sub._pix_pending[idx] = pend
                             sub._drain_pixpair(idx)
+                    sub._pix_settle(idx)
                     others.append(o[1])
                     del sub._pix[idx]
                 if not others:
                     return False
                 base._drain_pixpair(idx)
+                base._pix_settle(idx)
                 del base._pix[idx]
                 A = base.factors[idx][1]
                 for o in others[1:]:
                     buf.add_(o)
-                if geo[0] == "pair":
+                if geo[0] == "pair" and finish is not None:
+                    finish[idx] = (geo, buf, others[0], self.factors is not None or any(idx in sub._pix_early for sub in live))
+                elif geo[0] == "pair":
                     K.pixpair_assemble(buf, geo[4], geo[1], geo[2], geo[3], 1.0, A, blocks2=others[0], upper_only=True)
                 else:
                     buf.add_(others[0])
@@ -1167,6 +1198,7 @@
             if self.factors is None:
                 self.factors, self.loss, self._taps_meta = sub.factors, sub.loss, sub._taps_meta
                 self._pix, self._pix_pending, self._gslabs = {}, {}, {}
+                self._pix_fresh = set()
                 self._gscale, self._tap_index = dict(sub._gscale), dict(sub._tap_index)
             else:
                 if set(self._gscale) != set(sub._gscale):
@@ -1364,6 +1396,8 @@
                 raise RuntimeError("clone() of an accumulator with dense pixel-pair / slab state is not supported")
             for idx in list(self._pix_pending):
                 self._drain_pixpair(idx)
+            for idx in list(self._pix_fresh):
+                self._pix_settle(idx)
             new.factors = [[t.clone() for t in F] for F in self.factors]
             new.loss = self.loss.clone()
             new._taps_meta = list(self._taps_meta)
@@ -1451,24 +1485,41 @@
     def finalize(self):
         K = get_kernels()
         rt = math.sqrt(float(self.backend.factor))
-        self._fold_lanes()
+        late = set(self._pix_inputs)
+        self._fold_lanes(defer_finish=True)
+        finish = self.__dict__.pop("_pix_finish", None) or {}
         self._resolve_pix_inputs()
         self._flush_pixgrams()
         self._flush_g_slabs()
         self._join_side()
+        fin_items = []
         items, done = [], []
         for idx, ((G, A), (has_bias, native)) in enumerate(zip(self.factors, self._taps_meta)):
             s_ = self._gscale.get(idx)
             if s_ is not None:
                 s_ = s_.detach().to(torch.float32).reshape(-1).contiguous()
             items.append((G, None, s_, 0, 1))
-            if native is not None and native[1] > 1:
+            if idx in finish:
+                geo, buf, other, dirty = finish[idx]
+                assert native is not None and native[1] == 9 and native[0] == geo[3]
+                A_out = torch.empty_like(A)
+                fin_items.append((buf, other, geo[4], geo[1], geo[2], geo[3], 1.0, A if (dirty or idx in late) else None, A_out))
+                A = A_out
+            elif native is not None and native[1] > 1:
                 A_out = torch.empty_like(A)
                 items.append((A, A_out, None, native[0], native[1]))
                 A = A_out
             else:
                 items.append((A, None, None, 0, 1))
             done.append((G, A, has_bias))
+        if fin_items:
+            cur = torch.cuda.current_stream(fin_items[0][0].device)
+            fin_items.sort(key=lambda it: -it[3] * it[4])
+            for k in range(0, len(fin_items), K.pixpair_finish_max):
+                K.pixpair_finish(fin_items[k:k + K.pixpair_finish_max])
+            for it in fin_items:
+                it[0].record_stream(cur)
+                it[1].record_stream(cur)
         K.finalize_factors(items)
         self._gscale = {}
         kfacs = []
diff --git a/laplace_amd/csrc/lk_gram.hip b/laplace_amd/csrc/lk_gram.hip
--- a/laplace_amd/csrc/lk_gram.hip
+++ b/laplace_amd/csrc/lk_gram.hip
@@ -1067,6 +1067,164 @@
   }
 }
 
+struct PfDesc {
+  const float* blocks;
+  const float* blocks2;
+  const int* slots;
+  const float* addend;
+  float* dst;
+  float alpha;
+  int H, W, Cin, T, blk0;
+};
+constexpr int PF_MAX = 48;
+struct PfBatch {
+  int count, nblk;
+  PfDesc d[PF_MAX];
+};
+constexpr int PF_THREADS = 512;
+static inline size_t pf_lds_bytes(int T) { return (size_t)(9 * T) * (9 * T + 1) * sizeof(float); }
+
+__global__ __launch_bounds__(PF_THREADS) void pixpair_finish_kernel(const PfBatch fb) {
+  extern __shared__ __attribute__((aligned(16))) float pf_region[];
+  int k = 0;
+  for (int i = 1; i < fb.count; ++i)
+    if ((int)blockIdx.x >= fb.d[i].blk0) k = i;
+  const PfDesc& D = fb.d[k];
+  const int T = D.T, Cin = D.Cin, H = D.H, W = D.W, HW = H * W;
+  const int RT = 9 * T, LD = RT + 1;
+  const int nt = Cin / T;
+  int bi = 0, bj;
+  {
+    int p = (int)blockIdx.x - D.blk0;
+    while (p >= nt - bi) p -= nt - bi, ++bi;
+    bj = bi + p;
+  }
+  const bool diag = bi == bj;
+  const int tid = threadIdx.x;
+  const int side = tid >> 8, rem = tid & 255;
+  const int F = T * T / 4, P = 256 / F;
+  const int part = rem / F, f4 = rem - part * F;
+  const int i = f4 / (T / 4), j = (f4 - i * (T / 4)) * 4;
+  const bool loads = !(diag && side == 1);
+  const int64_t bsz = (int64_t)Cin * Cin;
+  const int64_t inner = (int64_t)((side ? bj : bi) * T + i) * Cin + (side ? bi : bj) * T + j;
+  const int per = (HW + P - 1) / P;
+  const int q_lo = part * per < HW ? part * per : HW, q_hi = q_lo + per < HW ? q_lo + per : HW;
+  const float* __restrict__ blocks = D.blocks;
+  const float* __restrict__ blocks2 = D.blocks2;
+  const int* __restrict__ slots = D.slots;
+  constexpr int U = 8;
+  for (int h = 0; h < 13; ++h) {
+    const int Dy = h < 3 ? 0 : (h < 8 ? 1 : 2);
+    const int Dx = h < 3 ? h : (h < 8 ? h - 5 : h - 10);
+    const int dy_lo = -1, dy_hi = 1 - Dy;
+    const int dx_lo = Dx < 0 ? -1 - Dx : -1, dx_hi = Dx > 0 ? 1 - Dx : 1;
+    float4 acc[3][3];
+#pragma unroll
+    for (int a = 0; a < 3; ++a)
+#pragma unroll
+      for (int b = 0; b < 3; ++b) acc[a][b] = make_float4(0.f, 0.f, 0.f, 0.f);
+    if (loads && !(side == 1 && h == 0)) {
+      int qy0 = q_lo / W, qx0 = q_lo - qy0 * W;
+      for (int q0 = q_lo; q0 < q_hi; q0 += U) {
+        float4 v[U], w[U];
+        bool have[U];
+        int64_t off[U];
+#pragma unroll
+        for (int u = 0; u < U; ++u) {
+          const int q = q0 + u;
+          const int slot = slots[(q < q_hi ? q : q_lo) * 13 + h];
+          have[u] = q < q_hi && slot >= 0;
+          off[u] = (int64_t)(have[u] ? slot : 0) * bsz + inner;
+        }
+#pragma unroll
+        for (int u = 0; u < U; ++u) v[u] = *reinterpret_cast<const float4*>(blocks + off[u]);
+        if (blocks2) {
+#pragma unroll
+          for (int u = 0; u < U; ++u) w[u] = *reinterpret_cast<const float4*>(blocks2 + off[u]);
+#pragma unroll
+          for (int u = 0; u < U; ++u) v[u].x += w[u].x, v[u].y += w[u].y, v[u].z += w[u].z, v[u].w += w[u].w;
+        }
+        int qy = qy0, qx = qx0;
+#pragma unroll
+        for (int u = 0; u < U; ++u, ++qx) {
+          if (qx == W) qx = 0, ++qy;
+          if (!have[u]) continue;
+#pragma unroll
+          for (int a = 0; a < 3; ++a)
+#pragma unroll
+            for (int b = 0; b < 3; ++b) {
+              const int dy = a - 1, dx = b - 1;
+              if (dy >= dy_lo && dy <= dy_hi && dx >= dx_lo && dx <= dx_hi && qy - dy >= 0 && qy - dy < H && qx - dx >= 0 &&
+                  qx - dx < W)
+                acc[a][b].x += v[u].x, acc[a][b].y += v[u].y, acc[a][b].z += v[u].z, acc[a][b].w += v[u].w;
+            }
+        }
+        if (qx == W) qx = 0, ++qy;
+        qy0 = qy, qx0 = qx;
+      }
+    }
+    for (int ph = 0; ph < P; ++ph) {
+      if (ph == part && loads && !(side == 1 && h == 0)) {
+#pragma unroll
+        for (int a = 0; a < 3; ++a)
+#pragma unroll
+          for (int b = 0; b < 3; ++b) {
+            const int dy = a - 1, dx = b - 1;
+            if (!(dy >= dy_lo && dy <= dy_hi && dx >= dx_lo && dx <= dx_hi)) continue;
+            const int d = a * 3 + b, e = (dy + Dy + 1) * 3 + (dx + Dx + 1);
+            const float s4[4] = {acc[a][b].x, acc[a][b].y, acc[a][b].z, acc[a][b].w};
+#pragma unroll
+            for (int c = 0; c < 4; ++c) {
+              const int jc = j + c;
+              const int direct = (i * 9 + d) * LD + jc * 9 + e, mirror = (jc * 9 + e) * LD + i * 9 + d;
+              if (side == 1) {
+                pf_region[mirror] = (ph ? pf_region[mirror] : 0.f) + s4[c];
+              } else if (!diag) {
+                pf_region[direct] = (ph ? pf_region[direct] : 0.f) + s4[c];
+              } else if (h != 0) {
+                pf_region[direct] = (ph ? pf_region[direct] : 0.f) + s4[c];
+                pf_region[mirror] = (ph ? pf_region[mirror] : 0.f) + s4[c];
+              } else if (i <= jc) {
+                const float t = (ph ? pf_region[direct] : 0.f) + s4[c];
+                pf_region[direct] = t;
+                pf_region[mirror] = t;
+              }
+            }
+          }
+      }
+      __syncthreads();
+    }
+  }
+  const int n = 9 * Cin;
+  const float alpha = D.alpha;
+  const float* __restrict__ add = D.addend;
+  float* __restrict__ dst = D.dst;
+  const int RT4 = RT / 4;
+  for (int pass = 0; pass < (diag ? 1 : 2); ++pass) {
+    const int r0 = (pass ? bj : bi) * RT, c0 = (pass ? bi : bj) * RT;
+    for (int idx = tid; idx < RT * RT4; idx += PF_THREADS) {
+      const int rr = idx / RT4, cc = (idx - rr * RT4) * 4;
+      float o[4];
+#pragma unroll
+      for (int c = 0; c < 4; ++c) {
+        o[c] = alpha * (pass ? pf_region[(cc + c) * LD + rr] : pf_region[rr * LD + cc + c]);
+        if (add) {
+          const int r = r0 + rr, cl = c0 + cc + c;
+          const int ci = r / 9, d = r - ci * 9, cj = cl / 9, e = cl - cj * 9;
+          int rs = d * Cin + ci, cs = e * Cin + cj;
+          if (rs > cs) {
+            const int t = rs;
+            rs = cs, cs = t;
+          }
+          o[c] += add[(int64_t)rs * n + cs];
+        }
+      }
+      *reinterpret_cast<float4*>(dst + (int64_t)(r0 + rr) * n + c0 + cc) = make_float4(o[0], o[1], o[2], o[3]);
+    }
+  }
+}
+
 }
 
 using namespace lk;
@@ -1365,6 +1523,49 @@
   return lk_conv3x3_pixpair_assemble2_f32(blocks, nullptr, slots_dev, H, W, Cin, alpha, A, 0, stream);
 }
 
+static int pixpair_finish_checked(int64_t count, const float* const* blocks, const float* const* blocks2,
+                                  const int32_t* const* slots_dev, const int64_t* H, const int64_t* W, const int64_t* Cin,
+                                  const float* alpha, const float* const* addend, float* const* dst, void* stream) {
+  LK_REQUIRE(count >= 0 && count <= PF_MAX, "lk_conv3x3_pixpair_finish_f32: at most %d layers per call", PF_MAX);
+  LK_REQUIRE(count == 0 || (blocks && blocks2 && slots_dev && H && W && Cin && alpha && addend && dst),
+             "lk_conv3x3_pixpair_finish_f32: bad arguments");
+  if (count == 0) return LK_OK;
+  PfBatch fb;
+  fb.count = 0, fb.nblk = 0;
+  size_t lds = 0;
+  for (int64_t i = 0; i < count; ++i) {
+    LK_REQUIRE(blocks[i] && slots_dev[i] && dst[i] && H[i] >= 1 && W[i] >= 1 && H[i] * W[i] < (1ll << 24),
+               "lk_conv3x3_pixpair_finish_f32: bad layer (null pointer, or a map outside 1 <= H W < 2^24)");
+    LK_REQUIRE(Cin[i] >= 64 && Cin[i] % 64 == 0 && Cin[i] <= 8192, "lk_conv3x3_pixpair_finish_f32: needs Cin % 64 == 0, Cin <= 8192");
+    LK_REQUIRE(((reinterpret_cast<uintptr_t>(blocks[i]) | reinterpret_cast<uintptr_t>(blocks2[i]) | reinterpret_cast<uintptr_t>(dst[i])) & 15) == 0,
+               "lk_conv3x3_pixpair_finish_f32: 16-byte aligned buffers");
+    LK_REQUIRE(dst[i] != addend[i], "lk_conv3x3_pixpair_finish_f32: dst must not be the addend");
+    PfDesc& D = fb.d[fb.count];
+    D.blocks = blocks[i], D.blocks2 = blocks2[i], D.slots = slots_dev[i], D.addend = addend[i], D.dst = dst[i];
+    D.alpha = alpha[i], D.H = (int)H[i], D.W = (int)W[i], D.Cin = (int)Cin[i];
+    D.T = Cin[i] == 64 ? 8 : 16;
+    D.blk0 = fb.nblk;
+    const int64_t nt = Cin[i] / D.T;
+    fb.nblk += (int)(nt * (nt + 1) / 2);
+    if (pf_lds_bytes(D.T) > lds) lds = pf_lds_bytes(D.T);
+    ++fb.count;
+  }
+  if (hipFuncSetAttribute((const void*)pixpair_finish_kernel, hipFuncAttributeMaxDynamicSharedMemorySize, (int)pf_lds_bytes(16)) !=
+      hipSuccess) {
+    set_error("lk_conv3x3_pixpair_finish_f32: cannot raise the dynamic LDS limit to %zu bytes", pf_lds_bytes(16));
+    return LK_ELAUNCH;
+  }
+  hipLaunchKernelGGL(pixpair_finish_kernel, dim3((unsigned)fb.nblk), dim3(PF_THREADS), lds, (hipStream_t)stream, fb);
+  return check_launch("pixpair_finish_kernel");
+}
+
+extern "C" int lk_conv3x3_pixpair_finish_f32(int64_t count, const float* const* blocks, const float* const* blocks2,
+                                             const int32_t* const* slots_dev, const int64_t* H, const int64_t* W,
+                                             const int64_t* Cin, const float* alpha, const float* const* addend,
+                                             float* const* dst, void* stream) {
+  return pixpair_finish_checked(count, blocks, blocks2, slots_dev, H, W, Cin, alpha, addend, dst, stream);
+}
+
 extern "C" int lk_conv3x3_pixgram_assemble_f32(const float* Cp, int64_t H, int64_t W, int64_t Cin, float alpha, float* A,
                                                void* stream) {
   LK_REQUIRE(Cp && A && H >= 1 && W >= 1 && Cin >= 1 && H * W * Cin < (1ll << 31) && 9 * Cin < (1ll << 24),
diff --git a/laplace_amd/csrc/lk_sweep16.hip b/laplace_amd/csrc/lk_sweep16.hip
--- a/laplace_amd/csrc/lk_sweep16.hip
+++ b/laplace_amd/csrc/lk_sweep16.hip
@@ -174,7 +174,7 @@
   float* blocks;
 };
 
-template <int NB, int BKR, int KW, bool TNP>
+template <int NB, int BKR, int KW, bool TNP, bool OW = false>
 __global__ __launch_bounds__(256) void gram16_kernel(const _Float16* __restrict__ Xh, const _Float16* __restrict__ Xl,
                                                      int64_t R, int64_t C, int64_t rows_per_split,
                                                      const _Float16* __restrict__ zero16, float* __restrict__ ws,
@@ -258,7 +258,11 @@
 
   constexpr int NOLD = TNP ? (KW == 4 ? TW * TW * 4 : TW * TW * 16) : 1;
   float old[NOLD];
-  if constexpr (TNP) {
+  static_assert(TNP || !OW, "overwrite mode is a pixel-pair mode");
+  if constexpr (OW) {
+#pragma unroll
+    for (int i = 0; i < NOLD; ++i) old[i] = 0.f;
+  } else if constexpr (TNP) {
     const int lr_ = lane & 31, lh_ = lane >> 5;
     if (KW == 4) {
 #pragma unroll
@@ -569,6 +573,7 @@
 #ifndef LK_PIX13_ABLATE
 #define LK_PIX13_ABLATE 0
 #endif
+template <bool OW>
 __global__ __launch_bounds__(512) void pixpair13_kernel(const Pix13Args p) {
   constexpr int C = 64, BKR = 16, PLANE = BKR * C * 2, PANEL = 2 * PLANE, STAGE = 13 * PANEL;
   extern __shared__ __attribute__((aligned(16))) char smem[];
@@ -664,7 +669,7 @@
       if (myslot[i] < 0 || ((LK_PIX13_ABLATE & 1) && p.alpha != 12345.f)) continue;
       const float* blk = p.blocks + (int64_t)myslot[i] * (C * C);
 #pragma unroll
-      for (int r = 0; r < 16; ++r) old[i - i0][r] = blk[(t_a * 32 + (r & 3) + 8 * (r >> 2) + 4 * lh) * C + t_b * 32 + lr];
+      for (int r = 0; r < 16; ++r) old[i - i0][r] = OW ? 0.f : blk[(t_a * 32 + (r & 3) + 8 * (r >> 2) + 4 * lh) * C + t_b * 32 + lr];
     }
 #pragma unroll
     for (int i = i0; i < (i0 + 4 < 7 ? i0 + 4 : 7); ++i) {
@@ -678,48 +683,99 @@
 }
 }
 
-extern "C" int lk_conv3x3_pixpair_accumulate13_f16x2(const void* x_h, const void* x_l, const int* sexp, int64_t B, int64_t H,
-                                                     int64_t W, int64_t Cin, float alpha, float* blocks,
-                                                     const int32_t* slots_dev, const void* zero16, void* stream) {
+namespace {
+int pixpair_zero_blocks(float* blocks, int64_t H, int64_t W, int64_t Cin, hipStream_t st, const char* who) {
+  int64_t T, nt, nb;
+  if (int rc = lk_conv3x3_pixpair_plan(H, W, Cin, &T, &nt, &nb)) return rc;
+  if (hipMemsetAsync(blocks, 0, (size_t)nb * Cin * Cin * sizeof(float), st) != hipSuccess) {
+    set_error("%s: hipMemsetAsync failed", who);
+    return LK_ELAUNCH;
+  }
+  return LK_OK;
+}
+
+int pixpair13_checked(const void* x_h, const void* x_l, const int* sexp, int64_t B, int64_t H, int64_t W, int64_t Cin, float alpha,
+                      float* blocks, const int32_t* slots_dev, const void* zero16, void* stream, bool overwrite) {
   LK_REQUIRE(x_h && x_l && sexp && blocks && slots_dev && zero16 && B >= 0 && H >= 1 && W >= 1,
              "lk_conv3x3_pixpair_accumulate13_f16x2: bad arguments");
   LK_REQUIRE(Cin == 64 && H * W * Cin < (1ll << 31) && B < (1ll << 31) && H * W * 13 * Cin * Cin < (1ll << 31),
              "lk_conv3x3_pixpair_accumulate13_f16x2: needs Cin == 64 (and a map within 2^31 elements)");
-  if (B == 0) return LK_OK;
+  if (B == 0) return overwrite ? pixpair_zero_blocks(blocks, H, W, Cin, (hipStream_t)stream, "lk_conv3x3_pixpair_accumulate13_ow_f16x2") : LK_OK;
   Pix13Args a;
   a.xh = (const _Float16*)x_h, a.xl = (const _Float16*)x_l, a.zero16 = (const _Float16*)zero16, a.slots = slots_dev, a.sexp = sexp;
   a.blocks = blocks, a.alpha = alpha, a.R = (int)B, a.H = (int)H, a.W = (int)W;
   constexpr int LDS = 3 * 13 * 4096;
+  if (overwrite) {
+    if (hipFuncSetAttribute((const void*)pixpair13_kernel<true>, hipFuncAttributeMaxDynamicSharedMemorySize, LDS) != hipSuccess) {
+      set_error("lk_conv3x3_pixpair_accumulate13_ow_f16x2: cannot raise the dynamic LDS limit to %d bytes", LDS);
+      return LK_ELAUNCH;
+    }
+    hipLaunchKernelGGL(pixpair13_kernel<true>, dim3((unsigned)(H * W)), dim3(512), LDS, (hipStream_t)stream, a);
+    return check_launch("pixpair13_kernel<overwrite>");
+  }
   static bool attr_set = false;
   if (!attr_set) {
-    (void)hipFuncSetAttribute((const void*)pixpair13_kernel, hipFuncAttributeMaxDynamicSharedMemorySize, LDS);
+    (void)hipFuncSetAttribute((const void*)pixpair13_kernel<false>, hipFuncAttributeMaxDynamicSharedMemorySize, LDS);
     attr_set = true;
   }
-  hipLaunchKernelGGL(pixpair13_kernel, dim3((unsigned)(H * W)), dim3(512), LDS, (hipStream_t)stream, a);
+  hipLaunchKernelGGL(pixpair13_kernel<false>, dim3((unsigned)(H * W)), dim3(512), LDS, (hipStream_t)stream, a);
   return check_launch("pixpair13_kernel");
 }
 
-extern "C" int lk_conv3x3_pixpair_accumulate_f16x2(const void* x_h, const void* x_l, const int* sexp, int64_t B, int64_t H,
-                                                   int64_t W, int64_t Cin, float alpha, float* blocks,
-                                                   const int32_t* tiles_dev, int64_t n_tiles, const void* zero16,
-                                                   void* stream) {
+int pixpair16_checked(const void* x_h, const void* x_l, const int* sexp, int64_t B, int64_t H, int64_t W, int64_t Cin, float alpha,
+                      float* blocks, const int32_t* tiles_dev, int64_t n_tiles, const void* zero16, void* stream, bool overwrite) {
   LK_REQUIRE(x_h && x_l && sexp && blocks && tiles_dev && zero16 && B >= 0 && n_tiles >= 0,
              "lk_conv3x3_pixpair_accumulate_f16x2: bad arguments");
   LK_REQUIRE(Cin >= 64 && Cin % 64 == 0 && n_tiles < (1ll << 31) && H * W * Cin < (1ll << 31),
              "lk_conv3x3_pixpair_accumulate_f16x2: needs Cin % 64 == 0");
+  if (overwrite) {
+    int64_t T, nt, nb;
+    if (int rc = lk_conv3x3_pixpair_plan(H, W, Cin, &T, &nt, &nb)) return rc;
+    LK_REQUIRE(nt == n_tiles, "lk_conv3x3_pixpair_accumulate_ow_f16x2: table does not match the geometry");
+    if (B == 0) return pixpair_zero_blocks(blocks, H, W, Cin, (hipStream_t)stream, "lk_conv3x3_pixpair_accumulate_ow_f16x2");
+  }
   if (B == 0 || n_tiles == 0) return LK_OK;
   Gram16Tnp tp;
   tp.tiles = tiles_dev, tp.ldc = (int)Cin, tp.sexp = sexp, tp.alpha = alpha, tp.blocks = blocks;
   hipStream_t st = (hipStream_t)stream;
   const int64_t ld = H * W * Cin;
+#define LK_PP16(NB, BKR, KW, OW)                                                                                              \
+  hipLaunchKernelGGL((gram16_kernel<NB, BKR, KW, true, OW>), dim3((unsigned)n_tiles), dim3(256), (2 * Gram16Cfg<NB, BKR, KW>::STAGE), \
+                     st, (const _Float16*)x_h, (const _Float16*)x_l, B, ld, B, (const _Float16*)zero16, (float*)nullptr, 0, tp)
   if (Cin % 128) {
-    using Gc = Gram16Cfg<64, 64, 4>;
-    hipLaunchKernelGGL((gram16_kernel<64, 64, 4, true>), dim3((unsigned)n_tiles), dim3(256), 2 * Gc::STAGE, st,
-                       (const _Float16*)x_h, (const _Float16*)x_l, B, ld, B, (const _Float16*)zero16, (float*)nullptr, 0, tp);
+    if (overwrite) LK_PP16(64, 64, 4, true);
+    else LK_PP16(64, 64, 4, false);
   } else {
-    using Gc = Gram16Cfg<128, 32, 1>;
-    hipLaunchKernelGGL((gram16_kernel<128, 32, 1, true>), dim3((unsigned)n_tiles), dim3(256), 2 * Gc::STAGE, st,
-                       (const _Float16*)x_h, (const _Float16*)x_l, B, ld, B, (const _Float16*)zero16, (float*)nullptr, 0, tp);
-  }
+    if (overwrite) LK_PP16(128, 32, 1, true);
+    else LK_PP16(128, 32, 1, false);
+  }
+#undef LK_PP16
   return check_launch("gram16_kernel<pixel pairs>");
 }
+}
+
+extern "C" int lk_conv3x3_pixpair_accumulate13_f16x2(const void* x_h, const void* x_l, const int* sexp, int64_t B, int64_t H,
+                                                     int64_t W, int64_t Cin, float alpha, float* blocks,
+                                                     const int32_t* slots_dev, const void* zero16, void* stream) {
+  return pixpair13_checked(x_h, x_l, sexp, B, H, W, Cin, alpha, blocks, slots_dev, zero16, stream, false);
+}
+
+extern "C" int lk_conv3x3_pixpair_accumulate13_ow_f16x2(const void* x_h, const void* x_l, const int* sexp, int64_t B, int64_t H,
+                                                        int64_t W, int64_t Cin, float alpha, float* blocks,
+                                                        const int32_t* slots_dev, const void* zero16, void* stream) {
+  return pixpair13_checked(x_h, x_l, sexp, B, H, W, Cin, alpha, blocks, slots_dev, zero16, stream, true);
+}
+
+extern "C" int lk_conv3x3_pixpair_accumulate_f16x2(const void* x_h, const void* x_l, const int* sexp, int64_t B, int64_t H,
+                                                   int64_t W, int64_t Cin, float alpha, float* blocks,
+                                                   const int32_t* tiles_dev, int64_t n_tiles, const void* zero16,
+                                                   void* stream) {
+  return pixpair16_checked(x_h, x_l, sexp, B, H, W, Cin, alpha, blocks, tiles_dev, n_tiles, zero16, stream, false);
+}
+
+extern "C" int lk_conv3x3_pixpair_accumulate_ow_f16x2(const void* x_h, const void* x_l, const int* sexp, int64_t B, int64_t H,
+                                                      int64_t W, int64_t Cin, float alpha, float* blocks,
+                                                      const int32_t* tiles_dev, int64_t n_tiles, const void* zero16,
+                                                      void* stream) {
+  return pixpair16_checked(x_h, x_l, sexp, B, H, W, Cin, alpha, blocks, tiles_dev, n_tiles, zero16, stream, true);
+}
```

Result: no change. 21000 samples/s, median of 5 (+0.1%).
